# justinkay/aldi

Measured on AMD Instinct MI355X. Metric: images/sec (student+teacher ALDI step), R50-FPN 1333x800, higher is better.
Workload: dtype bf16

## Files before the change

### aldi_amd/_lib.py

```python
from __future__ import annotations

import ctypes as C
import os
import re

_HERE = os.path.dirname(os.path.abspath(__file__))
LIB_PATH = os.path.join(_HERE, "lib", "libaldi_hip.so")
HEADER_PATH = os.path.join(os.path.dirname(_HERE), "include", "aldi_hip.h")


class AldiHipError(RuntimeError):
    pass


if not os.path.exists(LIB_PATH):
    raise ImportError(
        f"{LIB_PATH} not found: build it with `python -c 'import __graft_entry__ as g; g.build()'` "
        "(or `make -C aldi_amd/csrc`). There is no CPU fallback for the ALDI HIP path.")

lib = C.CDLL(LIB_PATH)

F32, BF16 = 0, 1
MAX_IMAGES, MAX_LEVELS = 16, 5
c_void_p, c_int, c_float, c_long = C.c_void_p, C.c_int, C.c_float, C.c_long


def _ctype(decl: str):
    decl = decl.strip()
    if "*" in decl or decl.startswith("aldi_stream_t"):
        return C.c_void_p
    base = decl.rsplit(" ", 1)[0].replace("const", "").strip() if " " in decl else decl
    return {"int": C.c_int, "long": C.c_long, "float": C.c_float, "size_t": C.c_size_t, "unsigned": C.c_uint, "unsigned long long": C.c_ulonglong,
            "double": C.c_double}[base]


def parse_header(path: str = HEADER_PATH):
    src = open(path).read()
    src = re.sub(r"/\*.*?\*/", "", src, flags=re.S)
    protos = {}
    for m in re.finditer(r"\b(int|long|size_t|const char\*)\s+(aldi_\w+)\s*\(([^;{}]*?)\)\s*;", src, flags=re.S):
        ret, name, args = m.group(1), m.group(2), m.group(3)
        args = " ".join(args.split())
        argtypes = [] if args in ("void", "") else [_ctype(a) for a in args.split(",")]
        restype = {"int": C.c_int, "long": C.c_long, "size_t": C.c_size_t, "const char*": C.c_char_p}[ret]
        protos[name] = (restype, argtypes)
    return protos


PROTOS = parse_header()
for _name, (_res, _args) in PROTOS.items():
    _fn = getattr(lib, _name)
    _fn.restype = _res
    _fn.argtypes = _args


def check(status: int, what: str = ""):
    if status != 0:
        raise AldiHipError(f"{what}: status {status}: {lib.aldi_last_error().decode()}")


def call(name: str, *args):
    check(getattr(lib, name)(*args), name)


def set_tuning(name: str, value: int):
    call("aldi_set_tuning", name.encode(), int(value))


def get_tuning(name: str) -> int:
    v = C.c_int(0)
    call("aldi_get_tuning", name.encode(), C.byref(v))
    return v.value


def reset_tuning():
    call("aldi_reset_tuning")


def last_dispatch() -> str:
    return lib.aldi_last_dispatch().decode()


def plan_dispatch(args, n: int = 1) -> str:
    buf = C.create_string_buffer(224)
    call("aldi_conv_igemm_plan", C.byref(args) if isinstance(args, C.Structure) else args, n, buf, len(buf))
    return buf.value.decode()


def plan_wgrad_dispatch(args, n: int = 1, group: bool = False):
    buf = C.create_string_buffer(224)
    ws = C.c_long(0)
    call("aldi_conv_wgrad_plan", C.byref(args) if isinstance(args, C.Structure) else args, n, int(group), buf, len(buf), C.byref(ws))
    return buf.value.decode(), ws.value


class BoxLossChunk(C.Structure):
    _fields_ = [("r0", c_int), ("r1", c_int), ("grad_scale_cls", c_float), ("grad_scale_box", c_float), ("loss_box", c_void_p),
                ("teacher_pred", c_void_p), ("cls_temperature", c_float), ("kl", c_int), ("do_cls", c_int), ("do_reg", c_int),
                ("grad_scale_distill_cls", c_float), ("grad_scale_distill_reg", c_float), ("loss_distill", c_void_p)]


class ConvArgs(C.Structure):
    _fields_ = [
        ("x", c_void_p), ("w", c_void_p), ("y", c_void_p), ("y_f32", c_void_p),
        ("scale", c_void_p), ("shift", c_void_p), ("res", c_void_p), ("mask", c_void_p),
        ("N", c_int), ("H", c_int), ("W", c_int), ("Cin", c_int),
        ("Cout", c_int), ("KH", c_int), ("KW", c_int), ("stride", c_int), ("pad", c_int),
        ("Ho", c_int), ("Wo", c_int),
        ("relu", c_int), ("res_mode", c_int), ("out_scale", c_int), ("OH", c_int), ("OW", c_int),
        ("dtype", c_int), ("ws", c_void_p), ("ksplit", c_int), ("mask_bits", c_void_p), ("bits_out", c_void_p),
    ]


class WgradArgs(C.Structure):
    _fields_ = [
        ("x", c_void_p), ("g", c_void_p), ("dw", c_void_p), ("scale", c_void_p),
        ("N", c_int), ("H", c_int), ("W", c_int), ("Cin", c_int), ("Cout", c_int), ("KH", c_int), ("KW", c_int),
        ("stride", c_int), ("pad", c_int), ("Ho", c_int), ("Wo", c_int), ("dtype", c_int), ("db", c_void_p),
        ("ws", c_void_p), ("ws_bytes", C.c_long),
    ]


class StemArgs(C.Structure):
    _fields_ = [
        ("img", c_void_p), ("w", c_void_p), ("scale", c_void_p), ("shift", c_void_p), ("y", c_void_p),
        ("N", c_int), ("Hs", c_int), ("Ws", c_int), ("Hc", c_int), ("Wc", c_int),
        ("h", c_int * MAX_IMAGES), ("w_img", c_int * MAX_IMAGES),
        ("mean", c_float * 3), ("std", c_float * 3), ("dtype", c_int),
    ]


class RpnGeom(C.Structure):
    _fields_ = [
        ("num_levels", c_int), ("A", c_int), ("C", c_int),
        ("H", c_int * MAX_LEVELS), ("W", c_int * MAX_LEVELS), ("off", c_int * (MAX_LEVELS + 1)),
    ]


class RoiFeats(C.Structure):
    _fields_ = [
        ("feat", c_void_p * 4), ("grad", c_void_p * 4), ("H", c_int * 4), ("W", c_int * 4),
        ("scale", c_float * 4), ("C", c_int),
    ]


class DgwItem(C.Structure):
    _fields_ = [("w_master", c_void_p), ("scale", c_void_p), ("wt", c_void_p),
                ("Cout", c_int), ("KH", c_int), ("KW", c_int), ("Cin", c_int), ("tile_begin", c_int), ("reserved", c_int)]


class FoldItem(C.Structure):
    _fields_ = [("w", c_void_p), ("scale", c_void_p), ("out", c_void_p), ("rows", c_int), ("cols", c_int), ("chunk_begin", c_int), ("reserved", c_int)]


class BottleneckArgs(C.Structure):
    _fields_ = [("x", c_void_p), ("res", c_void_p), ("y", c_void_p), ("w1", c_void_p), ("w2", c_void_p), ("w3", c_void_p),
                ("b1", c_void_p), ("b2", c_void_p), ("b3", c_void_p),
                ("N", c_int), ("H", c_int), ("W", c_int), ("Cin", c_int), ("mid", c_int), ("Cout", c_int)]


class AttnArgs(C.Structure):
    _fields_ = [
        ("qkv", c_void_p), ("rel_h", c_void_p), ("rel_w", c_void_p),
        ("Qp", c_void_p), ("Kp", c_void_p), ("KpT", c_void_p), ("VT", c_void_p), ("QsT", c_void_p),
        ("O", c_void_p), ("lse", c_void_p), ("dO", c_void_p), ("dOT", c_void_p), ("dQp", c_void_p), ("delta", c_void_p),
        ("dqkv", c_void_p), ("drel_h", c_void_p), ("drel_w", c_void_p),
        ("nB", c_int), ("gh", c_int), ("gw", c_int), ("heads", c_int), ("Dq", c_int), ("scale", c_float),
    ]


PtrArray5 = c_void_p * MAX_LEVELS
```

### aldi_amd/csrc/igemm.hip

```cpp
#include "common.h"
#include "igemm_select.h"
#include "tile_prims.h"
#include <stdlib.h>

namespace {

template <typename T, int BM, int BN, int WM, int WN, int LDS_BYTES>
__device__ __forceinline__ void igemm_epilogue(const ConvDev& p, f32x4_t (&acc)[BM / WM / 16][BN / WN / 16], const int m0, const int n0, unsigned char* stg) {
    constexpr int NT = WM * WN * 64;
    constexpr int TM = BM / WM / 16, TN = BN / WN / 16;
    const int tid = threadIdx.x, lane = tid & 63, wave = tid >> 6;
    const int wm = wave / WN, wn = wave % WN;
    const int fr = lane & 15, fq = lane >> 4;
    if (p.dbg & 4) return;
    T* __restrict__ Y = static_cast<T*>(p.y);
    const T* __restrict__ R = static_cast<const T*>(p.res);
    const T* __restrict__ Mk = static_cast<const T*>(p.mask);
    if constexpr (sizeof(T) == 2) {
        constexpr int ROWB = BN * 2 + 16;
        constexpr bool kStageFits = BM * ROWB <= LDS_BYTES;
        if (kStageFits && Y && !p.y_f32 && (p.Cout & 7) == 0) {
            __syncthreads();
            {
                unsigned char* wr = stg + (wm * (BM / WM) + fr) * ROWB + (wn * (BN / WN) + fq * 4) * 2;
#pragma unroll
                for (int j = 0; j < TN; ++j) {
                    const int c = n0 + wn * (BN / WN) + j * 16 + fq * 4;
                    float4 sc = make_float4(1.f, 1.f, 1.f, 1.f), sh = make_float4(0.f, 0.f, 0.f, 0.f);
                    if (c < p.Cout) {
                        if (p.scale) sc = *reinterpret_cast<const float4*>(p.scale + c);
                        if (p.shift) sh = *reinterpret_cast<const float4*>(p.shift + c);
                    }
#pragma unroll
                    for (int i = 0; i < TM; ++i) {
                        uint2 t;
                        if (p.scale || p.shift) {
                            t.x = pack2_bf16(acc[i][j][0] * sc.x + sh.x, acc[i][j][1] * sc.y + sh.y);
                            t.y = pack2_bf16(acc[i][j][2] * sc.z + sh.z, acc[i][j][3] * sc.w + sh.w);
                        } else {
                            t.x = pack2_bf16(acc[i][j][0], acc[i][j][1]);
                            t.y = pack2_bf16(acc[i][j][2], acc[i][j][3]);
                        }
                        *reinterpret_cast<uint2*>(wr + i * 16 * ROWB + j * 32) = t;
                    }
                }
            }
            __syncthreads();
            constexpr int CPR = BN / 8;
            constexpr int RPI = NT / CPR;
            const int rowl0 = tid / CPR, ch8 = tid % CPR;
            const int c = n0 + ch8 * 8;
            if (c >= p.Cout) return;
            const bool plain = p.out_scale == 1 && p.res_mode != 2;
            const unsigned char* rd = stg + rowl0 * ROWB + ch8 * 16;
            typedef short s16x2_t __attribute__((ext_vector_type(2)));
            constexpr int NI = BM / RPI;
            constexpr unsigned OOBX = 0x80000000u;
            const __amdgpu_buffer_rsrc_t ry = make_rsrc_uniform(Y, 0x7fffffffu);
            unsigned ooff[NI], roff[NI], boff[NI];
#pragma unroll
            for (int it = 0; it < NI; ++it) {
                const int m = m0 + rowl0 + it * RPI;
                const bool ok = m < p.M;
                unsigned oidx, ridx;
                if (plain) {
                    oidx = (unsigned)m * (unsigned)p.Cout;
                    ridx = oidx;
                } else {
                    const int mm = ok ? m : 0;
                    const int n = mm / (p.Ho * p.Wo);
                    const int r = mm - n * (p.Ho * p.Wo);
                    const int ho = r / p.Wo, wo = r - ho * p.Wo;
                    if (p.out_scale == 1) oidx = (unsigned)mm * (unsigned)p.Cout;
                    else oidx = (unsigned)((((long)n * p.OH + ho * p.out_scale) * p.OW + wo * p.out_scale) * p.Cout);
                    if (p.res_mode == 2) ridx = (unsigned)((((long)n * (p.Ho >> 1) + (ho >> 1)) * (p.Wo >> 1) + (wo >> 1)) * p.Cout);
                    else ridx = oidx;
                }
                ooff[it] = ok ? (oidx + (unsigned)c) * 2u : OOBX;
                roff[it] = ok ? (ridx + (unsigned)c) * 2u : OOBX;
                boff[it] = ok ? (oidx + (unsigned)c) >> 3 : OOBX;
            }
            u32x4_t rres[NI], rmsk[NI];
            if (p.res_mode) {
                const __amdgpu_buffer_rsrc_t rr_ = make_rsrc_uniform(R, 0x7fffffffu);
#pragma unroll
                for (int it = 0; it < NI; ++it) rres[it] = __builtin_amdgcn_raw_buffer_load_b128(rr_, roff[it], 0, 0);
            }
            if (Mk) {
                const __amdgpu_buffer_rsrc_t rm_ = make_rsrc_uniform(Mk, 0x7fffffffu);
#pragma unroll
                for (int it = 0; it < NI; ++it) rmsk[it] = __builtin_amdgcn_raw_buffer_load_b128(rm_, ooff[it], 0, 0);
            }
            unsigned rbits[NI];
            if (p.mask_bits) {
                const __amdgpu_buffer_rsrc_t rb_ = make_rsrc_uniform(p.mask_bits, 0x7fffffffu);
#pragma unroll
                for (int it = 0; it < NI; ++it) rbits[it] = __builtin_amdgcn_raw_buffer_load_b8(rb_, boff[it], 0, 0);
            }
            const __amdgpu_buffer_rsrc_t rbo = make_rsrc_uniform(p.bits_out, 0x7fffffffu);
#pragma unroll
            for (int it = 0; it < NI; ++it) {
                const uint4 raw4 = *reinterpret_cast<const uint4*>(rd + it * RPI * ROWB);
                uint32_t raw[4] = {raw4.x, raw4.y, raw4.z, raw4.w};
                if (p.res_mode) {
                    const uint32_t rs[4] = {rres[it].x, rres[it].y, rres[it].z, rres[it].w};
#pragma unroll
                    for (int q = 0; q < 4; ++q) {
                        float lo = __uint_as_float(raw[q] << 16) + __uint_as_float(rs[q] << 16);
                        float hi = __uint_as_float(raw[q] & 0xffff0000u) + __uint_as_float(rs[q] & 0xffff0000u);
                        if (p.relu) { lo = fmaxf(lo, 0.f); hi = fmaxf(hi, 0.f); }
                        raw[q] = pack2_bf16(lo, hi);
                    }
                } else if (p.relu) {
#pragma unroll
                    for (int q = 0; q < 4; ++q) {
                        s16x2_t v = *reinterpret_cast<s16x2_t*>(&raw[q]);
                        v = __builtin_elementwise_max(v, s16x2_t{0, 0});
                        raw[q] = *reinterpret_cast<uint32_t*>(&v);
                    }
                }
                if (Mk) {
                    const uint32_t ms[4] = {rmsk[it].x, rmsk[it].y, rmsk[it].z, rmsk[it].w};
#pragma unroll
                    for (int q = 0; q < 4; ++q) {
                        s16x2_t k = *reinterpret_cast<const s16x2_t*>(&ms[q]);
                        k = __builtin_elementwise_min(__builtin_elementwise_max(k, s16x2_t{0, 0}), s16x2_t{1, 1});
                        s16x2_t v = *reinterpret_cast<s16x2_t*>(&raw[q]);
                        v = v * k;
                        raw[q] = *reinterpret_cast<uint32_t*>(&v);
                    }
                }
                if (p.mask_bits) {
                    const unsigned b = rbits[it];
#pragma unroll
                    for (int q = 0; q < 4; ++q) {
                        const unsigned k32 = ((b >> (2 * q)) & 1u) | (((b >> (2 * q + 1)) & 1u) << 16);
                        s16x2_t k = *reinterpret_cast<const s16x2_t*>(&k32);
                        s16x2_t v = *reinterpret_cast<s16x2_t*>(&raw[q]);
                        v = v * k;
                        raw[q] = *reinterpret_cast<uint32_t*>(&v);
                    }
                }
                const u32x4_t ov = {raw[0], raw[1], raw[2], raw[3]};
                __builtin_amdgcn_raw_buffer_store_b128(ov, ry, ooff[it], 0, 0);
                if (p.bits_out) {
                    unsigned b = 0;
#pragma unroll
                    for (int q = 0; q < 4; ++q) {
                        b |= ((short)(raw[q] & 0xffffu) > 0 ? 1u : 0u) << (2 * q);
                        b |= ((short)(raw[q] >> 16) > 0 ? 1u : 0u) << (2 * q + 1);
                    }
                    __builtin_amdgcn_raw_buffer_store_b8((unsigned char)b, rbo, boff[it], 0, 0);
                }
            }
            return;
        }
    }
#pragma unroll
    for (int i = 0; i < TM; ++i) {
        int m = m0 + wm * (BM / WM) + i * 16 + fr;
        if (m >= p.M) continue;
        long oidx, ridx = 0;
        if (p.out_scale == 1 && p.res_mode != 2) {
            oidx = (long)m * p.Cout;
            ridx = oidx;
        } else {
            int n = m / (p.Ho * p.Wo);
            int r = m - n * (p.Ho * p.Wo);
            int ho = r / p.Wo, wo = r - ho * p.Wo;
            if (p.out_scale == 1) oidx = (long)m * p.Cout;
            else oidx = (((long)n * p.OH + ho * p.out_scale) * p.OW + wo * p.out_scale) * p.Cout;
            if (p.res_mode == 2) ridx = (((long)n * (p.Ho >> 1) + (ho >> 1)) * (p.Wo >> 1) + (wo >> 1)) * p.Cout;
            else ridx = oidx;
        }
#pragma unroll
        for (int j = 0; j < TN; ++j) {
            int c = n0 + wn * (BN / WN) + j * 16 + fq * 4;
            if (c >= p.Cout) continue;
            float v[4] = {acc[i][j][0], acc[i][j][1], acc[i][j][2], acc[i][j][3]};
            if (p.scale) {
                float4 sc = *reinterpret_cast<const float4*>(p.scale + c);
                v[0] *= sc.x; v[1] *= sc.y; v[2] *= sc.z; v[3] *= sc.w;
            }
            if (p.shift) {
                float4 sh = *reinterpret_cast<const float4*>(p.shift + c);
                v[0] += sh.x; v[1] += sh.y; v[2] += sh.z; v[3] += sh.w;
            }
            if (p.res_mode) {
                float r4[4];
                load4(R + ridx + c, r4);
                v[0] += r4[0]; v[1] += r4[1]; v[2] += r4[2]; v[3] += r4[3];
            }
            if (p.relu) {
#pragma unroll
                for (int r = 0; r < 4; ++r) v[r] = v[r] > 0.f ? v[r] : 0.f;
            }
            if (Mk) {
                float k4[4];
                load4(Mk + oidx + c, k4);
#pragma unroll
                for (int r = 0; r < 4; ++r) v[r] = k4[r] > 0.f ? v[r] : 0.f;
            }
            if (Y) store4(Y + oidx + c, v);
            if (p.y_f32) store4(p.y_f32 + oidx + c, v);
        }
    }
}


template <int N, int ROWB, int I = 0>
__device__ __forceinline__ void frag_read_each(u32x4_t* f, const unsigned* addr) {
    if constexpr (I < N) {
        f[I] = frag_read<I * 16 * ROWB>(addr[I]);
        frag_read_each<N, ROWB, I + 1>(f, addr);
    }
}

template <int WNE>
__device__ __forceinline__ int direct_perm(int row) {
    const int wv = row / WNE, rr = row % WNE, j = rr >> 4, r = rr & 15;
    return wv * WNE + (j >> 1) * 32 + (r >> 2) * 8 + (j & 1) * 4 + (r & 3);
}
__device__ __forceinline__ unsigned lds_read_u8(unsigned addr) {
    unsigned v;
    asm volatile("ds_read_u8 %0, %1" : "=v"(v) : "v"(addr));
    return v;
}
template <int BM, int BN, int WM, int WN, bool RESL>
__device__ __forceinline__ void igemm_epilogue_direct(const ConvDev& p, f32x4_t (&acc)[BM / WM / 16][BN / WN / 16], const int m0, const int n0,
                                                      u32x4_t (&rres)[BM / WM / 16][BN / WN / 32], const unsigned aux_addr) {
    constexpr int TM = BM / WM / 16, TN = BN / WN / 16, WNE = BN / WN, H = WNE / 32;
    static_assert(TN == 2 * H, "whole 32-channel blocks per wave");
    const int tid = threadIdx.x, lane = tid & 63, wave = tid >> 6;
    const int wm = wave / WN, wn = wave % WN;
    const int fr = lane & 15, fq = lane >> 4;
    if (p.dbg & 4) return;
    u32x4_t sc[TN], sh[TN];
    const bool has_sc = p.scale != nullptr, has_sh = p.shift != nullptr;
#pragma unroll
    for (int j = 0; j < TN; ++j) {
        const unsigned a = aux_addr + (unsigned)(wn * WNE + (j >> 1) * 32 + fq * 8 + (j & 1) * 4) * 4u;
        sc[j] = frag_read<0>(a);
        sh[j] = frag_read<256>(a);
    }
    unsigned mb[TM][H];
#pragma unroll
    for (int i = 0; i < TM; ++i)
#pragma unroll
        for (int h = 0; h < H; ++h) mb[i][h] = lds_read_u8(aux_addr + (unsigned)((wm * (BM / WM) + i * 16 + fr) * (BN / 8) + (wn * H + h) * 4 + fq));
    asm volatile("s_waitcnt lgkmcnt(0)" ::: "memory");
#pragma unroll
    for (int j = 0; j < TN; ++j) { asm volatile("" : "+v"(sc[j])); asm volatile("" : "+v"(sh[j])); }
#pragma unroll
    for (int i = 0; i < TM; ++i)
#pragma unroll
        for (int h = 0; h < H; ++h) asm volatile("" : "+v"(mb[i][h]));
    const bool has_res = RESL && p.res_mode != 0;
    if constexpr (RESL) {
        if (has_res) {
#pragma unroll
            for (int i = 0; i < TM; ++i)
#pragma unroll
                for (int h = 0; h < H; ++h) asm volatile("" : "+v"(rres[i][h]));
        }
    }
    const __amdgpu_buffer_rsrc_t ry = make_rsrc_uniform(p.y, 0x7fffffffu);
    const __amdgpu_buffer_rsrc_t rbo = make_rsrc_uniform(p.bits_out, 0x7fffffffu);
    typedef short s16x2_t __attribute__((ext_vector_type(2)));
    typedef unsigned short u16x2_t __attribute__((ext_vector_type(2)));
#pragma unroll
    for (int i = 0; i < TM; ++i) {
        const int m = m0 + wm * (BM / WM) + i * 16 + fr;
#pragma unroll
        for (int h = 0; h < H; ++h) {
            const int c = n0 + wn * WNE + h * 32 + fq * 8;
            const bool ok = m < p.M && c < p.Cout;
            const unsigned e0 = (unsigned)m * (unsigned)p.Cout + (unsigned)c;
            float v[8];
#pragma unroll
            for (int e = 0; e < 4; ++e) { v[e] = acc[i][2 * h][e]; v[4 + e] = acc[i][2 * h + 1][e]; }
            if (has_sc) {
#pragma unroll
                for (int e = 0; e < 4; ++e) { v[e] *= __uint_as_float(sc[2 * h][e]); v[4 + e] *= __uint_as_float(sc[2 * h + 1][e]); }
            }
            if (has_sh) {
#pragma unroll
                for (int e = 0; e < 4; ++e) { v[e] += __uint_as_float(sh[2 * h][e]); v[4 + e] += __uint_as_float(sh[2 * h + 1][e]); }
            }
            if constexpr (RESL) {
                if (has_res) {
#pragma unroll
                    for (int q = 0; q < 4; ++q) {
                        const unsigned r2 = rres[i][h][q];
                        v[2 * q] += __uint_as_float(r2 << 16);
                        v[2 * q + 1] += __uint_as_float(r2 & 0xffff0000u);
                    }
                }
            }
            if (p.mask_bits) {
#pragma unroll
                for (int t = 0; t < 8; ++t) v[t] = __uint_as_float(__float_as_uint(v[t]) & (unsigned)__builtin_amdgcn_sbfe((int)mb[i][h], t, 1));
            }
            uint32_t d[4];
#pragma unroll
            for (int q = 0; q < 4; ++q) d[q] = pack2_bf16(v[2 * q], v[2 * q + 1]);
            if (p.relu) {
#pragma unroll
                for (int q = 0; q < 4; ++q) {
                    s16x2_t t = *reinterpret_cast<s16x2_t*>(&d[q]);
                    t = __builtin_elementwise_max(t, s16x2_t{0, 0});
                    d[q] = *reinterpret_cast<uint32_t*>(&t);
                }
            }
            const u32x4_t ov = {d[0], d[1], d[2], d[3]};
            __builtin_amdgcn_raw_buffer_store_b128(ov, ry, ok ? e0 * 2u : 0x80000000u, 0, 0);
            if (p.bits_out) {
                unsigned u = 0;
#pragma unroll
                for (int q = 0; q < 4; ++q) {
                    u16x2_t t = *reinterpret_cast<u16x2_t*>(&d[q]);
                    if (!p.relu) { s16x2_t s_ = *reinterpret_cast<s16x2_t*>(&d[q]); s_ = __builtin_elementwise_max(s_, s16x2_t{0, 0}); t = *reinterpret_cast<u16x2_t*>(&s_); }
                    t = __builtin_elementwise_min(t, u16x2_t{1, 1});
                    u |= *reinterpret_cast<unsigned*>(&t) << (2 * q);
                }
                const unsigned b = (u & 0x55u) | ((u >> 15) & 0xaau);
                __builtin_amdgcn_raw_buffer_store_b8((unsigned char)b, rbo, ok ? e0 >> 3 : 0x80000000u, 0, 0);
            }
        }
    }
}

template <typename T, int BM, int BN, int WM, int WN, int KC, bool PIPE, bool HALO = false, int EPI = 0, bool LEAN = false>
__device__ __forceinline__ void igemm_body(const ConvDev& p, int bid, const int nmt, const int nnt) {
    static_assert(!LEAN || (EPI != 0 && !HALO), "lean K loop: the direct-epilogue tap tiles");
    constexpr int NT = WM * WN * 64;
    constexpr bool DIRECT = EPI != 0, RESL = EPI == 2;
    static_assert(!DIRECT || (sizeof(T) == 2 && BN == 64 && (BN / WN) % 32 == 0 && BM * BN / 32 <= NT), "direct epilogue: bf16, 64-channel tiles");
    static_assert(!RESL || (PIPE && !HALO), "residual prefetch: the register-pipelined 1x1 loop");
    constexpr int EP = Elem<T>::kPer16B;
    constexpr int BK = KC * EP;
    constexpr int LOG = KC == 8 ? 3 : 2;
    constexpr int A_IT = (BM * KC) / NT;
    constexpr int B_IT = (BN * KC + NT - 1) / NT;
    constexpr int TM = BM / WM / 16, TN = BN / WN / 16;
    static_assert(HALO || (BM * KC) % NT == 0, "tile/threads mismatch");

    constexpr int NBUF = 3;
    constexpr int SLOTS = HALO ? ((BM + 2) * KC + 63) / 64 * 64 + 3 * BN * KC : (BM + BN) * KC;
    constexpr int NSTAGE = HALO ? 2 : NBUF;
    constexpr int AUX_SLOTS = DIRECT ? 64 : 0;
    constexpr int ZERO_SLOTS = HALO ? 4 : 0;
    __shared__ __attribute__((aligned(128))) uint4 lds_all[NSTAGE * SLOTS + AUX_SLOTS + ZERO_SLOTS];
    uint4 (*const lds)[SLOTS] = reinterpret_cast<uint4 (*)[SLOTS]>(&lds_all[0]);
    uint4* const aux_lds = &lds_all[NSTAGE * SLOTS];
    constexpr int N_RES = RESL ? (BM / WM / 16) * (BN / WN / 32) : 0;
    constexpr int N_PRE = DIRECT ? N_RES + 1 : 0;
    u32x4_t rres[BM / WM / 16][BN / WN / 32 > 0 ? BN / WN / 32 : 1];

    const int tid = threadIdx.x, lane = tid & 63, wave = tid >> 6;
    const int wm = wave / WN, wn = wave % WN;
    if (p.xcd) {
        const int total = nmt * nnt, q = total >> 3, r = total & 7, xcd = bid & 7, idx = bid >> 3;
        bid = (xcd < r ? xcd * (q + 1) : r * (q + 1) + (xcd - r) * q) + idx;
    }
    const int m0 = (bid / nnt) * BM, n0 = (bid % nnt) * BN;
    const T* __restrict__ X = static_cast<const T*>(p.x);
    const T* __restrict__ Wt = static_cast<const T*>(p.w);

    const __amdgpu_buffer_rsrc_t rx = __builtin_amdgcn_make_buffer_rsrc(const_cast<T*>(X), 0, p.x_bytes, 0x00020000);
    const __amdgpu_buffer_rsrc_t rw = __builtin_amdgcn_make_buffer_rsrc(const_cast<T*>(Wt), 0, p.w_bytes, 0x00020000);
    constexpr unsigned OOB = 0x80000000u;
    const int wbase = __builtin_amdgcn_readfirstlane(tid & ~63);
    auto issue_pre = [&]() {
        if constexpr (DIRECT) {
            if constexpr (RESL) {
                const __amdgpu_buffer_rsrc_t rr = make_rsrc_uniform(p.res, 0x7fffffffu);
#pragma unroll
                for (int i = 0; i < BM / WM / 16; ++i) {
                    const int m = m0 + wm * (BM / WM) + i * 16 + (lane & 15);
                    unsigned ridx = (unsigned)m;
                    if (p.res_mode == 2) {
                        const int mm = m < p.M ? m : 0;
                        const int n = mm / (p.Ho * p.Wo), r = mm - n * (p.Ho * p.Wo), ho = r / p.Wo, wo = r - ho * p.Wo;
                        ridx = (unsigned)((n * (p.Ho >> 1) + (ho >> 1)) * (p.Wo >> 1) + (wo >> 1));
                    }
#pragma unroll
                    for (int h = 0; h < BN / WN / 32; ++h) {
                        const int ch = n0 + wn * (BN / WN) + h * 32 + (lane >> 4) * 8;
                        const bool ok = p.res_mode && m < p.M && ch < p.Cout;
                        rres[i][h] = __builtin_amdgcn_raw_buffer_load_b128(rr, ok ? (ridx * (unsigned)p.Cout + (unsigned)ch) * 2u : OOB, 0, 0);
                    }
                }
            }
            if (p.mask_bits) {
                const __amdgpu_buffer_rsrc_t rb = make_rsrc_uniform(p.mask_bits, 0x7fffffffu);
                const int row = tid >> 1, m = m0 + row, ch = n0 + (tid & 1) * 32;
                const bool ok = tid < BM * 2 && m < p.M && ch < p.Cout;
                __builtin_amdgcn_raw_ptr_buffer_load_lds(rb, (__attribute__((address_space(3))) void*)(reinterpret_cast<unsigned*>(aux_lds) + wbase), 4,
                                                         ok ? ((unsigned)m * (unsigned)p.Cout + (unsigned)ch) >> 3 : OOB, 0, 0, 0);
            } else {
                const bool odd = __builtin_amdgcn_readfirstlane(wave) & 1;
                const float* src = odd ? p.shift : p.scale;
                const __amdgpu_buffer_rsrc_t rs = make_rsrc_uniform(src, 0x7fffffffu);
                const int ch = n0 + lane;
                __builtin_amdgcn_raw_ptr_buffer_load_lds(rs, (__attribute__((address_space(3))) void*)(reinterpret_cast<unsigned*>(aux_lds) + (odd ? 64 : 0)), 4,
                                                         src && ch < p.Cout ? (unsigned)ch * 4u : OOB, 0, 0, 0);
            }
        }
    };
    f32x4_t acc[TM][TN];
#pragma unroll
    for (int i = 0; i < TM; ++i)
#pragma unroll
        for (int j = 0; j < TN; ++j) acc[i][j] = f32x4_t{0.f, 0.f, 0.f, 0.f};

    const int fr = lane & 15, fq = lane >> 4;
    bool pre_seen = true;
    if constexpr (HALO) {
    static_assert(KC == 4, "halo form: one MFMA k-step per tap");
    constexpr int AS = ((BM + 2) * KC + 63) / 64 * 64;
    constexpr int WS = 3 * BN * KC;
    constexpr int AH_IT = (AS + NT - 1) / NT, WH_IT = WS / NT;
    static_assert(WS % NT == 0, "weight slots per thread");
    unsigned ha_voff[AH_IT], ha_mask[AH_IT];
#pragma unroll
    for (int it = 0; it < AH_IT; ++it) {
        const int c = tid + it * NT, row = c >> 2, kce = swz_halo(row, c & 3);
        const int q0 = m0 - 1 + row;
        const bool ok = row < BM + 2 && q0 >= 0 && q0 < p.M;
        const int qq = ok ? q0 : 0;
        const int h0 = (qq / p.W) % p.H;
        ha_voff[it] = ((unsigned)qq * (unsigned)p.Cin + (unsigned)(kce * EP)) * (unsigned)sizeof(T);
        ha_mask[it] = ok ? ((h0 >= 1 ? 1u : 0u) | 2u | (h0 <= p.H - 2 ? 4u : 0u)) : 0u;
    }
    unsigned hw_voff[WH_IT];
#pragma unroll
    for (int it = 0; it < WH_IT; ++it) {
        const int c = tid + it * NT, kwi = c / (BN * KC), rem = c - kwi * (BN * KC), row = rem >> 2, kce = swz_halo(row, rem & 3);
        const int co = n0 + (DIRECT ? direct_perm<BN / WN>(row) : row);
        hw_voff[it] = co < p.Cout ? ((unsigned)co * (unsigned)p.K + (unsigned)(kwi * p.Cin + kce * EP)) * (unsigned)sizeof(T) : OOB;
    }
    int gkh = 0, gci = 0;
    unsigned ha_cur[AH_IT], hw_cur[WH_IT];
    auto rebase = [&]() {
        const unsigned a_off = (unsigned)(((gkh - 1) * p.W * p.Cin) * (int)sizeof(T));
#pragma unroll
        for (int it = 0; it < AH_IT; ++it) ha_cur[it] = ((ha_mask[it] >> gkh) & 1u) ? ha_voff[it] + a_off : OOB;
    };
    rebase();
#pragma unroll
    for (int it = 0; it < WH_IT; ++it) hw_cur[it] = hw_voff[it];
    auto issue_group = [&](int buf) {
#pragma unroll
        for (int it = 0; it < AH_IT; ++it)
            if (wbase + it * NT < AS) {
                glds16(rx, &lds[buf][wbase + it * NT], ha_cur[it]);
                ha_cur[it] += (unsigned)(BK * sizeof(T));
            }
#pragma unroll
        for (int it = 0; it < WH_IT; ++it) glds16(rw, &lds[buf][AS + wbase + it * NT], hw_cur[it]);
        gci += BK;
        unsigned w_adv = (unsigned)(BK * sizeof(T));
        if (gci >= p.Cin) {
            gci = 0; ++gkh;
            w_adv = (unsigned)((2 * p.Cin + BK) * (int)sizeof(T));
            rebase();
        }
#pragma unroll
        for (int it = 0; it < WH_IT; ++it) hw_cur[it] += w_adv;
    };
    bool edge_l[TM], edge_r[TM];
#pragma unroll
    for (int i = 0; i < TM; ++i) {
        const int m = m0 + wm * (BM / WM) + i * 16 + fr;
        const int wo = m % p.W;
        edge_l[i] = wo == 0;
        edge_r[i] = wo == p.W - 1;
    }
    const int xrow = wm * (BM / WM) + fr, wrow = wn * (BN / WN) + fr;
    const unsigned lbase = lds_addr(&lds[0][0]);
    unsigned x_rd[3];
#pragma unroll
    for (int kw = 0; kw < 3; ++kw) x_rd[kw] = lbase + (unsigned)((xrow + kw) * KC + swz_halo(xrow + kw, fq)) * 16u;
    const unsigned w_rd = lbase + (unsigned)((AS + wrow * KC) + swz_halo(wrow, fq)) * 16u;
    uint4* const zero_lds = &lds_all[NSTAGE * SLOTS + AUX_SLOTS];
    if (tid < ZERO_SLOTS) zero_lds[tid] = make_uint4(0u, 0u, 0u, 0u);
    unsigned zaddr[TM];
#pragma unroll
    for (int i = 0; i < TM; ++i) zaddr[i] = lds_addr(zero_lds) + (unsigned)fq * 16u - (unsigned)(i * 16 * KC * 16);
    constexpr unsigned GROUP_BYTES = (AS + WS) * 16;
    const int G = 3 * (p.Cin / BK);
    issue_group(0);
    issue_pre();
    int buf = 0;
    for (int g = 0; g < G; ++g) {
        asm volatile("s_waitcnt vmcnt(0)" ::: "memory");
        __builtin_amdgcn_s_barrier();
        __builtin_amdgcn_sched_barrier(0);
        if (g + 1 < G) issue_group(buf ^ 1);
        u32x4_t xf[2][TM], wf[2][TN];
        const unsigned gb = (unsigned)buf * GROUP_BYTES;
        {
            unsigned xa[TM];
#pragma unroll
            for (int i = 0; i < TM; ++i) xa[i] = edge_l[i] ? zaddr[i] : x_rd[0] + gb;
            frag_read_each<TM, KC * 16>(xf[0], xa);
        }
        frag_read_all<TN, KC * 16>(wf[0], w_rd + gb);
        frag_wait<TM, TN>(xf[0], wf[0]);
#pragma unroll
        for (int kw = 0; kw < 3; ++kw) {
            const int cur = kw & 1, nxt = cur ^ 1;
            if (kw < 2) {
                if (kw + 1 == 2) {
                    unsigned xa[TM];
#pragma unroll
                    for (int i = 0; i < TM; ++i) xa[i] = edge_r[i] ? zaddr[i] : x_rd[2] + gb;
                    frag_read_each<TM, KC * 16>(xf[nxt], xa);
                } else {
                    frag_read_all<TM, KC * 16>(xf[nxt], x_rd[kw + 1] + gb);
                }
                frag_read_all<TN, KC * 16>(wf[nxt], w_rd + gb + (unsigned)((kw + 1) * BN * KC * 16));
            }
#pragma unroll
            for (int i = 0; i < TM; ++i)
#pragma unroll
                for (int j = 0; j < TN; ++j) acc[i][j] = Mma<T>::run(wf[cur][j], xf[cur][i], acc[i][j]);
            if (kw < 2) frag_wait<TM, TN>(xf[nxt], wf[nxt]);
        }
        buf ^= 1;
    }
    } else {
    unsigned a_voff[A_IT], a_mask[A_IT];
    int a_kce[A_IT];
    unsigned b_voff[B_IT];
    int b_kce[B_IT];
    const bool ktail = !LEAN && (p.K % BK) != 0;
    if constexpr (LEAN) {
#pragma unroll
        for (int it = 0; it < A_IT; ++it) {
            const int c = tid + it * NT, row = c >> LOG, kce = swz<KC>(row, c & (KC - 1)), m = m0 + row;
            a_voff[it] = m < p.M ? ((unsigned)m * (unsigned)p.Cin + (unsigned)(kce * EP)) * (unsigned)sizeof(T) : OOB;
// ... 203 lines not shown
    if (p.xcd) {
        const int total = nmt * nnt, q = total >> 3, r = total & 7, xcd = bid & 7, idx = bid >> 3;
        bid = (xcd < r ? xcd * (q + 1) : r * (q + 1) + (xcd - r) * q) + idx;
    }
    const int m0 = (bid / nnt) * BM, n0 = (bid % nnt) * BN;
    const T* __restrict__ X = static_cast<const T*>(p.x);
    const T* __restrict__ Wt = static_cast<const T*>(p.w);
    const __amdgpu_buffer_rsrc_t rx = __builtin_amdgcn_make_buffer_rsrc(const_cast<T*>(X), 0, p.x_bytes, 0x00020000);
    const __amdgpu_buffer_rsrc_t rw = __builtin_amdgcn_make_buffer_rsrc(const_cast<T*>(Wt), 0, p.w_bytes, 0x00020000);
    constexpr unsigned OOB = 0x80000000u;
    const int wbase = __builtin_amdgcn_readfirstlane(tid & ~63);
    const bool half_b = __builtin_amdgcn_readfirstlane(wave) >= 4;
    const bool third_pix = wbase + 2 * NT < AS;
    f32x4_t acc[TM][TN];
#pragma unroll
    for (int i = 0; i < TM; ++i)
#pragma unroll
        for (int j = 0; j < TN; ++j) acc[i][j] = f32x4_t{0.f, 0.f, 0.f, 0.f};
    const int fr = lane & 15, fq = lane >> 4;
    if (tid < 4) lds[NS * STAGE + tid] = make_uint4(0u, 0u, 0u, 0u);

    unsigned ha_voff[AH_IT], ha_mask[AH_IT];
#pragma unroll
    for (int it = 0; it < AH_IT; ++it) {
        const int c = tid + it * NT, row = c >> 2, kce = swz_halo(row, c & 3);
        const int q0 = m0 - 1 + row;
        const bool ok = row < BM + 2 && q0 >= 0 && q0 < p.M;
        const int qq = ok ? q0 : 0;
        const int h0 = (qq / p.W) % p.H;
        ha_voff[it] = ((unsigned)qq * (unsigned)p.Cin + (unsigned)(kce * EP)) * (unsigned)sizeof(T);
        ha_mask[it] = ok ? ((h0 >= 1 ? 1u : 0u) | 2u | (h0 <= p.H - 2 ? 4u : 0u)) : 0u;
    }
    unsigned hw_voff[WH_IT];
#pragma unroll
    for (int it = 0; it < WH_IT; ++it) {
        const int c = tid + it * NT, kwi = c / (BN * KC), rem = c - kwi * (BN * KC), row = rem >> 2, kce = swz_halo(row, rem & 3);
        const int co = n0 + row;
        hw_voff[it] = co < p.Cout ? ((unsigned)co * (unsigned)p.K + (unsigned)(kwi * p.Cin + kce * EP)) * (unsigned)sizeof(T) : OOB;
    }
    const int xrow = wm * (BM / WM) + fr, wrow = wn * (BN / WN) + fr;
    const unsigned lbase = lds_addr(&lds[0]);
    const unsigned zrow = lbase + (unsigned)(NS * STAGE) * 16u + (unsigned)fq * 16u;
    bool edge_l[TM], edge_r[TM];
    unsigned zaddr[TM];
#pragma unroll
    for (int i = 0; i < TM; ++i) {
        const int m = m0 + wm * (BM / WM) + i * 16 + fr;
        const int wo = m % p.W;
        edge_l[i] = wo == 0;
        edge_r[i] = wo == p.W - 1;
        zaddr[i] = zrow - (unsigned)(i * 16 * KC * 16);
    }
    unsigned x_rd[3];
#pragma unroll
    for (int kw = 0; kw < 3; ++kw) x_rd[kw] = lbase + (unsigned)((xrow + kw) * KC + swz_halo(xrow + kw, fq)) * 16u;
    const unsigned w_rd = lbase + (unsigned)((AS + wrow * KC) + swz_halo(wrow, fq)) * 16u;
    constexpr unsigned STAGE_BYTES = STAGE * 16;
    const int G = 3 * (p.Cin / BK);

    unsigned a_off = 0, w_off = 0, ikh = 0;
    int gkh = 0, gci = 0;
    auto next_group = [&]() {
        a_off = (unsigned)(((gkh - 1) * p.W * p.Cin + gci) * (int)sizeof(T));
        w_off = (unsigned)((gkh * 3 * p.Cin + gci) * (int)sizeof(T));
        ikh = (unsigned)gkh;
        gci += BK;
        if (gci >= p.Cin) { gci = 0; ++gkh; }
    };
    const unsigned dmask = (p.dbg & 16) ? 0xfffu : 0xffffffffu;
    const bool no_dma = p.dbg & 32, no_mfma = p.dbg & 64;
    auto issue_pair = [&](int pair, int st) {
        uint4* base = &lds[st * STAGE];
        if (no_dma) return;
        if (pair == 0) {
            glds16(rx, base + wbase, ((ha_mask[0] >> ikh) & 1u) ? (ha_voff[0] + a_off) & dmask : OOB);
            glds16(rx, base + wbase + NT, ((ha_mask[1] >> ikh) & 1u) ? (ha_voff[1] + a_off) & dmask : OOB);
        } else if (pair == 1) {
            glds16(rw, base + AS + wbase, hw_voff[0] == OOB ? OOB : (hw_voff[0] + w_off) & dmask);
            glds16(rw, base + AS + wbase + NT, hw_voff[1] == OOB ? OOB : (hw_voff[1] + w_off) & dmask);
        } else {
            glds16(rw, base + AS + wbase + 2 * NT, hw_voff[2] == OOB ? OOB : (hw_voff[2] + w_off) & dmask);
            if (third_pix) glds16(rx, base + wbase + 2 * NT, ((ha_mask[2] >> ikh) & 1u) ? (ha_voff[2] + a_off) & dmask : OOB);
        }
    };
    next_group();
    issue_pair(0, 0); issue_pair(1, 0); issue_pair(2, 0);
    next_group();
    issue_pair(0, 1); issue_pair(1, 1);
    asm volatile("s_waitcnt vmcnt(4)" ::: "memory");
    __builtin_amdgcn_s_barrier();
    __builtin_amdgcn_sched_barrier(0);
    if (half_b) {
        __builtin_amdgcn_s_barrier();
        __builtin_amdgcn_sched_barrier(0);
    }
    int rs = 0, s1 = 1, s2 = 2;
    for (int g = 0; g < G; ++g) {
        const unsigned gb = (unsigned)rs * STAGE_BYTES;
#pragma unroll
        for (int t = 0; t < 3; ++t) {
            u32x4_t xf[TM], wf[TN];
            if (t == 1) {
                frag_read_all<TM, KC * 16>(xf, x_rd[1] + gb);
            } else {
                unsigned xa[TM];
#pragma unroll
                for (int i = 0; i < TM; ++i) xa[i] = (t == 0 ? edge_l[i] : edge_r[i]) ? zaddr[i] : x_rd[t] + gb;
                frag_read_each<TM, KC * 16>(xf, xa);
            }
            frag_read_all<TN, KC * 16>(wf, w_rd + gb + (unsigned)(t * BN * KC * 16));
            if (t == 0) {
                if (g + 1 < G) issue_pair(2, s1);
            } else if (g + 2 < G) {
                if (t == 1) next_group();
                issue_pair(t - 1, s2);
            }
            if (t == 2 && g + 1 < G) {
                if (g + 2 < G && !no_dma) asm volatile("s_waitcnt vmcnt(4)" ::: "memory");
                else asm volatile("s_waitcnt vmcnt(0)" ::: "memory");
            }
            __builtin_amdgcn_sched_barrier(0);
            __builtin_amdgcn_s_barrier();
            __builtin_amdgcn_sched_barrier(0);
            frag_wait<TM, TN>(xf, wf);
            __builtin_amdgcn_sched_barrier(0);
            __builtin_amdgcn_s_setprio(1);
            if (!no_mfma) {
#pragma unroll
                for (int i = 0; i < TM; ++i)
#pragma unroll
                    for (int j = 0; j < TN; ++j) acc[i][j] = Mma<T>::run(wf[j], xf[i], acc[i][j]);
            }
            __builtin_amdgcn_s_setprio(0);
            __builtin_amdgcn_sched_barrier(0);
            __builtin_amdgcn_s_barrier();
            __builtin_amdgcn_sched_barrier(0);
        }
        const int o = rs; rs = s1; s1 = s2; s2 = o;
    }
    if (!half_b) {
        __builtin_amdgcn_s_barrier();
        __builtin_amdgcn_sched_barrier(0);
    }
    igemm_epilogue<T, BM, BN, WM, WN, NS * STAGE * 16>(p, acc, m0, n0, reinterpret_cast<unsigned char*>(&lds[0]));
}

template <typename T, int BN>
__global__ __launch_bounds__(512) void igemm_halo_rs_kernel(ConvDev p) {
    igemm_halo_rs_body<T, BN>(p, (int)(blockIdx.y * gridDim.x + blockIdx.x), (int)gridDim.x, (int)gridDim.y);
}

#include "igemm_halo64.h"
#include "igemm_ws.h"

template <int BM, int NT, bool HALO> constexpr int min_waves_per_simd() { return HALO && BM == 240 ? 2 * NT / 256 : 1; }
template <typename T, int BM, int BN, int WM, int WN, int KC, bool PIPE, bool HALO = false, int EPI = 0, bool LEAN = false>
__global__ __launch_bounds__(WM* WN * 64, (min_waves_per_simd<BM, WM * WN * 64, HALO>())) void igemm_kernel(ConvDev p) {
    igemm_body<T, BM, BN, WM, WN, KC, PIPE, HALO, EPI, LEAN>(p, (int)(blockIdx.y * gridDim.x + blockIdx.x), (int)gridDim.x, (int)gridDim.y);
}

template <typename T, int BM, int BN, int WM, int WN, int KC, bool PIPE, bool HALO = false>
__global__ __launch_bounds__(WM* WN * 64, (min_waves_per_simd<BM, WM * WN * 64, HALO>())) void igemm_group_kernel(ConvGroup G) {
    const int bid = (int)blockIdx.x;
    int i = 0;
    for (int k = 1; k < G.n; ++k)
        if (bid >= G.wg_begin[k]) i = k;
    i = __builtin_amdgcn_readfirstlane(i);
    const int local = bid - G.wg_begin[i];
    if (local >= G.nmt[i] * G.nnt[i]) return;
    igemm_body<T, BM, BN, WM, WN, KC, PIPE, HALO>(G.p[i], local, G.nmt[i], G.nnt[i]);
}

template <int BM, int BN, int WM, int WN, bool DIRECT, bool ILV = false>
__global__ __launch_bounds__(WM* WN * 64) void igemm_halo64_group_kernel(ConvGroup G) {
    const int bid = (int)blockIdx.x;
    int i = 0;
    for (int k = 1; k < G.n; ++k)
        if (bid >= G.wg_begin[k]) i = k;
    i = __builtin_amdgcn_readfirstlane(i);
    const int local = bid - G.wg_begin[i];
    if (local >= G.nmt[i] * G.nnt[i]) return;
    igemm_halo64_body<BM, BN, WM, WN, DIRECT, ILV>(G.p[i], local, G.nmt[i], G.nnt[i]);
}


int group_table(ConvGroup& G, const int BM, const int BN, const ConvDev& d) {
    int wg = 0;
    for (int i = 0; i < G.n; ++i) {
        G.p[i].xcd = d.xcd; G.p[i].dbg = d.dbg;
        G.nmt[i] = cdiv(G.p[i].M, BM); G.nnt[i] = cdiv(G.p[i].Cout, BN);
        G.wg_begin[i] = wg;
        wg += (G.nmt[i] * G.nnt[i] + 7) / 8 * 8;
    }
    for (int i = G.n; i <= kMaxConvGroup; ++i) G.wg_begin[i] = wg;
    return wg;
}

template <typename T, int BM, int BN, int WM, int WN, int KC, bool PIPE, bool HALO, int EPI>
int launch_tile(const Choice& c, const ConvDev& d, const ConvGroup* g, hipStream_t st) {
    constexpr int NT = WM * WN * 64;
    if constexpr (EPI != 0) {
        const dim3 grid(cdiv(d.M, BM), cdiv(d.Cout, BN));
        if constexpr (!HALO) {
            if (c.lean) hipLaunchKernelGGL((igemm_kernel<T, BM, BN, WM, WN, KC, PIPE, HALO, EPI, true>), grid, dim3(NT), 0, st, d);
        }
        if (HALO || !c.lean) hipLaunchKernelGGL((igemm_kernel<T, BM, BN, WM, WN, KC, PIPE, HALO, EPI, false>), grid, dim3(NT), 0, st, d);
    } else if (g) {
        ConvGroup G = *g;
        const int wg = group_table(G, BM, BN, d);
        hipLaunchKernelGGL((igemm_group_kernel<T, BM, BN, WM, WN, KC, PIPE, HALO>), dim3(wg), dim3(NT), 0, st, G);
    } else {
        const dim3 grid(cdiv(d.M, BM), cdiv(d.Cout, BN), d.ksplit > 1 ? d.ksplit : 1);
        hipLaunchKernelGGL((igemm_kernel<T, BM, BN, WM, WN, KC, PIPE, HALO>), grid, dim3(NT), 0, st, d);
    }
    ALDI_CHECK_LAUNCH();
    return ALDI_OK;
}
template <typename T, int BM, int BN, int WM, int WN, int KC, bool PIPE, int EPI>
int launch_TAP(const Choice& c, const ConvDev& d, const ConvGroup* g, hipStream_t st) { return launch_tile<T, BM, BN, WM, WN, KC, PIPE, false, EPI>(c, d, g, st); }
template <typename T, int BM, int BN, int WM, int WN, int KC, bool PIPE, int EPI>
int launch_HALO(const Choice& c, const ConvDev& d, const ConvGroup* g, hipStream_t st) { return launch_tile<T, BM, BN, WM, WN, KC, PIPE, true, EPI>(c, d, g, st); }

template <typename T, int BM, int BN, int WM, int WN, int KC, bool PIPE, int EPI>
int launch_ROLES(const Choice&, const ConvDev& d, const ConvGroup*, hipStream_t st) {
    static_assert(BM == 256 && WM * WN * 64 == 512, "igemm_halo_rs_body: 256 pixels on eight waves");
    const dim3 grid(cdiv(d.M, BM), cdiv(d.Cout, BN));
    hipLaunchKernelGGL((igemm_halo_rs_kernel<T, BN>), grid, dim3(512), 0, st, d);
    ALDI_CHECK_LAUNCH();
    return ALDI_OK;
}

template <typename T, int BM, int BN, int WM, int WN, int KC, bool PIPE, int EPI>
int launch_HALO64(const Choice& c, const ConvDev& d, const ConvGroup* g, hipStream_t st) {
    constexpr int NT = WM * WN * 64;
    constexpr bool HAS_ILV = BM == 256 && BN == 256 && WM == 4 && WN == 2;
    if (g) {
        ConvGroup G = *g;
        const int wg = group_table(G, BM, BN, d);
        if (c.ilv) {
            if (c.direct) hipLaunchKernelGGL((igemm_halo64_group_kernel<BM, BN, WM, WN, true, HAS_ILV>), dim3(wg), dim3(NT), 0, st, G);
            else hipLaunchKernelGGL((igemm_halo64_group_kernel<BM, BN, WM, WN, false, HAS_ILV>), dim3(wg), dim3(NT), 0, st, G);
        } else {
            if (c.direct) hipLaunchKernelGGL((igemm_halo64_group_kernel<BM, BN, WM, WN, true>), dim3(wg), dim3(NT), 0, st, G);
            else hipLaunchKernelGGL((igemm_halo64_group_kernel<BM, BN, WM, WN, false>), dim3(wg), dim3(NT), 0, st, G);
        }
    } else {
        const dim3 grid(cdiv(d.M, BM), cdiv(d.Cout, BN));
        if (c.ilv) {
            if (c.direct) hipLaunchKernelGGL((igemm_halo64_kernel<BM, BN, WM, WN, true, HAS_ILV>), grid, dim3(NT), 0, st, d);
            else hipLaunchKernelGGL((igemm_halo64_kernel<BM, BN, WM, WN, false, HAS_ILV>), grid, dim3(NT), 0, st, d);
        } else {
            if (c.direct) hipLaunchKernelGGL((igemm_halo64_kernel<BM, BN, WM, WN, true>), grid, dim3(NT), 0, st, d);
            else hipLaunchKernelGGL((igemm_halo64_kernel<BM, BN, WM, WN, false>), grid, dim3(NT), 0, st, d);
        }
    }
    ALDI_CHECK_LAUNCH();
    return ALDI_OK;
}

int launch_choice(const Choice& c, const ConvDev& d, const ConvGroup* g, hipStream_t st) {
    switch (c.tile) {
#define IGEMM_TILE_CASE(id, T, form, BM, BN, WM, WN, KC, PIPE, EPI) \
    case id: return launch_##form<T, BM, BN, WM, WN, KC, PIPE != 0, EPI>(c, d, g, st);
        IGEMM_TILES(IGEMM_TILE_CASE)
#undef IGEMM_TILE_CASE
    default: break;
    }
    return aldi_set_error_msg(ALDI_ERR_ARG, "conv_igemm: unknown tile");
}

__global__ __launch_bounds__(256) void splitk_finalize_kernel(const float* __restrict__ ws, int ks, long mc, int C, const float* __restrict__ scale,
                                                              const float* __restrict__ shift, int relu, bf16_t* __restrict__ y) {
    const long e = ((long)blockIdx.x * blockDim.x + threadIdx.x) * 4;
    if (e >= mc) return;
    float4 a = *reinterpret_cast<const float4*>(ws + e);
    for (int z = 1; z < ks; ++z) {
        const float4 b = *reinterpret_cast<const float4*>(ws + z * mc + e);
        a.x += b.x; a.y += b.y; a.z += b.z; a.w += b.w;
    }
    const int c = (int)(e % C);
    if (scale) { const float4 s4 = *reinterpret_cast<const float4*>(scale + c); a.x *= s4.x; a.y *= s4.y; a.z *= s4.z; a.w *= s4.w; }
    if (shift) { const float4 s4 = *reinterpret_cast<const float4*>(shift + c); a.x += s4.x; a.y += s4.y; a.z += s4.z; a.w += s4.w; }
    if (relu) { a.x = fmaxf(a.x, 0.f); a.y = fmaxf(a.y, 0.f); a.z = fmaxf(a.z, 0.f); a.w = fmaxf(a.w, 0.f); }
    uint2 o;
    o.x = pack2_bf16(a.x, a.y); o.y = pack2_bf16(a.z, a.w);
    *reinterpret_cast<uint2*>(y + e) = o;
}

constexpr int kNameCap = 112;

int conv_one(const aldi_conv_args* a, const bool dry, hipStream_t st, char* name) {
    ConvDev d;
    Choice c;
    if (int rc = plan_conv(a, aldi_tuning(), d, c)) return rc;
    dispatch_name(c, name, kNameCap);
    if (dry) return ALDI_OK;
    if (int rc = launch_choice(c, d, nullptr, st)) return rc;
    aldi_note_dispatch(name);
    if (c.ksplit > 1) {
        const long mc = (long)d.M * d.Cout;
        hipLaunchKernelGGL(splitk_finalize_kernel, dim3(cdiv(mc / 4, 256)), dim3(256), 0, st, static_cast<const float*>(a->ws), c.ksplit, mc, d.Cout, a->scale, a->shift,
                           a->relu, static_cast<bf16_t*>(a->y));
        ALDI_CHECK_LAUNCH();
    }
    return ALDI_OK;
}

int conv_many(const aldi_conv_args* args, const int n, const bool dry, hipStream_t st, char* name) {
    if (!args || n < 1) return aldi_set_error_msg(ALDI_ERR_ARG, "conv_igemm_group: no problems");
    if (n == 1 || !conv_group_same(args, n, aldi_tuning())) {
        for (int i = 0; i < n; ++i)
            if (int rc = conv_one(&args[i], dry, st, name)) return rc;
        return ALDI_OK;
    }
    static thread_local ConvGroup G;
    ConvDev d;
    Choice c;
    if (int rc = plan_conv_group(args, n, aldi_tuning(), G, d, c)) return rc;
    dispatch_name(c, name, kNameCap);
    if (dry) return ALDI_OK;
    if (int rc = launch_choice(c, d, &G, st)) return rc;
    aldi_note_dispatch(name);
    return ALDI_OK;
}
}

extern "C" int aldi_conv_igemm(const aldi_conv_args* a, aldi_stream_t stream) {
    char name[kNameCap];
    return conv_one(a, false, static_cast<hipStream_t>(stream), name);
}

extern "C" int aldi_conv_igemm_group(const aldi_conv_args* args, int n, aldi_stream_t stream) {
    char name[kNameCap];
    return conv_many(args, n, false, static_cast<hipStream_t>(stream), name);
}

extern "C" int aldi_conv_igemm_plan(const aldi_conv_args* args, int n, char* name, int cap) {
    char buf[kNameCap] = "";
    const int rc = n == 1 ? conv_one(args, true, nullptr, buf) : conv_many(args, n, true, nullptr, buf);
    if (rc == ALDI_OK && name && cap > 0) snprintf(name, (size_t)cap, "%s", buf);
    return rc;
}
```

### aldi_amd/csrc/igemm_select.h

```cpp
#pragma once
#include "host.h"
#include <stdio.h>

namespace {

struct ConvDev {
    const void* x; const void* w; void* y; float* y_f32;
    const float* scale; const float* shift; const void* res; const void* mask;
    int N, H, W, Cin, Cout, KH, KW, stride, pad, Ho, Wo;
    int relu, res_mode, out_scale, OH, OW;
    int M, K, xcd, dbg;
    unsigned x_bytes, w_bytes;
    int ksplit, slabs_per_split;
    int lean;
    const unsigned char* mask_bits; unsigned char* bits_out;
};

constexpr int kMaxConvGroup = 12;
struct ConvGroup {
    int n;
    int wg_begin[kMaxConvGroup + 1];
    int nmt[kMaxConvGroup], nnt[kMaxConvGroup];
    ConvDev p[kMaxConvGroup];
};
// ... 37 lines not shown
#undef IGEMM_TILE_ROW
};

struct Choice {
    TileId tile;
    bool lean;
    bool direct, ilv;
    int ksplit;
    int ws_wgs;
    int group_n;
};

inline int ws_channels(int K) { return K == 64 || K == 128 ? 256 : K == 256 || K == 512 ? 128 : 0; }
inline bool ws_ok(const ConvDev& d) {
    const int bn = ws_channels(d.K);
    return d.KH * d.KW == 1 && d.stride == 1 && d.pad == 0 && d.K == d.Cin && bn && d.Cout % bn == 0 && d.y && !d.y_f32 && !d.mask && d.out_scale == 1 &&
           d.ksplit <= 1 && (long)d.M * d.Cout * 2 < (1L << 31);
}
inline bool halo64_direct_ok(const ConvDev& d) {
    return d.y && !d.y_f32 && d.out_scale == 1 && (d.Cout & 7) == 0 && !d.mask && !d.mask_bits && !d.bits_out && !d.res_mode;
}
inline bool plain_1x1(const ConvDev& d) { return d.KH * d.KW == 1 && d.stride == 1 && d.pad == 0; }

inline Choice select_tile(const ConvDev& d, const AldiTuning& tn, const bool f32, const int group_n, const ConvDev* group = nullptr) {
    Choice c = {BF16_TAP_128x128, false, false, false, d.ksplit > 1 ? d.ksplit : 0, tn.igemm_ws_wgs, group_n};
    const auto pick = [&](TileId bf16_id, TileId f32_id) {
        c.tile = f32 ? f32_id : bf16_id;
        const TileRow& r = kTiles[c.tile];
        c.lean = r.form == TAP && r.epi != 0 && tn.igemm_lean && plain_1x1(d) && d.K % 64 == 0 && !(tn.igemm_dbg & (8 | 16));
        if (r.form == HALO64) {
            c.direct = (tn.igemm_direct & 8) != 0;
            for (int i = 0; i < (group_n ? group_n : 1); ++i) c.direct = c.direct && halo64_direct_ok(group_n ? group[i] : d);
            c.ilv = c.tile == BF16_HALO64_256x256 && tn.igemm_halo_ilv != 0;
        }
        return c;
    };
#define BOTH(name) pick(BF16_##name, F32_##name)
#define BF16(name) pick(BF16_##name, BF16_##name)
    const bool bf16 = !f32;
    if (d.ksplit > 1) {
        const int tile_knob = tn.igemm_splitk_tile;
        const bool big_ok = (long)cdiv(d.M, 256) * cdiv(d.Cout, 128) * d.ksplit >= 200;
        if (tile_knob == 3 || (tile_knob == 2 && big_ok)) return BF16(TAP_256x128_K64);
        if (tile_knob == 1 || (tile_knob == 4 && big_ok)) return BF16(TAP_256x128);
        return BF16(TAP_128x128_K64);
    }
    const long big = (long)cdiv(d.M, 128) * cdiv(d.Cout, 128);
    const int force = tn.igemm_force;
    const bool direct_ok = bf16 && !group_n && d.y && !d.y_f32 && d.out_scale == 1 && (d.Cout & 7) == 0 && !d.mask && d.ksplit <= 1 &&
                           !(d.mask_bits && (d.scale || d.shift)) && d.Cout >= 64 &&
                           !(d.mask_bits && (d.Cout & 31));
    const int direct = direct_ok ? tn.igemm_direct : 0;
    {
        const bool same3 = d.KH == 3 && d.KW == 3 && d.stride == 1 && d.pad == 1 && d.Ho == d.H && d.Wo == d.W && d.Cin % 32 == 0 && d.out_scale == 1;
        const bool f32_halo = f32 && tn.igemm_halo_f32 > 0 && (long)cdiv(d.M, 128) * cdiv(d.Cout, 64) >= tn.igemm_halo_f32;
        if (tn.igemm_halo && (bf16 || f32_halo) && same3) {
            if (force == 1) return BOTH(HALO_128x128);
            if (bf16 && force == 2 && (direct & 4) && !d.res_mode) return BF16(HALO_128x64_D);
            if (force == 2) return BOTH(HALO_128x64);
            if (force == 4) return BOTH(HALO_256x128);
            if (bf16) {
                if (force == 17 && (direct & 4) && !d.res_mode) return BF16(HALO_96x64_D);
                if (force == 17) return BF16(HALO_96x64);
                if (force == 16 && (direct & 4) && !d.res_mode) return BF16(HALO_64x64_D);
                if (force == 16) return BF16(HALO_64x64);
                if (force == 9) return BF16(HALO_240x128);
                if (force == 10 && !group_n) return BF16(ROLES_256x128);
                if (force == 11 && d.Cin % 64 == 0) return BF16(HALO64_256x256);
                if (force == 13 && d.Cin % 64 == 0) return BF16(HALO64_128x128);
                if (force == 15 && d.Cin % 64 == 0) return BF16(HALO64_256x256_W4);
            }
            if (force == 0 || force == 3) {
                if (d.Cout <= 64) return BOTH(HALO_128x64);
                if (big >= tn.igemm_bigtile_min) {
                    if (bf16 && tn.igemm_bigtile == 64 && d.Cin % 64 == 0 && d.Cout % 256 == 0) return BF16(HALO64_256x256);
                    if (bf16 && tn.igemm_bigtile == 65 && d.Cin % 64 == 0 && d.Cout % 256 == 0) return BF16(HALO64_256x256_W4);
                    if (tn.igemm_bigtile == 1) return BOTH(HALO_128x128);
                    if (bf16 && tn.igemm_bigtile == 10 && !group_n) return BF16(ROLES_256x128);
                    return BOTH(HALO_256x128);
                }
                if (bf16 && tn.igemm_halo64_mid > 0 && big >= tn.igemm_halo64_mid && d.Cin % 64 == 0 && d.Cout % 128 == 0) return BF16(HALO64_128x128);
                const long t64 = (long)cdiv(d.M, 128) * cdiv(d.Cout, 64);
                if (bf16 && tn.igemm_halo96 > 0 && t64 >= 200 && t64 <= 600) {
                    if ((direct & 4) && !d.res_mode) return BF16(HALO_96x64_D);
                    return BF16(HALO_96x64);
                }
                if (bf16 && tn.igemm_halo_small > 0 && t64 <= tn.igemm_halo_small && d.Cin >= 512) {
                    if ((direct & 4) && !d.res_mode) return BF16(HALO_64x64_D);
                    return BF16(HALO_64x64);
                }
                if (bf16 && (direct & 4) && !d.res_mode) return BF16(HALO_128x64_D);
                return BOTH(HALO_128x64);
            }
        }
    }
    if (bf16 && !group_n && ws_ok(d) && (force == 14 || (force == 0 && tn.igemm_ws && (tn.igemm_direct & 1) && d.M >= (d.res_mode == 2 ? 4L : 1L) * tn.igemm_ws_min)))
        return d.K == 64 ? BF16(WS_K64) : d.K == 128 ? BF16(WS_K128) : d.K == 256 ? BF16(WS_K256) : BF16(WS_K512);
    if (force == 5 || (force == 0 && d.Cout <= 16)) return BOTH(TAP_128x16);
    if (force == 1) return BOTH(TAP_128x128);
    if (bf16 && force == 2 && (direct & 1)) return d.res_mode ? BF16(TAP_128x64_DR) : BF16(TAP_128x64_D);
    if (force == 2) return BOTH(TAP_128x64);
    if (force == 3) return BOTH(TAP_64x64);
    if (force == 4) return BOTH(TAP_256x128);
    if (bf16) {
        const bool plain = plain_1x1(d);
        if (plain && force == 6) return BF16(TAP_128x128_K64);
        if (plain && force == 7) return BF16(TAP_128x64_K64);
        if (plain && force == 12 && (direct & 1) && !d.res_mode && d.K % 64 == 0) return BF16(TAP_128x64_K64_D);
        const bool lin256 = tn.igemm_tile != 9 && big >= tn.igemm_lintile_min && d.K >= tn.igemm_bigtile_k;
        if (plain && (force == 8 || (force == 0 && !lin256 && d.Cout > 64 && d.K % 64 == 0 && d.K >= tn.igemm_k64_min))) {
            if ((direct & 2) && !d.res_mode) return BF16(TAP_64x64_K64_D);
            return BF16(TAP_64x64_K64);
        }
    }
    if (f32 && force == 0 && big < tn.igemm_f32_tile64_max) return BOTH(TAP_64x64);
    if (d.Cout <= 64) return BOTH(TAP_128x64);
    if (tn.igemm_tile != 9 && big >= tn.igemm_lintile_min && d.K >= tn.igemm_bigtile_k) {
        if (bf16 && tn.igemm_tile != 7 && plain_1x1(d) && d.K % 64 == 0) return BF16(TAP_256x128_K64);
        return BOTH(TAP_256x128);
    }
    if (big < 200) return BOTH(TAP_64x64);
    if (bf16 && d.K <= tn.igemm_narrow_k && (direct & 1)) return d.res_mode ? BF16(TAP_128x64_DR) : BF16(TAP_128x64_D);
    if (bf16 && d.K <= tn.igemm_narrow_k) return BOTH(TAP_128x64);
    return BOTH(TAP_128x128);
#undef BOTH
#undef BF16
}

inline int dispatch_name(const Choice& c, char* name, int cap) {
    const TileRow& r = kTiles[c.tile];
    const char* elem = r.f32 ? "f32" : "bf16";
    const char* grp = c.group_n ? "_group" : "";
    switch (r.form) {
    case WS: return snprintf(name, cap, "igemm_ws<%s,%d,%d,k%d>", elem, r.BM, r.BN, r.KC * 8);
    case HALO64:
        return snprintf(name, cap, "igemm%s%.0d<%s,%d,%d,%d,%d,halo64%s%s>", grp, c.group_n, elem, r.BM, r.BN, r.WM, r.WN, c.direct ? ",direct" : "",
                        (c.tile == BF16_HALO64_256x256 && !c.ilv) ? ",lockstep" : "");
    case ROLES: return snprintf(name, cap, "igemm<%s,%d,%d,%d,%d,roles,halo>", elem, r.BM, r.BN, r.WM, r.WN);
    default:
        return snprintf(name, cap, "igemm%s%.0d<%s,%d,%d,%d,%d,%s,%s%s%s>%s", grp, c.group_n, elem, r.BM, r.BN, r.WM, r.WN, r.pipe ? "pipe" : "flat", r.form == HALO ? "halo" : "tap",
                        r.KC == 8 ? ",k64" : "", r.epi == 2 ? ",direct+res" : r.epi == 1 ? ",direct" : "", c.ksplit > 1 ? " splitk" : "");
    }
}

inline int fill_convdev(const aldi_conv_args* a, ConvDev& d) {
    if (!a || !a->x || !a->w || (!a->y && !a->y_f32)) return aldi_set_error_msg(ALDI_ERR_ARG, "conv_igemm: null pointer");
    const int bk = a->dtype == ALDI_BF16 ? 32 : 16;
    const int ep = a->dtype == ALDI_BF16 ? 8 : 4;
    if (a->dtype != ALDI_BF16 && a->dtype != ALDI_F32) return aldi_set_error_msg(ALDI_ERR_ARG, "conv_igemm: bad dtype");
    if (a->KH * a->KW == 1 ? (a->Cin % ep != 0) : (a->Cin % bk != 0))
        return aldi_set_error_msg(ALDI_ERR_ARG, "conv_igemm: Cin must be a multiple of 32 (bf16) / 16 (f32) for KxK convs; of a 16-B chunk for 1x1");
    if (a->Cout % 4 != 0) return aldi_set_error_msg(ALDI_ERR_ARG, "conv_igemm: Cout must be a multiple of 4");
    if (a->res_mode == 2 && ((a->Ho & 1) || (a->Wo & 1))) return aldi_set_error_msg(ALDI_ERR_ARG, "conv_igemm: upsample residual needs even Ho,Wo");
    if (a->res_mode && !a->res) return aldi_set_error_msg(ALDI_ERR_ARG, "conv_igemm: res_mode set without res");
    d.x = a->x; d.w = a->w; d.y = a->y; d.y_f32 = a->y_f32; d.scale = a->scale; d.shift = a->shift;
    d.res = a->res; d.mask = a->mask;
    d.N = a->N; d.H = a->H; d.W = a->W; d.Cin = a->Cin; d.Cout = a->Cout; d.KH = a->KH; d.KW = a->KW;
    d.stride = a->stride; d.pad = a->pad; d.Ho = a->Ho; d.Wo = a->Wo;
    d.relu = a->relu; d.res_mode = a->res_mode; d.out_scale = a->out_scale < 1 ? 1 : a->out_scale;
    d.OH = a->OH; d.OW = a->OW;
    long M = (long)a->N * a->Ho * a->Wo;
    if (M <= 0 || M > 0x7fffffffL) return aldi_set_error_msg(ALDI_ERR_ARG, "conv_igemm: bad M");
    d.M = (int)M;
    d.K = a->KH * a->KW * a->Cin;
    const size_t esz = a->dtype == ALDI_BF16 ? 2 : 4;
    const size_t xb = (size_t)a->N * a->H * a->W * a->Cin * esz, wb = (size_t)a->Cout * d.K * esz;
    const size_t yb = (size_t)a->N * (d.out_scale > 1 ? (size_t)a->OH * a->OW : (size_t)a->Ho * a->Wo) * a->Cout * esz;
    if (xb >= 0x80000000ull || wb >= 0x80000000ull || yb >= 0x80000000ull)
        return aldi_set_error_msg(ALDI_ERR_ARG, "conv_igemm: operand larger than 2 GiB (32-bit buffer offsets)");
    if (a->KH * a->KW > 16) return aldi_set_error_msg(ALDI_ERR_ARG, "conv_igemm: at most 16 taps");
    d.x_bytes = (unsigned)xb;
    d.w_bytes = (unsigned)wb;
    d.xcd = 0; d.dbg = 0;
    d.ksplit = 0; d.slabs_per_split = 0; d.lean = 0;
    d.mask_bits = static_cast<const unsigned char*>(a->mask_bits);
    d.bits_out = static_cast<unsigned char*>(a->bits_out);
    if ((a->mask_bits || a->bits_out) && (a->dtype != ALDI_BF16 || (a->Cout & 7) || d.out_scale != 1 || a->res_mode == 2 || !a->y || a->y_f32 || a->ksplit > 1))
        return aldi_set_error_msg(ALDI_ERR_ARG, "conv_igemm: bit masks take bf16 outputs with Cout % 8 == 0 in the plain layout (no fp32 output, scatter, upsampled residual or split-K)");
    if (a->mask_bits && a->mask) return aldi_set_error_msg(ALDI_ERR_ARG, "conv_igemm: mask and mask_bits are alternatives");
    return ALDI_OK;
}

inline int plan_conv(const aldi_conv_args* a, const AldiTuning& tn, ConvDev& d, Choice& c) {
    if (int rc = fill_convdev(a, d)) return rc;
    if (a->ksplit > 1) {
        const int ks = a->ksplit;
        if (a->dtype != ALDI_BF16 || a->KH * a->KW != 1 || a->stride != 1 || a->pad != 0 || a->res_mode || a->mask || a->y_f32 || !a->y || !a->ws ||
            (a->out_scale > 1) || d.K % (64 * ks) != 0 || ks > 64)
            return aldi_set_error_msg(ALDI_ERR_ARG, "conv_igemm: split-K takes bf16 plain 1x1 / linear layers with K % (64 * ksplit) == 0, a workspace, no res / mask / fp32 output");
        d.y = nullptr; d.y_f32 = static_cast<float*>(a->ws); d.scale = nullptr; d.shift = nullptr; d.relu = 0;
        d.ksplit = ks;
    }
    c = select_tile(d, tn, a->dtype != ALDI_BF16, 0);
    d.xcd = tn.igemm_xcd; d.dbg = tn.igemm_dbg;
    if (c.ksplit > 1) d.slabs_per_split = d.K / (kTiles[c.tile].KC * 8) / c.ksplit;
    return ALDI_OK;
}

inline bool conv_group_same(const aldi_conv_args* args, int n, const AldiTuning& tn) {
    bool same = n <= kMaxConvGroup && tn.igemm_group;
    for (int i = 1; i < n && same; ++i) {
        const aldi_conv_args &a = args[0], &b = args[i];
        same = a.dtype == b.dtype && a.Cin == b.Cin && a.Cout == b.Cout && a.KH == b.KH && a.KW == b.KW &&
               a.stride == b.stride && a.pad == b.pad && (a.Ho == a.H) == (b.Ho == b.H) && (a.Wo == a.W) == (b.Wo == b.W) && a.out_scale == b.out_scale &&
               (a.y != nullptr) == (b.y != nullptr) && (a.y_f32 != nullptr) == (b.y_f32 != nullptr);
    }
    return same;
}

inline int plan_conv_group(const aldi_conv_args* args, int n, const AldiTuning& tn, ConvGroup& G, ConvDev& d, Choice& c) {
    G.n = n;
    long Msum = 0;
    for (int i = 0; i < n; ++i) {
        if (int rc = fill_convdev(&args[i], G.p[i])) return rc;
        Msum += G.p[i].M;
    }
    for (int i = 1; i < n; ++i)
        for (int j = i; j > 0 && G.p[j].M > G.p[j - 1].M; --j) { const ConvDev t_ = G.p[j]; G.p[j] = G.p[j - 1]; G.p[j - 1] = t_; }
    d = G.p[0];
    d.M = (int)(Msum > 0x7fffffffL ? 0x7fffffffL : Msum);
    c = select_tile(d, tn, args[0].dtype != ALDI_BF16, n, G.p);
    d.xcd = tn.igemm_xcd; d.dbg = tn.igemm_dbg;
    return ALDI_OK;
}

}
```

### aldi_amd/csrc/igemm_ws.h

```cpp
#pragma once

template <int KS, int TM, int TN>
__global__ __launch_bounds__(256, 2) void igemm_ws_kernel(ConvDev p, const int n_mtiles, const int ncg) {
    typedef bf16_t T;
    constexpr int BM = TM * 16, K = KS * 32, WNE = TN * 16, BN = 4 * WNE, H = TN / 2;
    constexpr int STAGE16 = BM * K * 2 / 16;
    constexpr int P = STAGE16 / 256;
    constexpr int NBUF = 3;
    static_assert(TN % 2 == 0 && STAGE16 % 256 == 0 && P >= 1 && K % 64 == 0, "whole 32-channel blocks per wave; whole DMA pieces per wave; whole 128-byte slabs");
    __shared__ __attribute__((aligned(128))) uint4 lds[NBUF * STAGE16 + BN / 2];
    const int tid = threadIdx.x, lane = tid & 63, wave = tid >> 6;
    const int fr = lane & 15, fq = lane >> 4;

    const int xcd = blockIdx.x & 7, slot = blockIdx.x >> 3;
    const int cg = slot % ncg, g = (slot / ncg) * 8 + xcd, G = (int)(gridDim.x >> 3) / ncg * 8;
    const int nt = g < n_mtiles ? (n_mtiles - g + G - 1) / G : 0;
    const int n0 = cg * BN + wave * WNE;

    u32x4_t wreg[TN][KS];
    {
        const T* __restrict__ Wp = static_cast<const T*>(p.w);
#pragma unroll
        for (int j = 0; j < TN; ++j) {
            const int co = n0 + (j >> 1) * 32 + (fr >> 2) * 8 + (j & 1) * 4 + (fr & 3);
#pragma unroll
            for (int ks = 0; ks < KS; ++ks) wreg[j][ks] = *reinterpret_cast<const u32x4_t*>(Wp + (size_t)co * K + ks * 32 + fq * 8);
        }
    }
    {
        float* aux = reinterpret_cast<float*>(&lds[NBUF * STAGE16]);
        for (int c = tid; c < BN; c += 256) {
            aux[c] = p.scale ? p.scale[cg * BN + c] : 1.f;
            aux[BN + c] = p.shift ? p.shift[cg * BN + c] : 0.f;
        }
    }
    const __amdgpu_buffer_rsrc_t rx = __builtin_amdgcn_make_buffer_rsrc(const_cast<T*>(static_cast<const T*>(p.x)), 0, p.x_bytes, 0x00020000);
    const unsigned out_bytes = (unsigned)p.M * (unsigned)p.Cout * 2u;
    const bool res_up = p.res_mode == 2;
    const __amdgpu_buffer_rsrc_t rr = make_rsrc_uniform(p.res, res_up ? out_bytes >> 2 : out_bytes);
    const __amdgpu_buffer_rsrc_t rmb = make_rsrc_uniform(p.mask_bits, out_bytes >> 4);
    const __amdgpu_buffer_rsrc_t ry = make_rsrc_uniform(p.y, out_bytes);
    const __amdgpu_buffer_rsrc_t rbo = make_rsrc_uniform(p.bits_out, out_bytes >> 4);
    constexpr unsigned OOB = 0x80000000u;

    unsigned vbase[P];
#pragma unroll
    for (int it = 0; it < P; ++it) {
        const int c = (wave + 4 * it) * 64 + lane, rr_ = c >> 3, r = rr_ % BM, s = rr_ / BM, lc = (c & 7) ^ ((r >> 1) & 7);
        vbase[it] = (unsigned)((r * K + s * 64 + lc * 8) * 2);
    }
    const int wbase = __builtin_amdgcn_readfirstlane(wave * 64);
    auto issue_tile = [&](int k, int stage) {
        const unsigned m0b = (unsigned)(g + k * G) * (unsigned)(BM * K * 2);
#pragma unroll
        for (int it = 0; it < P; ++it) glds16(rx, &lds[stage * STAGE16 + it * 256 + wbase], vbase[it] + m0b);
    };
    const unsigned lds0 = lds_addr(&lds[0]);
    const unsigned rd0 = lds0 + (unsigned)(fr * 128 + ((fq ^ ((fr >> 1) & 7)) * 16));
    const unsigned rd1 = lds0 + (unsigned)(fr * 128 + (((4 + fq) ^ ((fr >> 1) & 7)) * 16));
    const unsigned aux_rd = lds0 + (unsigned)(NBUF * STAGE16 * 16) + (unsigned)((wave * WNE + fq * 8) * 4);
    const bool has_sc = p.scale != nullptr, has_sh = p.shift != nullptr, has_res = p.res_mode != 0, has_mb = p.mask_bits != nullptr, has_bo = p.bits_out != nullptr;
    const bool relu = p.relu != 0, no_epi = (p.dbg & 4) != 0;
    const unsigned C2 = (unsigned)p.Cout * 2u, C8 = (unsigned)p.Cout >> 3;
    typedef short s16x2_t __attribute__((ext_vector_type(2)));
    typedef unsigned short u16x2_t __attribute__((ext_vector_type(2)));

    const float inv_wo = 1.f / (float)p.Wo, inv_ho = 1.f / (float)p.Ho;
    auto fdiv = [](unsigned m, unsigned d, float inv) {
        unsigned q = (unsigned)(((float)m + 0.5f) * inv);
        if (q * d > m) --q;
        else if ((q + 1) * d <= m) ++q;
        return q;
    };
    auto fetch_pre = [&](int k, u32x4_t (&rres)[TM][H], unsigned (&mb)[TM][H]) {
        const int m0 = (g + k * G) * BM;
#pragma unroll
        for (int i = 0; i < TM; ++i)
#pragma unroll
            for (int h = 0; h < H; ++h) {
                const unsigned m = (unsigned)(m0 + i * 16 + fr), c = (unsigned)(n0 + h * 32 + fq * 8);
                if (has_res) {
                    unsigned row = m;
                    if (res_up) {
                        const unsigned t_ = fdiv(m, (unsigned)p.Wo, inv_wo), wo = m - t_ * (unsigned)p.Wo, n = fdiv(t_, (unsigned)p.Ho, inv_ho), ho = t_ - n * (unsigned)p.Ho;
                        row = (n * (unsigned)(p.Ho >> 1) + (ho >> 1)) * (unsigned)(p.Wo >> 1) + (wo >> 1);
                    }
                    rres[i][h] = __builtin_amdgcn_raw_buffer_load_b128(rr, m < (unsigned)p.M ? row * C2 + c * 2u : OOB, 0, 0);
                }
                if (has_mb) mb[i][h] = __builtin_amdgcn_raw_buffer_load_b8(rmb, m * C8 + (c >> 3), 0, 0);
            }
    };
    auto step = [&](int k, int stage, u32x4_t (&rres)[TM][H], unsigned (&mb)[TM][H], u32x4_t (&rres_n)[TM][H], unsigned (&mb_n)[TM][H]) {
        __builtin_amdgcn_s_barrier();
        __builtin_amdgcn_sched_barrier(0);
        const int m0 = (g + k * G) * BM;
        const bool more = k + 2 < nt;
        if (more) issue_tile(k + 2, stage == 0 ? 2 : stage - 1);
        __builtin_amdgcn_sched_barrier(0);
        if (k + 1 < nt) fetch_pre(k + 1, rres_n, mb_n);
        __builtin_amdgcn_sched_barrier(0);
        f32x4_t acc[TM][TN];
        const unsigned sb = (unsigned)(stage * STAGE16 * 16);
        u32x4_t xa[TM], xb[TM];
        frag_read_n<TM, 2048, 0>(xa, rd0 + sb);
#pragma unroll
        for (int ks = 0; ks < KS; ++ks) {
            u32x4_t* cur = (ks & 1) ? xb : xa;
            u32x4_t* nxt = (ks & 1) ? xa : xb;
            frag_wait1<TM>(cur);
            if (ks + 1 < KS) {
                const unsigned a = (((ks + 1) & 1) ? rd1 : rd0) + sb + (unsigned)(((ks + 1) >> 1) * BM * 128);
                frag_read_n<TM, 2048, 0>(nxt, a);
            }
#pragma unroll
            for (int i = 0; i < TM; ++i)
#pragma unroll
                for (int j = 0; j < TN; ++j)
                    acc[i][j] = Mma<T>::run(wreg[j][ks], cur[i], ks == 0 ? f32x4_t{0.f, 0.f, 0.f, 0.f} : acc[i][j]);
        }
        if (no_epi) asm volatile("s_waitcnt vmcnt(0)" ::: "memory");
        else if (more) asm volatile("s_waitcnt vmcnt(%0)" ::"n"(P + TM * H) : "memory");
        else asm volatile("s_waitcnt vmcnt(%0)" ::"n"(TM * H) : "memory");
        if (no_epi) return;
#pragma unroll
        for (int h = 0; h < H; ++h) {
            u32x4_t sc0 = frag_read<0>(aux_rd + h * 128), sc1 = frag_read<16>(aux_rd + h * 128);
            u32x4_t sh0 = frag_read<BN * 4>(aux_rd + h * 128), sh1 = frag_read<BN * 4 + 16>(aux_rd + h * 128);
            asm volatile("s_waitcnt lgkmcnt(0)" ::: "memory");
            asm volatile("" : "+v"(sc0)); asm volatile("" : "+v"(sc1)); asm volatile("" : "+v"(sh0)); asm volatile("" : "+v"(sh1));
            const unsigned c = (unsigned)(n0 + h * 32 + fq * 8);
#pragma unroll
            for (int i = 0; i < TM; ++i) {
                const unsigned m = (unsigned)(m0 + i * 16 + fr);
                const unsigned e0 = m * (unsigned)p.Cout + c;
                const bool ok = m < (unsigned)p.M;
                float v[8];
#pragma unroll
                for (int e = 0; e < 4; ++e) { v[e] = acc[i][2 * h][e]; v[4 + e] = acc[i][2 * h + 1][e]; }
                if (has_sc) {
#pragma unroll
                    for (int e = 0; e < 4; ++e) { v[e] *= __uint_as_float(sc0[e]); v[4 + e] *= __uint_as_float(sc1[e]); }
                }
                if (has_sh) {
#pragma unroll
                    for (int e = 0; e < 4; ++e) { v[e] += __uint_as_float(sh0[e]); v[4 + e] += __uint_as_float(sh1[e]); }
                }
                if (has_res) {
#pragma unroll
                    for (int q = 0; q < 4; ++q) {
                        const unsigned r2 = rres[i][h][q];
                        v[2 * q] += __uint_as_float(r2 << 16);
                        v[2 * q + 1] += __uint_as_float(r2 & 0xffff0000u);
                    }
                }
                if (has_mb) {
#pragma unroll
                    for (int t = 0; t < 8; ++t) v[t] = __uint_as_float(__float_as_uint(v[t]) & (unsigned)__builtin_amdgcn_sbfe((int)mb[i][h], t, 1));
                }
                uint32_t d[4];
#pragma unroll
                for (int q = 0; q < 4; ++q) d[q] = pack2_bf16(v[2 * q], v[2 * q + 1]);
                if (relu) {
#pragma unroll
                    for (int q = 0; q < 4; ++q) {
                        s16x2_t t = *reinterpret_cast<s16x2_t*>(&d[q]);
                        t = __builtin_elementwise_max(t, s16x2_t{0, 0});
                        d[q] = *reinterpret_cast<uint32_t*>(&t);
                    }
                }
                const u32x4_t ov = {d[0], d[1], d[2], d[3]};
                __builtin_amdgcn_raw_buffer_store_b128(ov, ry, ok ? e0 * 2u : OOB, 0, 0);
                if (has_bo) {
                    unsigned u = 0;
#pragma unroll
                    for (int q = 0; q < 4; ++q) {
                        u16x2_t t = *reinterpret_cast<u16x2_t*>(&d[q]);
                        if (!relu) { s16x2_t s_ = *reinterpret_cast<s16x2_t*>(&d[q]); s_ = __builtin_elementwise_max(s_, s16x2_t{0, 0}); t = *reinterpret_cast<u16x2_t*>(&s_); }
                        t = __builtin_elementwise_min(t, u16x2_t{1, 1});
                        u |= *reinterpret_cast<unsigned*>(&t) << (2 * q);
                    }
                    const unsigned b = (u & 0x55u) | ((u >> 15) & 0xaau);
                    __builtin_amdgcn_raw_buffer_store_b8((unsigned char)b, rbo, ok ? e0 >> 3 : OOB, 0, 0);
                }
            }
        }
    };

    u32x4_t resA[TM][H], resB[TM][H];
    unsigned mbA[TM][H], mbB[TM][H];
    if (nt > 0) issue_tile(0, 0);
    if (nt > 1) issue_tile(1, 1);
    if (nt > 0) fetch_pre(0, resA, mbA);
    asm volatile("s_waitcnt vmcnt(0)" ::: "memory");
    __syncthreads();
    int stage = 0;
    for (int k = 0; k < nt; k += 2) {
        step(k, stage, resA, mbA, resB, mbB);
        stage = stage == NBUF - 1 ? 0 : stage + 1;
        if (k + 1 < nt) {
            step(k + 1, stage, resB, mbB, resA, mbA);
            stage = stage == NBUF - 1 ? 0 : stage + 1;
        }
    }
}

template <typename T, int BM, int BN, int WM, int WN, int KC, bool PIPE, int EPI>
int launch_WS(const Choice& c, const ConvDev& d, const ConvGroup*, hipStream_t st) {
    const int ncg = d.Cout / BN;
    const int n_mtiles = cdiv(d.M, BM);
    int sets = c.ws_wgs / (8 * ncg);
    if (sets < 1) sets = 1;
    if (sets > cdiv(n_mtiles, 8)) sets = cdiv(n_mtiles, 8);
    const dim3 grid(sets * 8 * ncg), block(256);
    hipLaunchKernelGGL((igemm_ws_kernel<KC / 4, BM / 16, BN / 64>), grid, block, 0, st, d, n_mtiles, ncg);
    ALDI_CHECK_LAUNCH();
    return ALDI_OK;
}
```

### aldi_amd/engine.py

```python
from __future__ import annotations

import contextlib
import dataclasses
import inspect
import math
import os
from collections import OrderedDict
from typing import Dict, List, Optional, Sequence, Tuple

import torch

from . import ops
from .arch import FC_DIM, FPN_C, NUM_ANCHORS, POOL, STAGE_BLOCKS, Packed, ParamLayout, pad_to

PIXEL_MEAN = (103.530, 116.280, 123.675)
PIXEL_STD = (1.0, 1.0, 1.0)
ANCHOR_SIZES = (32, 64, 128, 256, 512)
ANCHOR_RATIOS = (0.5, 1.0, 2.0)
STRIDES = (4, 8, 16, 32, 64)
GMAX = 128
RPN_BATCH, RPN_POS_FRAC = 256, 0.5
ROI_BATCH, ROI_POS_FRAC = 512, 0.25
RPN_PRE = (2000, 1000)
RPN_POST = (1000, 1000)
# ... 193 lines not shown
        ops.sgd_step(self.master, self.grad, self.mom, self.compute if self.dtype != torch.float32 else None, n, lr, momentum,
                     weight_decay, grad_scale * getattr(self, "_gscale", 1.0), self.first_step, self.dtype)
        self._after_sgd()

    def _after_sgd(self):
        self.first_step = False
        if self.lazy_wt:
            self._wt_dirty = True
        else:
            self._refresh_wt()

    def sgd_range_dev(self, lo: int, hi: int, hyper: torch.Tensor):
        hi = min(hi, self.layout.n_train)
        if hi > lo:
            ops.sgd_step_dev(self.master, self.grad, self.mom, self.compute if self.dtype != torch.float32 else None, lo, hi, hyper, self.dtype)

    def ema_from(self, student: "Weights", alpha: float, copy_only: bool):
        n = self.layout.n_total
        if self.dtype == torch.bfloat16:
            ops.ema_update(self.master, student.master, self.compute, n, alpha, copy_only, self.dtype, n_compute=self.layout.n_weights)
            self.refresh(cast=False)
        else:
            ops.ema_update(self.master, student.master, None, n, alpha, copy_only, torch.float32)
            self.refresh()


def make_anchors(shapes: Sequence[Tuple[int, int]], device, sizes: Sequence[float] = ANCHOR_SIZES) -> torch.Tensor:
    out = []
    for (h, w), size, stride in zip(shapes, sizes, STRIDES):
        cell = []
        for r in ANCHOR_RATIOS:
            area = size ** 2.0
            aw = math.sqrt(area / r)
            ah = r * aw
            cell.append([-aw / 2.0, -ah / 2.0, aw / 2.0, ah / 2.0])
        cell = torch.tensor(cell, dtype=torch.float32)
        sx = torch.arange(0, w * stride, step=stride, dtype=torch.float32)
        sy = torch.arange(0, h * stride, step=stride, dtype=torch.float32)
        yy, xx = torch.meshgrid(sy, sx, indexing="ij")
        shifts = torch.stack((xx.reshape(-1), yy.reshape(-1), xx.reshape(-1), yy.reshape(-1)), dim=1)
        out.append((shifts.view(-1, 1, 4) + cell.view(1, -1, 4)).reshape(-1, 4))
    return torch.cat(out).contiguous().to(device)


@dataclasses.dataclass(frozen=True)
class D2Params:
    pixel_mean: Tuple[float, ...] = PIXEL_MEAN
    pixel_std: Tuple[float, ...] = PIXEL_STD
    anchor_sizes: Tuple[float, ...] = ANCHOR_SIZES
    rpn_batch: int = RPN_BATCH
    rpn_pos_frac: float = RPN_POS_FRAC
    rpn_iou: Tuple[float, float] = (0.3, 0.7)
    rpn_pre: Tuple[int, int] = RPN_PRE
    rpn_post: Tuple[int, int] = RPN_POST
    rpn_nms: float = RPN_NMS
    roi_batch: int = ROI_BATCH
    roi_pos_frac: float = ROI_POS_FRAC
    roi_iou: float = 0.5
    roi_weights: Tuple[float, float, float, float] = ROI_WEIGHTS
    score_thresh: float = SCORE_THRESH
    nms_test: float = NMS_TEST
    dets: int = DETS

    @classmethod
    def from_cfg(cls, cfg) -> "D2Params":
        M = cfg.MODEL

        def get(node, key, default):
            return node.get(key, default) if hasattr(node, "get") else getattr(node, key, default)

        def need(cond, what):
            if not cond:
                raise ValueError(f"aldi_amd R50-FPN engine: unsupported config value: {what}")
        rpn, roi, box, ag = M.RPN, M.ROI_HEADS, get(M, "ROI_BOX_HEAD", {}), M.ANCHOR_GENERATOR
        sizes = [list(s_) for s_ in ag.SIZES]
        need(len(sizes) == 5 and all(len(s_) == 1 for s_ in sizes), f"ANCHOR_GENERATOR.SIZES {sizes} (one size per level p2..p6)")
        ratios = [list(r_) for r_ in ag.ASPECT_RATIOS]
        need(all(tuple(float(v) for v in r_) == ANCHOR_RATIOS for r_ in ratios), f"ANCHOR_GENERATOR.ASPECT_RATIOS {ratios} (kernels: {ANCHOR_RATIOS})")
        need(len(M.PIXEL_MEAN) == 3 and len(M.PIXEL_STD) == 3, "PIXEL_MEAN / PIXEL_STD must have 3 entries")
        need(list(get(rpn, "IN_FEATURES", ["p2", "p3", "p4", "p5", "p6"])) == ["p2", "p3", "p4", "p5", "p6"], "RPN.IN_FEATURES")
        need(list(get(roi, "IN_FEATURES", ["p2", "p3", "p4", "p5"])) == ["p2", "p3", "p4", "p5"], "ROI_HEADS.IN_FEATURES")
        need(tuple(get(rpn, "BBOX_REG_WEIGHTS", (1.0, 1.0, 1.0, 1.0))) == (1.0, 1.0, 1.0, 1.0), "RPN.BBOX_REG_WEIGHTS != (1, 1, 1, 1)")
        need(float(get(rpn, "SMOOTH_L1_BETA", 0.0)) == 0.0 and float(get(box, "SMOOTH_L1_BETA", 0.0)) == 0.0, "SMOOTH_L1_BETA != 0 (the losses are pure L1)")
        need(get(rpn, "BBOX_REG_LOSS_TYPE", "smooth_l1") == "smooth_l1" and get(box, "BBOX_REG_LOSS_TYPE", "smooth_l1") == "smooth_l1", "BBOX_REG_LOSS_TYPE")
        need(float(get(rpn, "LOSS_WEIGHT", 1.0)) == 1.0 and float(get(rpn, "BBOX_REG_LOSS_WEIGHT", 1.0)) == 1.0, "RPN loss weights != 1")
        need(int(get(box, "POOLER_RESOLUTION", POOL)) == POOL and int(get(box, "POOLER_SAMPLING_RATIO", 0)) == 0 and
             get(box, "POOLER_TYPE", "ROIAlignV2") == "ROIAlignV2", "ROI_BOX_HEAD pooler (kernels: ROIAlignV2, 7x7, adaptive sampling)")
        need(not get(box, "CLS_AGNOSTIC_BBOX_REG", False), "CLS_AGNOSTIC_BBOX_REG")
        need(get(roi, "PROPOSAL_APPEND_GT", True), "ROI_HEADS.PROPOSAL_APPEND_GT False")
        need(len(rpn.IOU_THRESHOLDS) == 2 and len(roi.IOU_THRESHOLDS) == 1, "IOU_THRESHOLDS (RPN: two, ROI heads: one)")
        pre = (int(rpn.PRE_NMS_TOPK_TRAIN), int(rpn.PRE_NMS_TOPK_TEST))
        post = (int(rpn.POST_NMS_TOPK_TRAIN), int(rpn.POST_NMS_TOPK_TEST))
        need(max(pre) <= 2048 and min(pre + post) >= 1, f"RPN.PRE_NMS_TOPK {pre} (the NMS workspace holds 2048 boxes per level and image)")
        dets = int(get(get(cfg, "TEST", {}), "DETECTIONS_PER_IMAGE", DETS))
        need(1 <= dets <= GMAX, f"TEST.DETECTIONS_PER_IMAGE {dets} (<= {GMAX}: pseudo-label rows)")
        need(int(rpn.BATCH_SIZE_PER_IMAGE) >= 1 and int(roi.BATCH_SIZE_PER_IMAGE) >= 1, "BATCH_SIZE_PER_IMAGE")
        return cls(pixel_mean=tuple(float(v) for v in M.PIXEL_MEAN), pixel_std=tuple(float(v) for v in M.PIXEL_STD),
                   anchor_sizes=tuple(float(s_[0]) for s_ in sizes), rpn_batch=int(rpn.BATCH_SIZE_PER_IMAGE), rpn_pos_frac=float(rpn.POSITIVE_FRACTION),
                   rpn_iou=(float(rpn.IOU_THRESHOLDS[0]), float(rpn.IOU_THRESHOLDS[1])), rpn_pre=pre, rpn_post=post, rpn_nms=float(rpn.NMS_THRESH),
                   roi_batch=int(roi.BATCH_SIZE_PER_IMAGE), roi_pos_frac=float(roi.POSITIVE_FRACTION), roi_iou=float(roi.IOU_THRESHOLDS[0]),
                   roi_weights=tuple(float(v) for v in get(box, "BBOX_REG_WEIGHTS", ROI_WEIGHTS)), score_thresh=float(roi.SCORE_THRESH_TEST),
                   nms_test=float(roi.NMS_THRESH_TEST), dets=dets)


def raise_on_error(code: int, who: str = "engine"):
    if code & 1:
        raise FloatingPointError(f"{who}: predicted boxes or scores contain Inf/NaN. Training has diverged.")
    if code & 2:
        raise RuntimeError(f"{who}: sparse RPN-head backward: more active pixels than (2 * BATCH_SIZE_PER_IMAGE + 4 * positives) per image; "
                           "the excess was dropped, gradients of this step are wrong -- or, from the detection post-processing: a row of class "
                           "scores contains Inf/NaN; the row was dropped")
    if code & 4:
        raise RuntimeError(f"{who}: detection post-processing: more than 8192 candidates above SCORE_THRESH_TEST in one image; the excess was dropped")
    if code & 8:
        raise RuntimeError(f"{who}: RPN top-k: the group barrier of `topk_fused_kernel` timed out (its workgroups were not co-resident); the candidates "
                           "of this step are wrong.  Set ALDI_RPN_TOPK_FUSED=0 for the five-launch path")
    if code:
        raise RuntimeError(f"{who}: device error word {code}")


class Ctx(dict):
    __getattr__ = dict.__getitem__
    __setattr__ = dict.__setitem__


class RCNN:
    p = D2Params()

    def __init__(self, weights: Weights, num_classes: int, params: Optional[D2Params] = None):
        self.wts = weights
        if params is not None:
            self.p = params
        self.K = num_classes
        self.device, self.dtype = weights.device, weights.dtype
        self.Cp = weights.layout.t["box_pred"].rows
        self.Ch = weights.layout.t["rpn_head_out"].rows
        self._anchor_cache: Dict[tuple, tuple] = {}
        self._ws: Dict[str, torch.Tensor] = {}
        self.err = torch.zeros(1, dtype=torch.int32, device=self.device)
        torch.set_num_threads(1)
        idx = lambda n: int(n.rsplit(".", 1)[1])
        names = list(getattr(weights.layout, "t", {}))
        self.img_da_layers = sorted((n for n in names if n.startswith("img_align.model.")), key=idx)
        self.ins_da_layers = sorted((n for n in names if n.startswith("ins_align.model.")), key=idx)
        self.has_img_da, self.has_ins_da = bool(self.img_da_layers), bool(self.ins_da_layers)
        self.fused_stem = os.environ.get("ALDI_FUSED_STEM", "1") == "1"
        self.wgrad_tail_split = int(os.environ.get("ALDI_WGRAD_TAIL_SPLIT", "2"))
        self.group_wgrad = os.environ.get("ALDI_WGRAD_GROUP", "1") == "1"
        self.mask_bits = os.environ.get("ALDI_MASK_BITS", "1") == "1"
        self.mask_bits_inner = os.environ.get("ALDI_MASK_BITS_INNER", "1") == "1"
        self.level_groups = os.environ.get("ALDI_LEVEL_GROUPS", "1") == "1"
        self.fused_res2 = os.environ.get("ALDI_FUSED_RES2", "1") == "1"
        self.fused_res2_shortcut = os.environ.get("ALDI_FUSED_RES2_SHORTCUT", "1") == "1"
        self._wg_queue: list = []
        self.sparse_rpn_backward = os.environ.get("ALDI_RPN_SPARSE_BWD", "1") == "1"
        spec = getattr(weights.layout, "img_da", None)
        self.img_da_level = ("p2", "p3", "p4", "p5", "p6").index(spec["layer"]) if spec else 0

    def stage_images(self, images: Sequence[torch.Tensor]):
        sizes = [(int(im.shape[1]), int(im.shape[2])) for im in images]
        Hs = pad_to(max(s[0] for s in sizes), 32)
        Ws = pad_to(max(s[1] for s in sizes), 32)
        N = len(images)
        if all(im.is_cuda for im in images):
            st = torch.zeros((N, 3, Hs, Ws), dtype=torch.uint8, device=self.device)
            for i, im in enumerate(images):
                st[i, :, : sizes[i][0], : sizes[i][1]] = im
        else:
            host = torch.zeros((N, 3, Hs, Ws), dtype=torch.uint8).pin_memory()
            for i, im in enumerate(images):
                host[i, :, : sizes[i][0], : sizes[i][1]] = im
            st = host.to(self.device, non_blocking=True)
        hw = torch.tensor(sizes, dtype=torch.int32).to(self.device)
        return st, sizes, hw

    def stage_gt(self, instances: Sequence[dict]):
        N = len(instances)
        gb = torch.zeros((N, GMAX, 4), dtype=torch.float32)
        gc = torch.zeros((N, GMAX), dtype=torch.int32)
        cnt = torch.zeros((N,), dtype=torch.int32)
        on_dev = []
        for i, inst in enumerate(instances):
            b = inst["gt_boxes"]
            b = b.tensor if hasattr(b, "tensor") else b
            g = int(b.shape[0])
            if g > GMAX:
                raise ValueError(f"more than {GMAX} GT boxes in one image")
            if g:
                if b.is_cuda:
                    on_dev.append((i, g, b, inst["gt_classes"]))
                else:
                    gb[i, :g] = b.reshape(-1, 4).to(torch.float32)
                    gc[i, :g] = inst["gt_classes"].to(torch.int32)
            cnt[i] = g
        gbd, gcd, cntd = ops.upload_packed([gb, gc, cnt], self.device)
        for i, g, b, cl in on_dev:
            gbd[i, :g] = b.reshape(-1, 4).to(torch.float32)
            gcd[i, :g] = cl.to(torch.int32)
        return {"boxes": gbd, "classes": gcd, "count": cntd, "host_count": cnt.tolist()}

    def geometry(self, Hs: int, Ws: int):
        key = (Hs, Ws)
        if key not in self._anchor_cache:
            shapes = []
            h, w = Hs // 4, Ws // 4
            for l in range(4):
                shapes.append((h, w))
                if l < 3:
                    h, w = h // 2, w // 2
            shapes.append(((shapes[3][0] - 1) // 2 + 1, (shapes[3][1] - 1) // 2 + 1))
            geom = ops.make_geom(shapes, NUM_ANCHORS, self.Ch)
            anchors = make_anchors(shapes, self.device, getattr(self, "anchor_sizes", self.p.anchor_sizes))
            self._anchor_cache[key] = (shapes, geom, anchors)
            while len(self._anchor_cache) > 16:
                self._anchor_cache.pop(next(iter(self._anchor_cache)))
        else:
            self._anchor_cache[key] = self._anchor_cache.pop(key)
        return self._anchor_cache[key]

    def workspace(self, name: str, nbytes: int) -> torch.Tensor:
        t = self._ws.get(name)
        if t is None or t.numel() < nbytes:
            t = torch.empty(nbytes, dtype=torch.uint8, device=self.device)
            self._ws[name] = t
        return t

    def _conv_call(self, x, name, *, relu=False, res=None, res_mode=0, want_f32=False, out=None, bits_out=None):
        W = self.wts
        p = W.layout.t[name]
        return x, W.w(name), dict(stride=p.stride, pad=p.pad, scale=W.scale(name), shift=W.shift(name), res=res, res_mode=res_mode, relu=relu,
                                  want_f32=want_f32, out=out, bits_out=bits_out)

    def conv(self, x, name, **kw):
        x, w, kw = self._conv_call(x, name, **kw)
        return ops.conv2d(x, w, **kw)

    def _serve(self, req):
        if isinstance(req, list):
            return ops.conv2d_group([self._conv_call(r[0], r[1], **r[2]) for r in req])
        return self.conv(req[0], req[1], **req[2])

    def _drive(self, gen):
        try:
            req = next(gen)
            while True:
                req = gen.send(self._serve(req))
        except StopIteration as e:
            return e.value

    @staticmethod
    def drive_pair(eng_a, gen_a, eng_b, gen_b, streams=None):
        res = [None, None]
        ctx_a = torch.cuda.stream(streams[0]) if streams else contextlib.nullcontext()
        ctx_b = torch.cuda.stream(streams[1]) if streams else contextlib.nullcontext()
        try:
            with ctx_a:
                ra = next(gen_a)
        except StopIteration as e:
            ra, res[0] = None, e.value
        try:
            with ctx_b:
                rb = next(gen_b)
        except StopIteration as e:
            rb, res[1] = None, e.value
        while ra is not None or rb is not None:
            if streams:
                if ra is not None:
                    with ctx_a:
                        ya = eng_a._serve(ra)
                        try:
                            ra = gen_a.send(ya)
                        except StopIteration as e:
                            ra, res[0] = None, e.value
                if rb is not None:
                    with ctx_b:
                        yb = eng_b._serve(rb)
                        try:
                            rb = gen_b.send(yb)
                        except StopIteration as e:
                            rb, res[1] = None, e.value
                continue
            if ra is not None and rb is not None:
                la, lb = (ra if isinstance(ra, list) else [ra]), (rb if isinstance(rb, list) else [rb])
                ys = ops.conv2d_group([eng_a._conv_call(r[0], r[1], **r[2]) for r in la] + [eng_b._conv_call(r[0], r[1], **r[2]) for r in lb])
                ya = ys[:len(la)] if isinstance(ra, list) else ys[0]
                yb = ys[len(la):] if isinstance(rb, list) else ys[len(la)]
            elif ra is not None:
                ya = eng_a._serve(ra)
            else:
                yb = eng_b._serve(rb)
            if ra is not None:
                try:
                    ra = gen_a.send(ya)
                except StopIteration as e:
                    ra, res[0] = None, e.value
            if rb is not None:
                try:
                    rb = gen_b.send(yb)
                except StopIteration as e:
                    rb, res[1] = None, e.value
        return res[0], res[1]

    def trunk(self, st_u8: torch.Tensor, sizes, save: bool) -> Ctx:
        return self._drive(self.trunk_steps(st_u8, sizes, save))

    def prefix_pipelinable(self) -> bool:
        return type(self) is RCNN and self.dtype == torch.bfloat16 and self.fused_stem and self.fused_res2

    def trunk_steps(self, st_u8: torch.Tensor, sizes, save: bool, fpn: bool = True, pre: Optional[torch.Tensor] = None,
                    prefix_out: Optional[torch.Tensor] = None):
        W = self.wts
        c = Ctx()
        bu = "backbone.bottom_up."
        if pre is not None:
            x = pre
        elif self.dtype == torch.bfloat16 and self.fused_stem:
            x = ops.stem_pool_forward(st_u8, sizes, W.stem_packed(bu + "stem.conv1"), W.scale(bu + "stem.conv1"), W.shift(bu + "stem.conv1"),
                                      self.p.pixel_mean, self.p.pixel_std)
        else:
            stem = ops.stem_forward(st_u8, sizes, W.w_master(bu + "stem.conv1"), W.scale(bu + "stem.conv1"), W.shift(bu + "stem.conv1"),
                                    self.p.pixel_mean, self.p.pixel_std, self.dtype)
            x = ops.maxpool3s2(stem)
            del stem
        blocks = []
        cs = []
        out_bits = {}
        fuse2 = self.dtype == torch.bfloat16 and self.fused_res2
        if fuse2:
            res2 = [f"{bu}res2.{b}.conv{k}" for b in range(STAGE_BLOCKS[0]) for k in (1, 2, 3)]
            fw = dict(zip(res2, W.folded(res2)))
        assert prefix_out is None or (fuse2 and pre is None)
        for si, nb in enumerate(STAGE_BLOCKS):
            if si == 0 and pre is not None:
                cs.append(x)
                continue
            for b in range(nb):
                p = f"{bu}res{si + 2}.{b}."
                if si == 0 and fuse2:
                    fold_sc = b == 0 and self.fused_res2_shortcut
                    sc = (yield x, p + "shortcut", {}) if b == 0 and not fold_sc else x
                    x = ops.bottleneck_fused(x, sc, fw[p + "conv1"], fw[p + "conv2"], fw[p + "conv3"], W.shift(p + "conv1"), W.shift(p + "conv2"),
                                             W.shift(p + "conv3"), out=prefix_out if (prefix_out is not None and b == nb - 1) else None,
                                             shortcut=(W.w(p + "shortcut"), W.scale(p + "shortcut"), W.shift(p + "shortcut")) if fold_sc else None)
                    continue
                sc = (yield x, p + "shortcut", {}) if b == 0 else x
                want_bits = save and si > 0 and self.mask_bits and self.dtype == torch.bfloat16

                def bits_for(inp, name):
                    if not want_bits:
                        return None
                    lt = W.layout.t[name]
                    ho = (inp.shape[1] + 2 * lt.pad - lt.kk) // lt.stride + 1
                    wo = (inp.shape[2] + 2 * lt.pad - lt.kk) // lt.stride + 1
                    return torch.empty(inp.shape[0] * ho * wo * (lt.wshape[0] // 8), dtype=torch.uint8, device=self.device)
                b1 = bits_for(x, p + "conv1") if self.mask_bits_inner else None
                h1 = yield x, p + "conv1", dict(relu=True, bits_out=b1)
                b2 = bits_for(h1, p + "conv2") if self.mask_bits_inner else None
                h2 = yield h1, p + "conv2", dict(relu=True, bits_out=b2)
                bits = bits_for(h2, p + "conv3")
                out = yield h2, p + "conv3", dict(relu=True, res=sc, res_mode=1, bits_out=bits)
                if save and si > 0:
                    blocks.append((p, x, h1, h2, out, b == 0))
                    if bits is not None:
                        out_bits[out.data_ptr()] = bits
                        if b1 is not None:
                            out_bits[h1.data_ptr()], out_bits[h2.data_ptr()] = b1, b2
                x = out
            cs.append(x)
            if prefix_out is not None:
                return x
        if not fpn:
            if save:
                c.blocks, c.cs, c.out_bits = blocks, cs, out_bits
            else:
                c.cs = cs
            return c
        prev = {}
        P = {}
        prev[5] = yield cs[3], "backbone.fpn_lateral5", {}
        if self.level_groups:
            for lvl in (4, 3, 2):
                prev[lvl] = yield cs[lvl - 2], f"backbone.fpn_lateral{lvl}", dict(res=prev[lvl + 1], res_mode=2)
            outs = yield [(prev[lvl], f"backbone.fpn_output{lvl}", {}) for lvl in (2, 3, 4, 5)]
            P.update(zip((2, 3, 4, 5), outs))
        else:
            P[5] = yield prev[5], "backbone.fpn_output5", {}
            for lvl in (4, 3, 2):
                prev[lvl] = yield cs[lvl - 2], f"backbone.fpn_lateral{lvl}", dict(res=prev[lvl + 1], res_mode=2)
                P[lvl] = yield prev[lvl], f"backbone.fpn_output{lvl}", {}
        P[6] = ops.subsample2(P[5])
        c.P = [P[2], P[3], P[4], P[5], P[6]]
        if save:
            c.blocks, c.cs, c.prev, c.out_bits = blocks, cs, prev, out_bits
        return c

    def rpn_head(self, c: Ctx, save: bool):
        self._drive(self.rpn_head_steps(c, save))

    def rpn_head_steps(self, c: Ctx, save: bool):
        px = [f.shape[0] * f.shape[1] * f.shape[2] for f in c.P]
        flat = torch.empty((1, sum(px), 1, FPN_C), dtype=self.dtype, device=self.device)
        ts, o, reqs = [], 0, []
        for f, n in zip(c.P, px):
            view = flat[0, o:o + n, 0].view(f.shape[0], f.shape[1], f.shape[2], FPN_C)
            reqs.append((f, "proposal_generator.rpn_head.conv", dict(relu=True, out=view)))
            o += n
        if self.level_groups:
            ts = yield reqs
        else:
            for r in reqs:
                ts.append((yield r))
        hf = yield flat, "rpn_head_out", dict(want_f32=True)
        heads, o = [], 0
        for f, n in zip(c.P, px):
            heads.append(hf[0, o:o + n, 0].view(f.shape[0], f.shape[1], f.shape[2], hf.shape[3]))
            o += n
        c.head, c.head_flat = heads, hf
        if save:
            c.rpn_t = ts

    def box_head(self, pooled: torch.Tensor, c: Optional[Ctx] = None):
        R = pooled.shape[0]
        x = pooled.view(R, 1, 1, POOL * POOL * FPN_C)
        fc1 = self.conv(x, "roi_heads.box_head.fc1", relu=True)
        bits2 = None
        if c is not None and self.mask_bits and self.dtype == torch.bfloat16 and R > 0 and os.environ.get("ALDI_MASK_BITS_FC", "1") == "1":
            bits2 = torch.empty(R * (FC_DIM // 8), dtype=torch.uint8, device=self.device)
        fc2 = self.conv(fc1, "roi_heads.box_head.fc2", relu=True, bits_out=bits2)
        pred = self.conv(fc2, "box_pred", want_f32=True).view(R, self.Cp)
        if c is not None:
            c.pooled, c.fc1, c.fc2 = pooled, fc1, fc2
            if bits2 is not None:
                if c.get("out_bits") is None:
                    c.out_bits = {}
                c.out_bits[fc2.data_ptr()] = bits2
        return pred, fc2

    def roi_feats(self, c: Ctx, grads=None):
        return ops.make_roi_feats(c.P[:4], grads, [1.0 / s for s in STRIDES[:4]])

    def _sample_host(self, counts: List[List[int]], batch: int, frac: float):
        N = len(counts)
        S = batch
        sel = torch.zeros((N, 2, S), dtype=torch.int32)
        nsel = torch.zeros((N, 2), dtype=torch.int32)
        for n, (npos, nneg) in enumerate(counts):
            num_pos = min(npos, int(batch * frac))
            num_neg = min(nneg, batch - num_pos)
            perm1 = randperm_prefix(npos, num_pos)
            perm2 = randperm_prefix(nneg, num_neg)
            sel[n, 0, :num_pos] = perm1.to(torch.int32)
            sel[n, 1, :num_neg] = perm2.to(torch.int32)
            nsel[n, 0], nsel[n, 1] = num_pos, num_neg
        return sel, nsel, nsel.tolist()

    def _sample(self, counts: List[List[int]], batch: int, frac: float):
        sel, nsel, h = self._sample_host(counts, batch, frac)
        sel_d, nsel_d = ops.upload_packed([sel, nsel], self.device)
        return sel_d, nsel_d, h

    def rpn_match(self, geom, anchors, gt, N):
        sumA = anchors.shape[0]
        dev = self.device
        best_iou = torch.empty((N, sumA), dtype=torch.float32, device=dev)
        best_idx = torch.empty((N, sumA), dtype=torch.int32, device=dev)
        labels = torch.empty((N, sumA), dtype=torch.int32, device=dev)
        scratch = ops.box_match_scratch(N, GMAX, dev)
        ops.box_match(anchors, 0, None, sumA, gt["boxes"], gt["count"], GMAX, N, self.p.rpn_iou[0], self.p.rpn_iou[1], True, best_iou, best_idx, scratch, labels)
        lists = torch.empty((N, 2, sumA), dtype=torch.int32, device=dev)
        counts = torch.empty((N, 2), dtype=torch.int32, device=dev)
        ops.compact_labels(labels, sumA, N, 0, lists, counts)
        return labels, best_idx, lists, counts

    def rpn_sample(self, lists, counts, N, host_counts=None):
        if host_counts is None:
            both = torch.cat([counts.view(-1), self.err.view(-1)]).cpu().tolist()
            raise_on_error(both[-1])
            host_counts = [both[2 * i: 2 * i + 2] for i in range(N)]
        lists = lists.contiguous()
        sel, nsel, nsel_h = self._sample(host_counts, self.p.rpn_batch, self.p.rpn_pos_frac)
        L_ = lists.shape[2]
        labels = torch.empty((N, L_), dtype=torch.int32, device=self.device)
        ops.rpn_apply_sample(labels, L_, N, lists, sel, nsel, self.p.rpn_batch)
        n_fg = sum(a for a, _ in nsel_h)
        n_valid = sum(a + b for a, b in nsel_h)
        return labels, n_valid, n_fg, host_counts

    def proposals(self, c: Ctx, geom, anchors, hw, N, training: bool):
        nl = 5
        ws = self.workspace("rpn", ops.rpn_proposals_workspace(N, nl))
        post = self.p.rpn_post[0 if training else 1]
        boxes = torch.empty((N, post, 4), dtype=torch.float32, device=self.device)
        scores = torch.empty((N, post), dtype=torch.float32, device=self.device)
        count = torch.empty((N,), dtype=torch.int32, device=self.device)
        ops.rpn_proposals(geom, c.head, anchors, hw, N, self.p.rpn_pre[0 if training else 1], post, self.p.rpn_nms, ws, boxes, scores, count, self.err)
        return boxes, scores, count

    def forward_train(self, images, instances, *, roi_seed: Optional[int] = None, pre_roi_hook=None,
                      gt_dev: Optional[dict] = None, do_align: bool = False, labeled: bool = True,
                      da_weights: Tuple[float, float] = (0.0, 0.0)) -> Ctx:
        N = len(images)
        st, sizes, hw = self.stage_images(images)
        shapes, geom, anchors = self.geometry(st.shape[2], st.shape[3])
        gt = gt_dev if gt_dev is not None else self.stage_gt(instances)
        c = self.trunk(st, sizes, save=True)
        c.N, c.sizes, c.hw, c.geom, c.anchors, c.gt, c.shapes = N, sizes, hw, geom, anchors, gt, shapes
        self.rpn_head(c, save=True)
        dev = self.device
        _, matched, lists, counts = self.rpn_match(geom, anchors, gt, N)
        labels, _, _, c.rpn_host_counts = self.rpn_sample(lists, counts, N)
        c.rpn_labels, c.rpn_matched, c.rpn_lists, c.rpn_counts = labels, matched, lists, counts
        c.loss_rpn = torch.zeros(2, dtype=torch.float32, device=dev)
        ops.rpn_loss(geom, c.head, None, anchors, labels, matched, gt["boxes"], gt["count"], GMAX, N, 1.0 / (self.p.rpn_batch * N), 0.0, 0.0, c.loss_rpn)
# ... 339 lines not shown
        else:
            scratch = torch.empty((N, GMAX), dtype=torch.int32, device=dev)
            ops.roi_prepare(props, prop_count, P, gt["boxes"], gt["classes"], gt["count"], GMAX, N, self.K, self.p.roi_iou, cand, ccount, best_iou, best_idx,
                            scratch, labels, cls)
            ops.compact_labels(cls, Lc, N, self.K, lists, counts)
        return dict(cand=cand, cls=cls, best_idx=best_idx, lists=lists, counts=counts, Lc=Lc, counts_tail=cbuf)

    def _roi_gather(self, c: Ctx, prep: dict, sel, nsel, nsel_h, gt, N, row_off_dev=None):
        dev = self.device
        rows = [a + b for a, b in nsel_h]
        row_off = [0]
        for r in rows[:-1]:
            row_off.append(row_off[-1] + r)
        R = sum(rows)
        c.R, c.rows = R, rows
        c.rois = torch.empty((max(R, 1), 5), dtype=torch.float32, device=dev)
        c.r_cls = torch.empty((max(R, 1),), dtype=torch.int32, device=dev)
        c.r_gt = torch.empty((max(R, 1), 4), dtype=torch.float32, device=dev)
        c.r_idx = torch.empty((max(R, 1),), dtype=torch.int32, device=dev)
        if row_off_dev is None:
            row_off_dev = torch.tensor(row_off, dtype=torch.int32).to(dev)
        ops.roi_gather(prep["cand"], prep["cls"], prep["best_idx"], prep["Lc"], prep["lists"], sel, nsel, self.p.roi_batch,
                       row_off_dev, gt["boxes"], gt["count"], GMAX, N, c.rois, c.r_cls, c.r_gt, c.r_idx)

    def roi_sample(self, c: Ctx, props, prop_count, gt, N):
        prep = self._roi_prepare(props, prop_count, gt, N)
        host_counts = prep["counts"].cpu().tolist()
        c.roi_host_counts = host_counts
        sel, nsel, nsel_h = self._sample(host_counts, self.p.roi_batch, self.p.roi_pos_frac)
        self._roi_gather(c, prep, sel, nsel, nsel_h, gt, N)

    def roi_forward(self, c: Ctx):
        R = c.R
        pooled = torch.empty((R, POOL, POOL, FPN_C), dtype=self.dtype, device=self.device)
        ops.roialign(self.roi_feats(c), c.rois, R, POOL, pooled, backward=False)
        c.pred, _ = self.box_head(pooled, c)

    def box_head_on(self, c_feats: Ctx, rois: torch.Tensor, R: int):
        pooled = torch.empty((R, POOL, POOL, FPN_C), dtype=self.dtype, device=self.device)
        ops.roialign(self.roi_feats(c_feats), rois, R, POOL, pooled, backward=False)
        pred, fc2 = self.box_head(pooled)
        return pred

    def inference(self, images, pl_thresh: float, keep_ctx: bool = True, staged=None, pl_out=None) -> Ctx:
        st, sizes, hw = staged if staged is not None else self.stage_images(images)
        c = self.trunk(st, sizes, save=False)
        self.rpn_head(c, save=False)
        return self.inference_heads(c, st, sizes, hw, pl_thresh, pl_out=pl_out)

    def inference_heads(self, c: Ctx, st, sizes, hw, pl_thresh: float, pl_out=None) -> Ctx:
        N = st.shape[0]
        shapes, geom, anchors = self.geometry(st.shape[2], st.shape[3])
        c.N, c.sizes, c.hw, c.geom, c.anchors, c.shapes = N, sizes, hw, geom, anchors, shapes
        props, pscores, pcount = self.proposals(c, geom, anchors, hw, N, training=False)
        P = props.shape[1]
        rois = torch.empty((N * P, 5), dtype=torch.float32, device=self.device)
        ops.rois_from_proposals(props, pcount, P, N, rois)
        pooled = torch.empty((N * P, POOL, POOL, FPN_C), dtype=self.dtype, device=self.device)
        ops.roialign(self.roi_feats(c), rois, N * P, POOL, pooled, backward=False)
        pred, _ = self.box_head(pooled)
        dev = self.device
        ws = self.workspace("det", ops.detections_workspace(N))
        d = Ctx()
        d.boxes = torch.empty((N, self.p.dets, 4), dtype=torch.float32, device=dev)
        d.scores = torch.empty((N, self.p.dets), dtype=torch.float32, device=dev)
        d.classes = torch.empty((N, self.p.dets), dtype=torch.int32, device=dev)
        d.count = torch.empty((N,), dtype=torch.int32, device=dev)
        if pl_out is not None:
            pl_boxes, pl_cls, pl_count = pl_out
        else:
            pl_boxes = torch.empty((N, GMAX, 4), dtype=torch.float32, device=dev)
            pl_cls = torch.empty((N, GMAX), dtype=torch.int32, device=dev)
            pl_count = torch.empty((N,), dtype=torch.int32, device=dev)
        pl_scores = torch.empty((N, GMAX), dtype=torch.float32, device=dev)
        ops.detections(pred, self.Cp, self.K, props, pcount, P, N, hw, self.p.roi_weights, self.p.score_thresh, self.p.nms_test, self.p.dets, pl_thresh, ws,
                       d.boxes, d.scores, d.classes, d.count, pl_boxes, pl_cls, pl_scores, pl_count, self.err)
        c.det = d
        c.pseudo = {"boxes": pl_boxes, "classes": pl_cls, "count": pl_count, "scores": pl_scores}
        c.props, c.prop_count, c.pred_all = props, pcount, pred
        return c

    def feature_pass(self, images, pooling: str = "avg"):
        if type(self) is not RCNN:
            raise ValueError(f"feature_pass: only the R50-FPN engine is supported, not {type(self).__name__}")
        st, sizes, hw = self.stage_images(images)
        c = self.trunk(st, sizes, save=False)
        self.rpn_head(c, save=False)
        N = st.shape[0]
        shapes, geom, anchors = self.geometry(st.shape[2], st.shape[3])
        props, _, pcount = self.proposals(c, geom, anchors, hw, N, training=False)
        P = props.shape[1]
        rois = torch.empty((N * P, 5), dtype=torch.float32, device=self.device)
        ops.rois_from_proposals(props, pcount, P, N, rois)
        pooled = torch.empty((N * P, POOL, POOL, FPN_C), dtype=self.dtype, device=self.device)
        ops.roialign(self.roi_feats(c), rois, N * P, POOL, pooled, backward=False)
        p6 = c.P[4]
        img = torch.empty((N, FPN_C), dtype=torch.float32, device=self.device)
        ops.pool_rows(p6.view(N, p6.shape[1] * p6.shape[2], FPN_C), img, pooling)
        prop = torch.empty((N * P, FPN_C), dtype=torch.float32, device=self.device)
        total = torch.empty((1,), dtype=torch.int32, device=self.device)
        ops.pool_rows_counted(pooled.view(N, P, POOL * POOL, FPN_C), pcount, prop, total, pooling)
        return img, prop, total

    def backward(self, c: Ctx, scales: Dict[str, float]):
        W = self.wts
        T = self.dtype
        dev = self.device
        sc = lambda k: float(scales.get(k, 0.0))
        scratch = torch.zeros(2, dtype=torch.float32, device=dev)
        c.ghead = [torch.zeros_like(h) for h in c.head]
        c.gpred = torch.zeros((max(c.R, 1), self.Cp), dtype=torch.float32, device=dev)
        gt = c.gt
        ops.rpn_loss(c.geom, c.head, c.ghead, c.anchors, c.rpn_labels, c.rpn_matched, gt["boxes"], gt["count"], GMAX, c.N,
                     1.0 / (self.p.rpn_batch * c.N), sc("loss_rpn_cls"), sc("loss_rpn_loc"), scratch)
        ops.box_loss(c.pred, self.Cp, self.K, c.R, c.rois, c.r_cls, c.r_gt, self.p.roi_weights, sc("loss_cls"), sc("loss_box_reg"), c.gpred, scratch)
        if c.distill is not None:
            d = c.distill
            def rpn_d(do_obj, do_reg, s_):
                ops.rpn_distill_loss(c.geom, c.head, d["t_head"], c.ghead, d["labels"], c.N, d["obj_T"], d["n_valid"], d["n_fg"],
                                     do_obj, do_reg, s_, scratch)

            def roi_d(do_cls, do_reg, s_):
                ops.roih_distill_loss(c.pred, d["t_pred"], self.Cp, self.K, c.R, d["cls_T"], d["kl"], do_cls, do_reg, s_, c.gpred, scratch)
            if sc("loss_obj_bce") == sc("loss_rpn_l1"):
                rpn_d(d["do_obj"], d["do_rpn_reg"], sc("loss_obj_bce"))
            else:
                rpn_d(d["do_obj"], False, sc("loss_obj_bce"))
                rpn_d(False, d["do_rpn_reg"], sc("loss_rpn_l1"))
            if sc("loss_cls_ce") == sc("loss_roih_l1"):
                roi_d(d["do_cls"], d["do_roih_reg"], sc("loss_cls_ce"))
            else:
                roi_d(d["do_cls"], False, sc("loss_cls_ce"))
                roi_d(False, d["do_roih_reg"], sc("loss_roih_l1"))
        label = 1.0 if c.labeled else 0.0
        if "img" in c.align:
            acts, pooled, logit = c.align["img"]
            glog = torch.empty(logit.shape, dtype=T, device=dev)
            ops.domain_bce(logit, logit.shape[-1], c.N, label, c.da_weights[0], sc("loss_da_img"), glog, scratch)
            c.align["img"] = (acts, pooled, glog)
        if "ins" in c.align:
            acts, logit = c.align["ins"]
            glog = torch.empty(logit.shape, dtype=T, device=dev)
            ops.domain_bce(logit, logit.shape[-1], c.R, label, c.da_weights[1], sc("loss_da_ins"), glog, scratch)
            c.align["ins"] = (acts, glog)
        al = dict(n0=0, n1=c.N, r0=0, r1=c.R, **c.align)
        self._backward_trunk(c, [al] if c.align else [])

    def _backward_trunk(self, c: Ctx, align_list: List[dict]):
        W = self.wts
        T = self.dtype
        dev = self.device
        gx_pre, gx_ev = {}, None
        side0 = self._wgrad_stream()
        if side0 is not None and "cs" in c:
            side0.wait_stream(torch.cuda.current_stream())
            with torch.cuda.stream(side0):
                for si_, ci_ in ((3, 2), (2, 1)):
                    gx_pre[si_] = torch.zeros_like(c.cs[ci_])
                gx_ev = torch.cuda.Event()
                gx_ev.record(side0)
        sp_pre, aux = None, None
        if self.sparse_rpn_backward:
            aux = self._aux_stream()
            if aux is not None:
                aux.wait_stream(torch.cuda.current_stream())
                with torch.cuda.stream(aux):
                    sp_pre = self._rpn_sparse_prepare(c)
        g_dt = T if (self.sparse_rpn_backward and T == torch.bfloat16) else torch.float32
        gP_roi = [(torch.empty if c.R > 0 else torch.zeros)(f.shape, dtype=g_dt, device=dev) for f in c.P[:4]]
        if c.R > 0:
            g_extra = None
            for al in align_list:
                if "ins" not in al:
                    continue
                acts, g_ = al["ins"]
                r0, r1 = al["r0"], al["r1"]
                if g_extra is None:
                    g_extra = torch.zeros((c.R, 1, 1, FC_DIM), dtype=T, device=dev)
                L_ = self.ins_da_layers
                for i in range(len(L_) - 1, -1, -1):
                    self._wgrad(L_[i], acts[i], g_)
                    if i == 0:
                        ops.conv2d(g_, W.wt(L_[0], negate=True), out=g_extra[r0:r1])
                    else:
                        g_ = ops.conv2d(g_, W.wt(L_[i]), mask=acts[i])
            lo = c.get("gpred_lo")
            gpred = (lo if lo is not None else ops.cast_from_f32(c.gpred[:c.R], T)).view(c.R, 1, 1, self.Cp)
            self._wgrad("box_pred", c.fc2, gpred)
            g_fc2 = ops.conv2d(gpred, W.wt("box_pred"), res=g_extra, res_mode=1 if g_extra is not None else 0, **self._relu_mask(c, c.fc2))
            self._wgrad("roi_heads.box_head.fc2", c.fc1, g_fc2)
            g_fc1 = ops.conv2d(g_fc2, W.wt("roi_heads.box_head.fc2"), mask=c.fc1)
            x = c.pooled.view(c.R, 1, 1, POOL * POOL * FPN_C)
            self._wgrad("roi_heads.box_head.fc1", x, g_fc1)
            g_pooled = ops.conv2d(g_fc1, W.wt("roi_heads.box_head.fc1")).view(c.R, POOL, POOL, FPN_C)
            ops.roialign_backward(self.roi_feats(c, gP_roi), c.rois, c.R, POOL, g_pooled, c.N, rois_sorted=True, grad_dtype=g_dt)
        self._grads_final(["box_pred", "roi_heads.box_head.fc2", "roi_heads.box_head.fc1"])
        if self.sparse_rpn_backward:
            if sp_pre is not None:
                main_ = torch.cuda.current_stream()
                main_.wait_stream(aux)
                for t_ in sp_pre.values():
                    if isinstance(t_, torch.Tensor):
                        t_.record_stream(main_)
                gP = self._rpn_sparse_finish(c, gP_roi, sp_pre)
            else:
                gP = self._rpn_head_backward_sparse(c, gP_roi)
        else:
            gP = []
            for l in range(5):
                gh = ops.cast_from_f32(c.ghead[l], T)
                self._wgrad("rpn_head_out", c.rpn_t[l], gh)
                g_t = ops.conv2d(gh, W.wt("rpn_head_out"), mask=c.rpn_t[l])
                self._wgrad("proposal_generator.rpn_head.conv", c.P[l], g_t)
                gP.append(ops.conv2d(g_t, W.wt("proposal_generator.rpn_head.conv"), pad=1))
            for l in range(4):
                ops.add_f32(gP[l], gP_roi[l], gP[l])
        for al in align_list:
            if "img" not in al:
                continue
            acts, pooled, glog = al["img"]
            n0, n1 = al["n0"], al["n1"]
            L_ = self.img_da_layers
            lvl = self.img_da_level
            self._wgrad(L_[-1], pooled, glog)
            g_pooled = ops.conv2d(glog, W.wt(L_[-1], negate=len(L_) == 1))
            if len(L_) == 1:
                hw = acts[0].shape[1] * acts[0].shape[2]
                gP[lvl][n0:n1] += (g_pooled.float() / hw).to(T)
                continue
            g_ = ops.avgpool_bwd(g_pooled, acts[-1])
            for i in range(len(L_) - 2, -1, -1):
                self._wgrad(L_[i], acts[i], g_)
                if i == 0:
                    ops.conv2d(g_, W.wt(L_[0], negate=True), pad=2, res=gP[lvl][n0:n1], res_mode=1, out=gP[lvl][n0:n1])
                else:
                    g_ = ops.conv2d(g_, W.wt(L_[i]), pad=2, mask=acts[i])
        ops.subsample2_bwd(gP[4], gP[3])
        gprev = {}
        for i, lvl in enumerate((2, 3, 4, 5)):
            self._wgrad(f"backbone.fpn_output{lvl}", c.prev[lvl], gP[i])
        if self.level_groups:
            gs = ops.conv2d_group([(gP[i], W.wt(f"backbone.fpn_output{lvl}"), dict(pad=1)) for i, lvl in enumerate((2, 3, 4, 5))])
            gprev.update(zip((2, 3, 4, 5), gs))
        else:
            for i, lvl in enumerate((2, 3, 4, 5)):
                gprev[lvl] = ops.conv2d(gP[i], W.wt(f"backbone.fpn_output{lvl}"), pad=1)
        sh = [tuple(gprev[lvl].shape) for lvl in (2, 3, 4, 5)]
        if (all(sh[i][1] == 2 * sh[i + 1][1] and sh[i][2] == 2 * sh[i + 1][2] for i in range(3)) and all(gprev[lvl].is_contiguous() for lvl in (2, 3, 4, 5))
                and os.environ.get("ALDI_UPSAMPLE_CHAIN", "1") == "1"):
            ops.upsample2_bwd_chain(gprev[2], gprev[3], gprev[4], gprev[5])
        else:
            for lvl in (3, 4, 5):
                ops.upsample2_bwd(gprev[lvl - 1], gprev[lvl], accumulate=True)
        for lvl in (2, 3, 4, 5):
            self._wgrad(f"backbone.fpn_lateral{lvl}", c.cs[lvl - 2], gprev[lvl])
        self._grads_final(["rpn_head_out", "proposal_generator.rpn_head.conv"] + [f"backbone.fpn_output{l}" for l in (2, 3, 4, 5)] +
                          [f"backbone.fpn_lateral{l}" for l in (2, 3, 4, 5)])
        g = ops.conv2d(gprev[5], W.wt("backbone.fpn_lateral5"), **self._relu_mask(c, c.cs[3]))
        blocks = c.blocks
        bi = len(blocks) - 1
        for si in (3, 2, 1):
            stage_names: List[str] = []
            for b in range(STAGE_BLOCKS[si] - 1, -1, -1):
                p, xin, h1, h2, out, first = blocks[bi]
                bi -= 1
                stage_names += [p + "conv3", p + "conv2", p + "conv1"] + ([p + "shortcut"] if first else [])
                self._wgrad(p + "conv3", h2, g)
                g2 = ops.conv2d(g, W.wt(p + "conv3"), **self._relu_mask(c, h2))
                self._wgrad(p + "conv2", h1, g2)
                g1 = ops.conv2d(g2, W.wt(p + "conv2"), pad=1, **self._relu_mask(c, h1))
                self._wgrad(p + "conv1", xin, g1)
                if si == 1 and not first and self.wgrad_tail_split > 0 and (STAGE_BLOCKS[si] - b) % self.wgrad_tail_split == 0:
                    self._flush_wgrads()
                if first:
                    self._wgrad(p + "shortcut", xin, g)
                    self._grads_final(stage_names)
                    if si == 1:
                        break
                    stride = W.layout.t[p + "conv1"].stride
                    Hin, Win = xin.shape[1], xin.shape[2]
                    gx = gx_pre.pop(si, None)
                    if gx is None or gx.shape != xin.shape:
                        gx = torch.zeros_like(xin)
                    else:
                        torch.cuda.current_stream().wait_event(gx_ev)
                        gx.record_stream(torch.cuda.current_stream())
                    ops.conv2d(g, W.wt(p + "shortcut"), out=gx, out_scale=stride, out_hw=(Hin, Win))
                    ops.conv2d(g1, W.wt(p + "conv1"), out=gx, out_scale=stride, out_hw=(Hin, Win), res=gx, res_mode=1)
                    lvl = si + 1
                    g = ops.conv2d(gprev[lvl], W.wt(f"backbone.fpn_lateral{lvl}"), res=gx, res_mode=1, **self._relu_mask(c, xin))
                else:
                    g = ops.conv2d(g1, W.wt(p + "conv1"), res=g, res_mode=1, **self._relu_mask(c, xin))
        self._join_wgrads()

    def trunk_backward(self, c: Ctx, gC: Dict[int, Optional[torch.Tensor]]):
        W = self.wts
        assert self.dtype == torch.float32, "the bare-trunk backward runs in the fp32 mode (the DETR path's AMP is off)"
        def masked(a, b, act):
            if a is None and b is None:
                return None
            x, y = (a, b) if b is not None else (None, a)
            return ops.add_f32(x, y, torch.empty_like(act), relu_src=act)
        blocks = c.blocks
        bi = len(blocks) - 1
        g = masked(gC.get(5), None, c.cs[3])
        for si in (3, 2, 1):
            stage_names: List[str] = []
            for b in range(STAGE_BLOCKS[si] - 1, -1, -1):
                p, xin, h1, h2, out, first = blocks[bi]
                bi -= 1
                stage_names += [p + "conv3", p + "conv2", p + "conv1"] + ([p + "shortcut"] if first else [])
                self._wgrad(p + "conv3", h2, g)
                g2 = ops.conv2d(g, W.wt(p + "conv3"), mask=h2)
                self._wgrad(p + "conv2", h1, g2)
                g1 = ops.conv2d(g2, W.wt(p + "conv2"), pad=1, mask=h1)
                self._wgrad(p + "conv1", xin, g1)
                if first:
                    self._wgrad(p + "shortcut", xin, g)
                    self._grads_final(stage_names)
                    if si == 1:
                        break
                    stride = W.layout.t[p + "conv1"].stride
                    Hin, Win = xin.shape[1], xin.shape[2]
                    gx = torch.zeros_like(xin)
                    ops.conv2d(g, W.wt(p + "shortcut"), out=gx, out_scale=stride, out_hw=(Hin, Win))
                    ops.conv2d(g1, W.wt(p + "conv1"), out=gx, out_scale=stride, out_hw=(Hin, Win), res=gx, res_mode=1)
                    g = masked(gC.get(si + 1), gx, xin)
                else:
                    g = ops.conv2d(g1, W.wt(p + "conv1"), res=g, res_mode=1, mask=xin)
        self._join_wgrads()

    @staticmethod
    def _relu_mask(c: Ctx, act: torch.Tensor) -> dict:
        bits = (c.get("out_bits") or {}).get(act.data_ptr())
        return dict(mask_bits=bits) if bits is not None else dict(mask=act)

    def _rpn_sparse_prepare(self, c: Ctx):
        W, T, dev = self.wts, self.dtype, self.device
        N, Cf, Ch = c.N, FPN_C, self.Ch
        cap = (2 * self.p.rpn_batch + 4 * int(self.p.rpn_batch * self.p.rpn_pos_frac)) * N
        idx = torch.empty(cap, dtype=torch.int32, device=dev)
        count = torch.empty(1, dtype=torch.int32, device=dev)
        ws = torch.empty(ops.rpn_active_pixels_workspace(c.geom, N), dtype=torch.uint8, device=dev)
        ops.rpn_active_pixels(c.geom, c.ghead, N, cap, idx, count, ws, self.err)
        G = torch.empty((cap, 1, 1, Ch), dtype=T, device=dev)
        Tm = torch.empty((cap, 1, 1, Cf), dtype=T, device=dev)
        X9 = torch.empty((cap, 1, 1, 9 * Cf), dtype=T, device=dev)
        ops.rpn_sparse_gather(c.geom, c.ghead, c.rpn_t, c.P, N, Cf, cap, idx, count, G, Tm, X9)
        g_t = ops.conv2d(G, W.wt("rpn_head_out"), mask=Tm)
        Y = ops.conv2d(g_t, W.wt_flat("proposal_generator.rpn_head.conv"))
        return dict(cap=cap, idx=idx, count=count, G=G, Tm=Tm, X9=X9, g_t=g_t, Y=Y)

    def _rpn_sparse_finish(self, c: Ctx, gP_roi: List[torch.Tensor], sp: dict) -> List[torch.Tensor]:
        T, dev = self.dtype, self.device
        self._wgrad("rpn_head_out", sp["Tm"], sp["G"], temp_x=True)
        self._wgrad("proposal_generator.rpn_head.conv", sp["X9"], sp["g_t"], flat=True, temp_x=True)
        g32 = list(gP_roi) + [torch.zeros(c.P[4].shape, dtype=gP_roi[0].dtype, device=dev)]
        ops.rpn_sparse_scatter(c.geom, g32, sp["Y"], c.N, FPN_C, sp["cap"], sp["idx"], sp["count"])
        return g32 if g32[0].dtype == T else [ops.cast_from_f32(g, T) for g in g32]

    def _rpn_head_backward_sparse(self, c: Ctx, gP_roi: List[torch.Tensor]) -> List[torch.Tensor]:
        return self._rpn_sparse_finish(c, gP_roi, self._rpn_sparse_prepare(c))

    def _aux_stream(self):
        if not hasattr(self, "_aux_side"):
            self._aux_side = torch.cuda.Stream(device=self.device) if os.environ.get("ALDI_AUX_STREAM", "1") == "1" and torch.device(self.device).type == "cuda" else None
        return self._aux_side

    def _grads_final(self, names: List[str]):
        self._flush_wgrads()
        cb = getattr(self, "grad_ready", None)
        if cb is None:
            return
        evs = []
        side = getattr(self, "_wg_side", None)
        if side is not None and self._wgrad_pending:
            ev = torch.cuda.Event()
            ev.record(side)
            evs.append(ev)
        ev = torch.cuda.Event()
        ev.record()
        evs.append(ev)
        if len(inspect.signature(cb).parameters) >= 2:
            cb(self.wts.layout.ranges(names), evs)
        else:
            self._join_wgrads()
            cb(self.wts.layout.ranges(names))

    def _wgrad(self, name: str, x: torch.Tensor, g: torch.Tensor, flat: bool = False, temp_x: bool = False):
        W = self.wts
        p = W.layout.t[name]
        geo = dict(KH=1, KW=1, stride=1, pad=0) if flat else dict(KH=p.kk, KW=p.kk, stride=p.stride, pad=p.pad)
        geo["scale"] = W.scale(name)
        if (not flat and p.kk == 1 and p.stride == 2 and p.pad == 0 and self.dtype == torch.bfloat16 and getattr(self, "group_wgrad", False)
                and os.environ.get("ALDI_WGRAD_SUBSAMPLE", "1") == "1"):
            cache = self.__dict__.setdefault("_sub_cache", {})
            hit = cache.get(id(x))
            if hit is None or hit[0] is not x:
                side_ = self._wgrad_stream()
                if side_ is not None and os.environ.get("ALDI_WGRAD_SUBSAMPLE_SIDE", "1") == "1":
                    ev_ = torch.cuda.Event()
                    ev_.record()
                    side_.wait_event(ev_)
                    with torch.cuda.stream(side_):
                        hit = (x, ops.subsample2(x))
                else:
                    hit = (x, ops.subsample2(x))
                cache.clear()
                cache[id(x)] = hit
            x, temp_x = hit[1], True
            geo.update(stride=1)
        if getattr(self, "group_wgrad", False) and self.dtype == torch.bfloat16:
            fused_bias = p.bias and os.environ.get("ALDI_WGRAD_BIAS_FUSED", "1") == "1"
            if fused_bias:
                geo["db"] = W.gb(name)
            self._wg_queue.append((x, g, W.gw(name), geo, W.gb(name) if p.bias and not fused_bias else None, temp_x))
            return
        side = self._wgrad_stream()
        if p.bias:
            geo["db"] = W.gb(name)
        if side is None:
            ops.conv_wgrad(x, g, W.gw(name), **geo)
            return
        ev = torch.cuda.Event()
        ev.record()
        side.wait_event(ev)
        g.record_stream(side)
        if temp_x:
            x.record_stream(side)
        with torch.cuda.stream(side):
            ops.conv_wgrad(x, g, W.gw(name), **geo)
        self._wgrad_pending = True

    def _flush_wgrads(self):
        q = getattr(self, "_wg_queue", None)
        if not q:
            return
        self._wg_queue = []
        side = self._wgrad_stream()

        def launch():
            ops.conv_wgrad_group([(x, g, dw, geo) for x, g, dw, geo, _, _ in q])
            for _, g, _, _, gb, _ in q:
                if gb is not None:
                    ops.bias_grad(g, gb)
        if side is None:
# ... 26 lines not shown
```

### aldi_amd/ops.py

```python
from __future__ import annotations

import ctypes as C
import os
from typing import List, Optional, Sequence

import torch

from . import _lib as L


def dtype_code(t: torch.dtype) -> int:
    if t == torch.float32:
        return L.F32
    if t == torch.bfloat16:
        return L.BF16
    raise TypeError(f"unsupported dtype {t}")


def _p(t: Optional[torch.Tensor]):
    return None if t is None else t.data_ptr()


_RAW_STREAM = getattr(torch._C, "_cuda_getCurrentRawStream", None)


def stream_ptr() -> int:
    if _RAW_STREAM is not None:
        return _RAW_STREAM(torch.cuda.current_device())
    return torch.cuda.current_stream().cuda_stream


def upload_packed(tensors, device):
    metas, off = [], 0
    for t in tensors:
        nb = t.numel() * t.element_size()
        metas.append((off, nb))
        off += (nb + 15) // 16 * 16
    host = torch.empty(max(off, 16), dtype=torch.uint8).pin_memory()
    for t, (o, nb) in zip(tensors, metas):
        if nb:
            host[o:o + nb] = t.contiguous().view(-1).view(torch.uint8)
    dev = host.to(device, non_blocking=True)
    return [dev[o:o + nb].view(t.dtype).view(t.shape) for t, (o, nb) in zip(tensors, metas)]


def conv2d(x: torch.Tensor, w: torch.Tensor, *, stride: int = 1, pad: int = 0,
           scale: Optional[torch.Tensor] = None, shift: Optional[torch.Tensor] = None,
           res: Optional[torch.Tensor] = None, res_mode: int = 0, relu: bool = False,
           mask: Optional[torch.Tensor] = None, out: Optional[torch.Tensor] = None,
           out_f32: Optional[torch.Tensor] = None, want_f32: bool = False,
           out_scale: int = 1, out_hw=None, ksplit: Optional[int] = None, mask_bits: Optional[torch.Tensor] = None,
           bits_out: Optional[torch.Tensor] = None) -> torch.Tensor:
    N, H, W_, Cin = x.shape
    Cout, KH, KW, Cin2 = w.shape
    assert Cin == Cin2 and x.is_contiguous() and w.is_contiguous() and x.dtype == w.dtype, (x.shape, w.shape, x.dtype, w.dtype)
    Ho = (H + 2 * pad - KH) // stride + 1
    Wo = (W_ + 2 * pad - KW) // stride + 1
    if out_scale > 1:
        OH, OW = out_hw
        shape = (N, OH, OW, Cout)
    else:
        OH = OW = 0
        shape = (N, Ho, Wo, Cout)
    if out is None and not want_f32:
        out = torch.empty(shape, dtype=x.dtype, device=x.device)
    if want_f32 and out_f32 is None:
        out_f32 = torch.empty(shape, dtype=torch.float32, device=x.device)
    ws = None
    if ksplit is None:
        ksplit = _auto_ksplit(x, N * Ho * Wo, Cout, KH * KW * Cin, KH * KW == 1 and stride == 1 and pad == 0 and res is None and mask is None
                              and not want_f32 and out_f32 is None and out_scale == 1 and mask_bits is None and bits_out is None)
    if ksplit and ksplit > 1:
        ws = torch.empty(ksplit * N * Ho * Wo * Cout, dtype=torch.float32, device=x.device)
    a = L.ConvArgs(_p(x), _p(w), _p(out), _p(out_f32), _p(scale), _p(shift), _p(res), _p(mask),
                   N, H, W_, Cin, Cout, KH, KW, stride, pad, Ho, Wo,
                   int(relu), res_mode, out_scale, OH, OW, dtype_code(x.dtype), _p(ws), int(ksplit or 0), _p(mask_bits), _p(bits_out))
    L.call("aldi_conv_igemm", C.byref(a), stream_ptr())
    return out_f32 if want_f32 and out is None else out


def _auto_ksplit(x, M, Cout, K, plain: bool) -> int:
    if not plain or x.dtype != torch.bfloat16 or K < 4096 or K % 256 or os.environ.get("ALDI_SPLITK", "1") != "1":
        return 0
    tiles = ((M + 127) // 128) * ((Cout + 127) // 128)
    if not (16 <= tiles <= 160) or Cout % 4:
        return 0
    tiles256 = ((M + 255) // 256) * ((Cout + 127) // 128)
    for ks in (2, 4, 7, 8, 14, 16):
        if K % (64 * ks) == 0 and tiles256 * ks >= 216:
            return ks
    return 4 if K % 256 == 0 else 0


def _conv_args(x, w, *, stride=1, pad=0, scale=None, shift=None, res=None, res_mode=0, relu=False, mask=None, out=None, out_f32=None,
               want_f32=False, out_scale=1, out_hw=None, mask_bits=None, bits_out=None):
    N, H, W_, Cin = x.shape
    Cout, KH, KW, Cin2 = w.shape
    assert Cin == Cin2 and x.is_contiguous() and w.is_contiguous() and x.dtype == w.dtype, (x.shape, w.shape, x.dtype, w.dtype)
    Ho = (H + 2 * pad - KH) // stride + 1
    Wo = (W_ + 2 * pad - KW) // stride + 1
    if out_scale > 1:
        OH, OW = out_hw
        shape = (N, OH, OW, Cout)
    else:
        OH = OW = 0
        shape = (N, Ho, Wo, Cout)
    if out is None and not want_f32:
        out = torch.empty(shape, dtype=x.dtype, device=x.device)
    if want_f32 and out_f32 is None:
        out_f32 = torch.empty(shape, dtype=torch.float32, device=x.device)
    a = L.ConvArgs(_p(x), _p(w), _p(out), _p(out_f32), _p(scale), _p(shift), _p(res), _p(mask),
                   N, H, W_, Cin, Cout, KH, KW, stride, pad, Ho, Wo,
                   int(relu), res_mode, out_scale, OH, OW, dtype_code(x.dtype), None, 0, _p(mask_bits), _p(bits_out))
    return a, (out_f32 if want_f32 and out is None else out)


def conv2d_group(calls) -> List[torch.Tensor]:
    arr = (L.ConvArgs * len(calls))()
    outs = []
    for i, (x, w, kw) in enumerate(calls):
        arr[i], y = _conv_args(x, w, **kw)
        outs.append(y)
    L.call("aldi_conv_igemm_group", arr, len(calls), stream_ptr())
    return outs


_WGRAD_WS = {}
WGRAD_WS_EPOCH = 0
WGRAD_ORDERED = os.environ.get("ALDI_WGRAD_ORDERED", "1") != "0"


def _wgrad_workspace(arr, n: int, device) -> None:
    if not WGRAD_ORDERED:
        return
    need = L.lib.aldi_conv_wgrad_group_workspace(arr, n)
    if need < 0:
        raise RuntimeError("aldi_conv_wgrad_group_workspace: " + L.lib.aldi_last_error().decode())
    if need == 0:
        need = 256
    key = (device, stream_ptr())
    buf = _WGRAD_WS.get(key)
    if buf is None or buf.numel() * 4 < need:
        global WGRAD_WS_EPOCH
        if buf is not None:
            WGRAD_WS_EPOCH += 1
            if torch.cuda.is_current_stream_capturing():
                raise RuntimeError("the weight-gradient workspace has to grow during a hipGraph capture: run the new shapes eagerly once first")
        else:
            need = max([need] + [b.numel() * 4 for (d_, _), b in _WGRAD_WS.items() if d_ == device])
        buf = torch.empty((need + (need >> 2) + 3) // 4, dtype=torch.float32, device=device)
        _WGRAD_WS[key] = buf
    arr[0].ws = buf.data_ptr()
    arr[0].ws_bytes = buf.numel() * 4


def conv_wgrad(x: torch.Tensor, g: torch.Tensor, dw: torch.Tensor, *, KH: int, KW: int, stride: int = 1, pad: int = 0,
               scale: Optional[torch.Tensor] = None, db: Optional[torch.Tensor] = None) -> None:
    N, H, W_, Cin = x.shape
    _, Ho, Wo, Cout = g.shape
    assert dw.dtype == torch.float32 and dw.numel() == Cout * KH * KW * Cin and x.dtype == g.dtype, (dw.shape, x.shape, g.shape)
    arr = (L.WgradArgs * 1)()
    arr[0] = L.WgradArgs(_p(x), _p(g), _p(dw), _p(scale), N, H, W_, Cin, Cout, KH, KW, stride, pad, Ho, Wo, dtype_code(x.dtype), _p(db), None, 0)
    if x.dtype == torch.bfloat16:
        _wgrad_workspace(arr, 1, x.device)
    L.call("aldi_conv_wgrad", arr, stream_ptr())


def conv_wgrad_group(problems) -> None:
    arr = (L.WgradArgs * len(problems))()
    for i, (x, g, dw, kw) in enumerate(problems):
        N, H, W_, Cin = x.shape
        _, Ho, Wo, Cout = g.shape
        KH, KW = kw["KH"], kw["KW"]
        assert dw.dtype == torch.float32 and dw.numel() == Cout * KH * KW * Cin and x.dtype == g.dtype, (dw.shape, x.shape, g.shape)
        arr[i] = L.WgradArgs(_p(x), _p(g), _p(dw), _p(kw.get("scale")), N, H, W_, Cin, Cout, KH, KW, kw.get("stride", 1), kw.get("pad", 0), Ho, Wo,
                             dtype_code(x.dtype), _p(kw.get("db")), None, 0)
    _wgrad_workspace(arr, len(problems), problems[0][0].device)
    L.call("aldi_conv_wgrad_group", arr, len(problems), stream_ptr())


def noop() -> None:
    L.call("aldi_noop", stream_ptr())


def bias_grad(g: torch.Tensor, db: torch.Tensor) -> None:
    Cc = g.shape[-1]
    L.call("aldi_bias_grad", _p(g), _p(db), g.numel() // Cc, Cc, dtype_code(g.dtype), stream_ptr())


def dgrad_weights(w_master: torch.Tensor, scale: Optional[torch.Tensor], dtype: torch.dtype,
                  out: Optional[torch.Tensor] = None) -> torch.Tensor:
    Cout, KH, KW, Cin = w_master.shape
    if out is None:
        out = torch.empty((Cin, KH, KW, Cout), dtype=dtype, device=w_master.device)
    L.call("aldi_dgrad_weights", _p(w_master), _p(scale), _p(out), Cout, KH, KW, Cin, dtype_code(dtype), stream_ptr())
    return out


class DgradWeightsPlan:

    def __init__(self, entries, dtype: torch.dtype):
        dev = entries[0][0].device
        self.dtype = dtype
        self.keep = list(entries)
        sizes = [w.numel() for w, _ in entries]
        offs, tot = [], 0
        for n in sizes:
            offs.append(tot)
            tot += (n + 63) // 64 * 64
        self.buf = torch.empty(tot, dtype=dtype, device=dev)
        self.out = []
        items = (L.DgwItem * len(entries))()
        tile = 0
        for i, (w, sc) in enumerate(entries):
            Cout, KH, KW, Cin = w.shape
            o = self.buf[offs[i]:offs[i] + sizes[i]].view(Cin, KH, KW, Cout)
            self.out.append(o)
            it = items[i]
            it.w_master, it.scale, it.wt = w.data_ptr(), (sc.data_ptr() if sc is not None else None), o.data_ptr()
            it.Cout, it.KH, it.KW, it.Cin, it.tile_begin, it.reserved = Cout, KH, KW, Cin, tile, 0
            tile += KH * KW * ((Cout + 31) // 32) * ((Cin + 31) // 32)
        self.total_tiles = tile
        self.n = len(entries)
        raw = torch.frombuffer(bytearray(bytes(items)), dtype=torch.uint8)
        self.items = raw.to(dev)

    def run(self):
        L.call("aldi_dgrad_weights_batch", _p(self.items), self.n, self.total_tiles, dtype_code(self.dtype), stream_ptr())

# ... 384 lines not shown
```

### include/aldi_hip.h

```cpp
#ifndef ALDI_HIP_H
#define ALDI_HIP_H
#include <stddef.h>
#include <stdint.h>

#ifdef __cplusplus
extern "C" {
#endif

typedef void* aldi_stream_t;

enum { ALDI_F32 = 0, ALDI_BF16 = 1 };
enum { ALDI_OK = 0, ALDI_ERR_HIP = -1, ALDI_ERR_ARG = -2 };

const char* aldi_last_error(void);
int aldi_version(void);
int aldi_noop(aldi_stream_t stream);

int aldi_set_tuning(const char* name, int value);
int aldi_get_tuning(const char* name, int* value);
int aldi_reset_tuning(void);
const char* aldi_last_dispatch(void);

typedef struct {
    const void* x;
    const void* w;
    void* y;
    float* y_f32;
    const float* scale;
    const float* shift;
    const void* res;
    const void* mask;
    int N, H, W, Cin;
    int Cout, KH, KW, stride, pad;
    int Ho, Wo;
    int relu;
    int res_mode;
    int out_scale;
    int OH, OW;
    int dtype;
    void* ws;
    int ksplit;
    const void* mask_bits;
    void* bits_out;
} aldi_conv_args;

int aldi_conv_igemm(const aldi_conv_args* a, aldi_stream_t stream);
int aldi_conv_igemm_group(const aldi_conv_args* args, int n, aldi_stream_t stream);
int aldi_conv_igemm_plan(const aldi_conv_args* args, int n, char* name, int cap);

typedef struct {
    const void* x;
    const void* g;
    float* dw;
    const float* scale;
    int N, H, W, Cin, Cout, KH, KW, stride, pad, Ho, Wo;
    int dtype;
    float* db;
    void* ws;
    long ws_bytes;
} aldi_wgrad_args;
int aldi_conv_wgrad(const aldi_wgrad_args* a, aldi_stream_t stream);

int aldi_conv_wgrad_group(const aldi_wgrad_args* args, int n, aldi_stream_t stream);
long aldi_conv_wgrad_group_workspace(const aldi_wgrad_args* args, int n);
int aldi_conv_wgrad_plan(const aldi_wgrad_args* args, int n, int group, char* name, int cap, long* ws_bytes);

int aldi_bias_grad(const void* g, float* db, int M, int C, int dtype, aldi_stream_t stream);

int aldi_dgrad_weights(const float* w_master, const float* scale, void* wt, int Cout, int KH, int KW, int Cin,
                       int dtype, aldi_stream_t stream);

typedef struct aldi_dgw_item {
    const float* w_master;
    const float* scale;
    void* wt;
    int Cout, KH, KW, Cin;
    int tile_begin, reserved;
} aldi_dgw_item;
int aldi_dgrad_weights_batch(const aldi_dgw_item* items, int n_items, int total_tiles, int dtype, aldi_stream_t stream);

typedef struct aldi_bottleneck_args {
    const void* x;
    const void* res;
    void* y;
    const void* w1; const void* w2; const void* w3;
    const float* b1; const float* b2; const float* b3;
    int N, H, W, Cin, mid, Cout;
} aldi_bottleneck_args;
int aldi_bottleneck_fused(const aldi_bottleneck_args* a, aldi_stream_t stream);
int aldi_bottleneck_fused_sc(const aldi_bottleneck_args* a, const void* wsc, const float* sc_scale, const float* sc_shift, aldi_stream_t stream);
typedef struct aldi_fold_item {
    const float* w; const float* scale; void* out;
    int rows, cols, chunk_begin, reserved;
} aldi_fold_item;
int aldi_fold_weights_batch(const aldi_fold_item* items, int n_items, int total_chunks, aldi_stream_t stream);

#define ALDI_MAX_IMAGES 16

typedef struct {
    const uint8_t* img;
    const float* w;
    const float* scale; const float* shift;
    void* y;
    int N, Hs, Ws, Hc, Wc;
    int h[ALDI_MAX_IMAGES], w_img[ALDI_MAX_IMAGES];
    float mean[3], std[3];
    int dtype;
} aldi_stem_args;
int aldi_stem_forward(const aldi_stem_args* a, aldi_stream_t stream);
int aldi_stem_pack_weights(const float* w, void* w_packed, aldi_stream_t stream);
int aldi_stem_pool_forward(const aldi_stem_args* a, const void* w_packed, void* y_pool, aldi_stream_t stream);

int aldi_maxpool3s2(const void* x, void* y, int N, int H, int W, int C, int dtype, aldi_stream_t stream);
int aldi_stage_images(const void* const* images, const int* heights, const int* widths, int n, int C, int Hs, int Ws, void* batch,
                      aldi_stream_t stream);
int aldi_subsample2(const void* x, void* y, int N, int H, int W, int C, int backward, int dtype, aldi_stream_t stream);
int aldi_upsample2_bwd(const void* g, void* out, int N, int Hc, int Wc, int C, int accumulate, int dtype, aldi_stream_t stream);
int aldi_upsample2_bwd_chain(const void* g2, void* o3, void* o4, void* o5, int N, int H5, int W5, int C, int dtype, aldi_stream_t stream);
int aldi_add_f32(const void* a, const float* b, const void* relu_src, void* out, long n, int dtype, aldi_stream_t stream);
int aldi_cast_from_f32(const float* src, void* dst, long n, int dtype, aldi_stream_t stream);

int aldi_sgd_step(float* p, const float* g, float* buf, void* p_compute, long n, float lr, float momentum, float weight_decay,
                  float grad_scale, int first_step, int dtype, aldi_stream_t stream);
int aldi_sgd_step_dev(float* p, const float* g, float* buf, void* p_compute, long n, const float* hyper, int dtype, aldi_stream_t stream);
int aldi_ema_update(float* teacher, const float* student, void* teacher_compute, long n, long n_compute, double alpha, int copy_only, int dtype,
                    aldi_stream_t stream);
int aldi_bn_fold(const float* w, const float* b, const float* mean, const float* var, float* scale, float* shift, int C, aldi_stream_t stream);

#define ALDI_MAX_LEVELS 5
typedef struct {
    int num_levels;
    int A;
    int C;
    int H[ALDI_MAX_LEVELS], W[ALDI_MAX_LEVELS];
    int off[ALDI_MAX_LEVELS + 1];
} aldi_rpn_geom;

int aldi_box_match(const float* boxes, long box_stride_n, const int* box_count, int L,
                   const float* gt_boxes, const int* gt_count, int Gmax, int N,
                   float lo, float hi, int allow_low_quality,
                   float* best_iou, int* best_idx, unsigned* gt_best_scratch, size_t gt_best_bytes, int* labels, aldi_stream_t stream);
size_t aldi_compact_labels_workspace(int L, int N);
int aldi_compact_labels(const int* labels, int L, int N, int bg_label, int* lists, int* counts, void* workspace, aldi_stream_t stream);
int aldi_rpn_apply_sample(int* labels, int L, int N, const int* lists, const int* sel, const int* nsel, int S, aldi_stream_t stream);
int aldi_rpn_loss(const aldi_rpn_geom* gm, float* const* head, float* const* grad, const float* anchors, const int* labels, const int* matched,
                  const float* gt_boxes, const int* gt_count, int Gmax, int N, float inv_norm, float grad_scale_cls, float grad_scale_loc,
                  float* loss2, aldi_stream_t stream);
size_t aldi_rpn_proposals_workspace(int N, int num_levels);
int aldi_rpn_proposals(const aldi_rpn_geom* gm, float* const* head, const float* anchors, const int* img_hw, int N,
                       int pre_nms_topk, int post_nms_topk, float nms_thresh, void* workspace,
                       float* out_boxes, float* out_scores, int* out_count, int* err_flag, aldi_stream_t stream);

size_t aldi_rpn_active_pixels_workspace(const aldi_rpn_geom* gm, int N);
int aldi_rpn_active_pixels(const aldi_rpn_geom* gm, float* const* grad_head, int N, int cap, int* idx, int* count, void* workspace,
                           int* err_flag, aldi_stream_t stream);
int aldi_rpn_sparse_gather(const aldi_rpn_geom* gm, float* const* grad_head, const void* const* hidden, const void* const* feat, int N, int Cf,
                           int cap, const int* idx, const int* count, void* G, void* Tm, void* X9, int dtype, aldi_stream_t stream);
int aldi_rpn_sparse_scatter(const aldi_rpn_geom* gm, void* const* gfeat, const void* Y, int N, int Cf, int cap, const int* idx,
                            const int* count, int dtype, int grad_dtype, aldi_stream_t stream);

typedef struct {
    const void* feat[4];
    float* grad[4];
    int H[4], W[4];
    float scale[4];
    int C;
} aldi_roi_feats;

int aldi_roi_prepare(const float* props, const int* pcount, int P, const float* gt_boxes, const int* gt_classes, const int* gt_count,
                     int Gmax, int N, int K, float iou_thresh, float* cand, int* ccount, float* best_iou, int* best_idx,
                     unsigned* gt_best_scratch, int* labels, int* cls, aldi_stream_t stream);
int aldi_roi_prepare_lists(const float* props, const int* pcount, int P, const float* gt_boxes, const int* gt_classes, const int* gt_count,
                           int Gmax, int N, int K, float iou_thresh, float* cand, int* ccount, float* best_iou, int* best_idx, int* labels,
                           int* cls, int* lists, int* counts, unsigned* tickets, const int* tail_a, const int* tail_b, aldi_stream_t stream);
int aldi_roi_gather(const float* cand, const int* cls, const int* best_idx, int L, const int* lists, const int* sel, const int* nsel, int S,
                    const int* row_off, const float* gt_boxes, const int* gt_count, int Gmax, int N,
                    float* rois, int* r_cls, float* r_gt, int* r_idx, aldi_stream_t stream);
int aldi_rois_from_proposals(const float* props, const int* pcount, int P, int N, float* rois, aldi_stream_t stream);
int aldi_roialign(const aldi_roi_feats* f, const float* rois, int R, int P, void* pooled, int backward, int dtype, aldi_stream_t stream);
int aldi_roialign_backward(const aldi_roi_feats* f, const float* rois, int R, int P, const void* g_pooled, int N, int rois_sorted, int dtype,
                           int grad_dtype, aldi_stream_t stream);

int aldi_box_loss(const float* pred, int Cp, int K, int R, const float* rois, const int* cls, const float* gt_boxes,
                  const float* weights4, float grad_scale_cls, float grad_scale_box, float* grad, float* loss2, aldi_stream_t stream);
typedef struct {
    int r0, r1;
    float grad_scale_cls, grad_scale_box;
    float* loss_box;
    const float* teacher_pred;
    float cls_temperature;
    int kl, do_cls, do_reg;
    float grad_scale_distill_cls, grad_scale_distill_reg;
    float* loss_distill;
} aldi_box_loss_chunk;
int aldi_box_losses_fused(const float* pred, int Cp, int K, const float* rois, const int* cls, const float* gt_boxes, const float* weights4,
                          const aldi_box_loss_chunk* chunks, int nchunks, float* grad, void* grad_lo, aldi_stream_t stream);
size_t aldi_detections_workspace(int N);
int aldi_detections(const float* pred, int Cp, int K, const float* props, const int* pcount, int P, int N, const int* img_hw,
                    const float* weights4, float score_thresh, float nms_thresh, int topk, float pl_thresh, void* workspace,
                    float* det_boxes, float* det_scores, int* det_cls, int* det_count,
                    float* pl_boxes, int* pl_cls, float* pl_scores, int* pl_count, int pl_rows, int* err_flag, aldi_stream_t stream);
// ... 163 lines not shown
```

Baseline: 511.0.

## Fuse stage-entrance shortcut conv into conv3 GEMM and fold backward input grad

Adds a paired implicit-GEMM kernel that computes the 1x1 strided shortcut conv first, applies its BN scale/shift, keeps the result in registers as the residual, then runs conv3 and adds it in the epilogue. The shortcut output tensor no longer has to be written and re-read. In backward, the strided shortcut and conv1 input-grad convolutions are fused into one pair GEMM at reduced resolution. A new res_mode=3 then upsamples the residual by scattering into the lateral-conv epilogue, which replaces the zero-filled full-resolution buffer and the side-stream precompute. Risks include a different bf16 rounding point for the residual and lower parallelism from the 128x64 tile.

```diff
diff --git a/aldi_amd/_lib.py b/aldi_amd/_lib.py
--- a/aldi_amd/_lib.py
+++ b/aldi_amd/_lib.py
@@ -87,6 +87,12 @@
     return buf.value.decode()
 
 
+def plan_pair_dispatch(args, pre) -> str:
+    buf = C.create_string_buffer(224)
+    call("aldi_conv_pair_igemm_plan", C.byref(args), C.byref(pre), buf, len(buf))
+    return buf.value.decode()
+
+
 def plan_wgrad_dispatch(args, n: int = 1, group: bool = False):
     buf = C.create_string_buffer(224)
     ws = C.c_long(0)
@@ -110,6 +116,11 @@
         ("relu", c_int), ("res_mode", c_int), ("out_scale", c_int), ("OH", c_int), ("OW", c_int),
         ("dtype", c_int), ("ws", c_void_p), ("ksplit", c_int), ("mask_bits", c_void_p), ("bits_out", c_void_p),
     ]
+
+
+class ConvPreArgs(C.Structure):
+    _fields_ = [("x2", c_void_p), ("w2", c_void_p), ("scale2", c_void_p), ("shift2", c_void_p),
+                ("H2", c_int), ("W2", c_int), ("Cin2", c_int), ("stride2", c_int), ("rounding", c_int)]
 
 
 class WgradArgs(C.Structure):
diff --git a/aldi_amd/csrc/igemm.hip b/aldi_amd/csrc/igemm.hip
--- a/aldi_amd/csrc/igemm.hip
+++ b/aldi_amd/csrc/igemm.hip
@@ -51,7 +51,8 @@
             const int rowl0 = tid / CPR, ch8 = tid % CPR;
             const int c = n0 + ch8 * 8;
             if (c >= p.Cout) return;
-            const bool plain = p.out_scale == 1 && p.res_mode != 2;
+            const bool plain = p.out_scale == 1 && p.res_mode < 2;
+            const int up = p.res_mode & 1;
             const unsigned char* rd = stg + rowl0 * ROWB + ch8 * 16;
             typedef short s16x2_t __attribute__((ext_vector_type(2)));
             constexpr int NI = BM / RPI;
@@ -63,6 +64,7 @@
                 const int m = m0 + rowl0 + it * RPI;
                 const bool ok = m < p.M;
                 unsigned oidx, ridx;
+                bool rok = ok;
                 if (plain) {
                     oidx = (unsigned)m * (unsigned)p.Cout;
                     ridx = oidx;
@@ -73,11 +75,13 @@
                     const int ho = r / p.Wo, wo = r - ho * p.Wo;
                     if (p.out_scale == 1) oidx = (unsigned)mm * (unsigned)p.Cout;
                     else oidx = (unsigned)((((long)n * p.OH + ho * p.out_scale) * p.OW + wo * p.out_scale) * p.Cout);
-                    if (p.res_mode == 2) ridx = (unsigned)((((long)n * (p.Ho >> 1) + (ho >> 1)) * (p.Wo >> 1) + (wo >> 1)) * p.Cout);
-                    else ridx = oidx;
+                    if (p.res_mode >= 2) {
+                        ridx = (unsigned)((((long)n * ((p.Ho + up) >> 1) + (ho >> 1)) * ((p.Wo + up) >> 1) + (wo >> 1)) * p.Cout);
+                        rok = ok && !(up & (ho | wo));
+                    } else ridx = oidx;
                 }
                 ooff[it] = ok ? (oidx + (unsigned)c) * 2u : OOBX;
-                roff[it] = ok ? (ridx + (unsigned)c) * 2u : OOBX;
+                roff[it] = rok ? (ridx + (unsigned)c) * 2u : OOBX;
                 boff[it] = ok ? (oidx + (unsigned)c) >> 3 : OOBX;
             }
             u32x4_t rres[NI], rmsk[NI];
@@ -161,7 +165,8 @@
         int m = m0 + wm * (BM / WM) + i * 16 + fr;
         if (m >= p.M) continue;
         long oidx, ridx = 0;
-        if (p.out_scale == 1 && p.res_mode != 2) {
+        bool rok = true;
+        if (p.out_scale == 1 && p.res_mode < 2) {
             oidx = (long)m * p.Cout;
             ridx = oidx;
         } else {
@@ -170,8 +175,11 @@
             int ho = r / p.Wo, wo = r - ho * p.Wo;
             if (p.out_scale == 1) oidx = (long)m * p.Cout;
             else oidx = (((long)n * p.OH + ho * p.out_scale) * p.OW + wo * p.out_scale) * p.Cout;
-            if (p.res_mode == 2) ridx = (((long)n * (p.Ho >> 1) + (ho >> 1)) * (p.Wo >> 1) + (wo >> 1)) * p.Cout;
-            else ridx = oidx;
+            const int up = p.res_mode & 1;
+            if (p.res_mode >= 2) {
+                ridx = (((long)n * ((p.Ho + up) >> 1) + (ho >> 1)) * ((p.Wo + up) >> 1) + (wo >> 1)) * p.Cout;
+                rok = !(up & (ho | wo));
+            } else ridx = oidx;
         }
 #pragma unroll
         for (int j = 0; j < TN; ++j) {
@@ -187,8 +195,8 @@
                 v[0] += sh.x; v[1] += sh.y; v[2] += sh.z; v[3] += sh.w;
             }
             if (p.res_mode) {
-                float r4[4];
-                load4(R + ridx + c, r4);
+                float r4[4] = {0.f, 0.f, 0.f, 0.f};
+                if (rok) load4(R + ridx + c, r4);
                 v[0] += r4[0]; v[1] += r4[1]; v[2] += r4[2]; v[3] += r4[3];
             }
             if (p.relu) {
@@ -226,7 +234,7 @@
     asm volatile("ds_read_u8 %0, %1" : "=v"(v) : "v"(addr));
     return v;
 }
-template <int BM, int BN, int WM, int WN, bool RESL>
+template <int BM, int BN, int WM, int WN, bool RESL, bool TWO = false>
 __device__ __forceinline__ void igemm_epilogue_direct(const ConvDev& p, f32x4_t (&acc)[BM / WM / 16][BN / WN / 16], const int m0, const int n0,
                                                       u32x4_t (&rres)[BM / WM / 16][BN / WN / 32], const unsigned aux_addr) {
     constexpr int TM = BM / WM / 16, TN = BN / WN / 16, WNE = BN / WN, H = WNE / 32;
@@ -286,6 +294,16 @@
             if (has_sh) {
 #pragma unroll
                 for (int e = 0; e < 4; ++e) { v[e] += __uint_as_float(sh[2 * h][e]); v[4 + e] += __uint_as_float(sh[2 * h + 1][e]); }
+            }
+            if constexpr (RESL && TWO) {
+                if (has_res) {
+#pragma unroll
+                    for (int q = 0; q < 4; ++q) {
+                        const unsigned r2 = pack2_bf16(v[2 * q], v[2 * q + 1]);
+                        v[2 * q] = __uint_as_float(r2 << 16);
+                        v[2 * q + 1] = __uint_as_float(r2 & 0xffff0000u);
+                    }
+                }
             }
             if constexpr (RESL) {
                 if (has_res) {
@@ -379,15 +397,17 @@
                 for (int i = 0; i < BM / WM / 16; ++i) {
                     const int m = m0 + wm * (BM / WM) + i * 16 + (lane & 15);
                     unsigned ridx = (unsigned)m;
-                    if (p.res_mode == 2) {
-                        const int mm = m < p.M ? m : 0;
+                    bool rok = true;
+                    if (p.res_mode >= 2) {
+                        const int mm = m < p.M ? m : 0, up = p.res_mode & 1;
                         const int n = mm / (p.Ho * p.Wo), r = mm - n * (p.Ho * p.Wo), ho = r / p.Wo, wo = r - ho * p.Wo;
-                        ridx = (unsigned)((n * (p.Ho >> 1) + (ho >> 1)) * (p.Wo >> 1) + (wo >> 1));
+                        ridx = (unsigned)((n * ((p.Ho + up) >> 1) + (ho >> 1)) * ((p.Wo + up) >> 1) + (wo >> 1));
+                        rok = !(up & (ho | wo));
                     }
 #pragma unroll
                     for (int h = 0; h < BN / WN / 32; ++h) {
                         const int ch = n0 + wn * (BN / WN) + h * 32 + (lane >> 4) * 8;
-                        const bool ok = p.res_mode && m < p.M && ch < p.Cout;
+                        const bool ok = p.res_mode && rok && m < p.M && ch < p.Cout;
                         rres[i][h] = __builtin_amdgcn_raw_buffer_load_b128(rr, ok ? (ridx * (unsigned)p.Cout + (unsigned)ch) * 2u : OOB, 0, 0);
                     }
                 }
@@ -897,6 +917,7 @@
 
 #include "igemm_halo64.h"
 #include "igemm_ws.h"
+#include "igemm_pair.h"
 
 template <int BM, int NT, bool HALO> constexpr int min_waves_per_simd() { return HALO && BM == 240 ? 2 * NT / 256 : 1; }
 template <typename T, int BM, int BN, int WM, int WN, int KC, bool PIPE, bool HALO = false, int EPI = 0, bool LEAN = false>
@@ -1051,6 +1072,18 @@
     return ALDI_OK;
 }
 
+int conv_pair(const aldi_conv_args* a, const aldi_conv_pre_args* pre, const bool dry, hipStream_t st, char* name) {
+    ConvDev d;
+    PairPre q;
+    bool two = false;
+    if (int rc = plan_conv_pair(a, pre, aldi_tuning(), d, q, two)) return rc;
+    pair_dispatch_name(two, name, kNameCap);
+    if (dry) return ALDI_OK;
+    if (int rc = launch_pair(two, d, q, st)) return rc;
+    aldi_note_dispatch(name);
+    return ALDI_OK;
+}
+
 int conv_many(const aldi_conv_args* args, const int n, const bool dry, hipStream_t st, char* name) {
     if (!args || n < 1) return aldi_set_error_msg(ALDI_ERR_ARG, "conv_igemm_group: no problems");
     if (n == 1 || !conv_group_same(args, n, aldi_tuning())) {
@@ -1080,6 +1113,18 @@
     return conv_many(args, n, false, static_cast<hipStream_t>(stream), name);
 }
 
+extern "C" int aldi_conv_pair_igemm(const aldi_conv_args* a, const aldi_conv_pre_args* pre, aldi_stream_t stream) {
+    char name[kNameCap];
+    return conv_pair(a, pre, false, static_cast<hipStream_t>(stream), name);
+}
+
+extern "C" int aldi_conv_pair_igemm_plan(const aldi_conv_args* a, const aldi_conv_pre_args* pre, char* name, int cap) {
+    char buf[kNameCap] = "";
+    const int rc = conv_pair(a, pre, true, nullptr, buf);
+    if (rc == ALDI_OK && name && cap > 0) snprintf(name, (size_t)cap, "%s", buf);
+    return rc;
+}
+
 extern "C" int aldi_conv_igemm_plan(const aldi_conv_args* args, int n, char* name, int cap) {
     char buf[kNameCap] = "";
     const int rc = n == 1 ? conv_one(args, true, nullptr, buf) : conv_many(args, n, true, nullptr, buf);
diff --git a/aldi_amd/csrc/igemm_pair.h b/aldi_amd/csrc/igemm_pair.h
--- /dev/null
+++ b/aldi_amd/csrc/igemm_pair.h
@@ -0,0 +1,186 @@
+#pragma once
+
+template <bool TWO>
+__global__ __launch_bounds__(256, 4) void igemm_pair_kernel(ConvDev p, PairPre q) {
+    typedef bf16_t T;
+    constexpr int BM = 128, BN = 64, WM = 4, WN = 1, KC = 4, NT = 256, EP = 8, BK = KC * EP;
+    constexpr int A_IT = BM * KC / NT, TM = BM / WM / 16, TN = BN / WN / 16, H = TN / 2;
+    static_assert(BN * KC == NT && A_IT == 2, "one weight chunk and two pixel chunks per thread and slab");
+    constexpr int NBUF = 3, SLOTS = (BM + BN) * KC;
+    constexpr int AUX_SLOTS = 64, AUX2_SLOTS = 32;
+    __shared__ __attribute__((aligned(128))) uint4 lds_all[NBUF * SLOTS + AUX_SLOTS + AUX2_SLOTS];
+    uint4 (*const lds)[SLOTS] = reinterpret_cast<uint4 (*)[SLOTS]>(&lds_all[0]);
+    uint4* const aux_lds = &lds_all[NBUF * SLOTS];
+    uint4* const aux2_lds = &lds_all[NBUF * SLOTS + AUX_SLOTS];
+
+    const int tid = threadIdx.x, lane = tid & 63, wave = tid >> 6;
+    const int wm = wave;
+    const int nmt = (int)gridDim.x, nnt = (int)gridDim.y;
+    int bid = (int)(blockIdx.y * gridDim.x + blockIdx.x);
+    if (p.xcd) {
+        const int total = nmt * nnt, qq = total >> 3, r = total & 7, xcd = bid & 7, idx = bid >> 3;
+        bid = (xcd < r ? xcd * (qq + 1) : r * (qq + 1) + (xcd - r) * qq) + idx;
+    }
+    const int m0 = (bid / nnt) * BM, n0 = (bid % nnt) * BN;
+    const __amdgpu_buffer_rsrc_t rx = __builtin_amdgcn_make_buffer_rsrc(const_cast<void*>(p.x), 0, p.x_bytes, 0x00020000);
+    const __amdgpu_buffer_rsrc_t rw = __builtin_amdgcn_make_buffer_rsrc(const_cast<void*>(p.w), 0, p.w_bytes, 0x00020000);
+    const __amdgpu_buffer_rsrc_t rx2 = __builtin_amdgcn_make_buffer_rsrc(const_cast<void*>(q.x2), 0, q.x2_bytes, 0x00020000);
+    const __amdgpu_buffer_rsrc_t rw2 = __builtin_amdgcn_make_buffer_rsrc(const_cast<void*>(q.w2), 0, q.w2_bytes, 0x00020000);
+    constexpr unsigned OOB = 0x80000000u;
+    const int wbase = __builtin_amdgcn_readfirstlane(tid & ~63);
+
+    unsigned a1[A_IT], a2[A_IT], b1, b2;
+#pragma unroll
+    for (int it = 0; it < A_IT; ++it) {
+        const int c = tid + it * NT, row = c >> 2, kce = swz<KC>(row, c & (KC - 1)), m = m0 + row;
+        const bool ok = m < p.M;
+        const int mm = ok ? m : 0;
+        const int n = mm / (p.Ho * p.Wo), r = mm - n * (p.Ho * p.Wo), ho = r / p.Wo, wo = r - ho * p.Wo;
+        const unsigned pix = (unsigned)((n * q.H2 + ho * q.stride2) * q.W2 + wo * q.stride2);
+        a1[it] = ok ? (pix * (unsigned)q.Cin2 + (unsigned)(kce * EP)) * 2u : OOB;
+        a2[it] = ok ? ((unsigned)m * (unsigned)p.Cin + (unsigned)(kce * EP)) * 2u : OOB;
+    }
+    {
+        const int row = tid >> 2, kce = swz<KC>(row, tid & (KC - 1));
+        const int co = n0 + direct_perm<BN / WN>(row);
+        b1 = ((unsigned)co * (unsigned)q.Cin2 + (unsigned)(kce * EP)) * 2u;
+        b2 = ((unsigned)co * (unsigned)p.K + (unsigned)(kce * EP)) * 2u;
+    }
+    const int S1 = q.Cin2 / BK, S = S1 + p.K / BK;
+    auto issue_slab = [&](int s, int buf) {
+        if (s < S1) {
+#pragma unroll
+            for (int it = 0; it < A_IT; ++it) {
+                glds16(rx2, &lds[buf][wbase + it * NT], a1[it]);
+                a1[it] += (unsigned)(BK * sizeof(T));
+            }
+            glds16(rw2, &lds[buf][BM * KC + wbase], b1);
+            b1 += (unsigned)(BK * sizeof(T));
+        } else {
+#pragma unroll
+            for (int it = 0; it < A_IT; ++it) {
+                glds16(rx, &lds[buf][wbase + it * NT], a2[it]);
+                a2[it] += (unsigned)(BK * sizeof(T));
+            }
+            glds16(rw, &lds[buf][BM * KC + wbase], b2);
+            b2 += (unsigned)(BK * sizeof(T));
+        }
+    };
+    {
+        const bool odd = __builtin_amdgcn_readfirstlane(wave) & 1;
+        const int ch = n0 + lane;
+        const float* src = odd ? p.shift : p.scale;
+        const __amdgpu_buffer_rsrc_t rs = make_rsrc_uniform(src, 0x7fffffffu);
+        __builtin_amdgcn_raw_ptr_buffer_load_lds(rs, (__attribute__((address_space(3))) void*)(reinterpret_cast<unsigned*>(aux_lds) + (odd ? 64 : 0)), 4,
+                                                 src ? (unsigned)ch * 4u : OOB, 0, 0, 0);
+        const float* src2 = odd ? q.shift2 : q.scale2;
+        const __amdgpu_buffer_rsrc_t rs2 = make_rsrc_uniform(src2, 0x7fffffffu);
+        __builtin_amdgcn_raw_ptr_buffer_load_lds(rs2, (__attribute__((address_space(3))) void*)(reinterpret_cast<unsigned*>(aux2_lds) + (odd ? 64 : 0)), 4,
+                                                 src2 ? (unsigned)ch * 4u : OOB, 0, 0, 0);
+    }
+    __builtin_amdgcn_sched_barrier(0);
+
+    f32x4_t acc[TM][TN];
+#pragma unroll
+    for (int i = 0; i < TM; ++i)
+#pragma unroll
+        for (int j = 0; j < TN; ++j) acc[i][j] = f32x4_t{0.f, 0.f, 0.f, 0.f};
+    u32x4_t rres[TM][H];
+#pragma unroll
+    for (int i = 0; i < TM; ++i)
+#pragma unroll
+        for (int h = 0; h < H; ++h) rres[i][h] = u32x4_t{0u, 0u, 0u, 0u};
+
+    const int fr = lane & 15, fq = lane >> 4;
+    const unsigned aux2_addr = lds_addr(aux2_lds);
+    const bool has_sc2 = q.scale2 != nullptr, has_sh2 = q.shift2 != nullptr;
+    auto seam = [&]() {
+#pragma unroll
+        for (int h = 0; h < H; ++h) {
+            u32x4_t sc[2], sh[2];
+#pragma unroll
+            for (int k = 0; k < 2; ++k) {
+                const unsigned a = aux2_addr + (unsigned)(h * 32 + fq * 8 + k * 4) * 4u;
+                sc[k] = frag_read<0>(a);
+                sh[k] = frag_read<256>(a);
+            }
+            asm volatile("s_waitcnt lgkmcnt(0)" ::: "memory");
+#pragma unroll
+            for (int k = 0; k < 2; ++k) { asm volatile("" : "+v"(sc[k])); asm volatile("" : "+v"(sh[k])); }
+#pragma unroll
+            for (int i = 0; i < TM; ++i) {
+                float v[8];
+#pragma unroll
+                for (int e = 0; e < 4; ++e) { v[e] = acc[i][2 * h][e]; v[4 + e] = acc[i][2 * h + 1][e]; }
+                if (has_sc2) {
+#pragma unroll
+                    for (int e = 0; e < 4; ++e) { v[e] *= __uint_as_float(sc[0][e]); v[4 + e] *= __uint_as_float(sc[1][e]); }
+                }
+                if (has_sh2) {
+#pragma unroll
+                    for (int e = 0; e < 4; ++e) { v[e] += __uint_as_float(sh[0][e]); v[4 + e] += __uint_as_float(sh[1][e]); }
+                }
+#pragma unroll
+                for (int qd = 0; qd < 4; ++qd) rres[i][h][qd] = pack2_bf16(v[2 * qd], v[2 * qd + 1]);
+            }
+        }
+#pragma unroll
+        for (int i = 0; i < TM; ++i)
+#pragma unroll
+            for (int j = 0; j < TN; ++j) acc[i][j] = f32x4_t{0.f, 0.f, 0.f, 0.f};
+    };
+
+    constexpr int N_DMA = A_IT + 1;
+    issue_slab(0, 0);
+    if (S > 1) issue_slab(1, 1);
+    if (S > 2) issue_slab(2, 2);
+    __builtin_amdgcn_sched_barrier(0);
+    constexpr unsigned SLAB_BYTES = SLOTS * 16;
+    const int xrow = wm * (BM / WM) + fr, wrow = fr;
+    const unsigned x_rd0 = lds_addr(&lds[0][0]) + (unsigned)(xrow * KC + swz<KC>(xrow, fq)) * 16u;
+    const unsigned w_rd0 = lds_addr(&lds[0][0]) + (unsigned)((BM + wrow) * KC + swz<KC>(wrow, fq)) * 16u;
+    u32x4_t xf0[TM], wf0[TN], xf1[TM], wf1[TN];
+    if (S > 2) asm volatile("s_waitcnt vmcnt(%0)" ::"n"(2 * N_DMA) : "memory");
+    else if (S > 1) asm volatile("s_waitcnt vmcnt(%0)" ::"n"(N_DMA) : "memory");
+    else asm volatile("s_waitcnt vmcnt(0)" ::: "memory");
+    __builtin_amdgcn_s_barrier();
+    __builtin_amdgcn_sched_barrier(0);
+    frag_read_all<TM, KC * 16>(xf0, x_rd0);
+    frag_read_all<TN, KC * 16>(wf0, w_rd0);
+    frag_wait<TM, TN>(xf0, wf0);
+    int rbuf = 1, ibuf = 0;
+    auto step = [&](int s, u32x4_t* xc, u32x4_t* wc, u32x4_t* xn, u32x4_t* wn_) {
+        const bool more = s + 1 < S;
+        if (more) {
+            if (s + 2 < S) asm volatile("s_waitcnt vmcnt(%0)" ::"n"(N_DMA) : "memory");
+            else asm volatile("s_waitcnt vmcnt(0)" ::: "memory");
+            __builtin_amdgcn_s_barrier();
+            __builtin_amdgcn_sched_barrier(0);
+        }
+        frag_read_all<TM, KC * 16>(xn, x_rd0 + (unsigned)rbuf * SLAB_BYTES);
+        frag_read_all<TN, KC * 16>(wn_, w_rd0 + (unsigned)rbuf * SLAB_BYTES);
+        if (more && s + 3 < S) issue_slab(s + 3, ibuf);
+#pragma unroll
+        for (int i = 0; i < TM; ++i)
+#pragma unroll
+            for (int j = 0; j < TN; ++j) acc[i][j] = Mma<T>::run(wc[j], xc[i], acc[i][j]);
+        frag_wait<TM, TN>(xn, wn_);
+        rbuf = rbuf == NBUF - 1 ? 0 : rbuf + 1;
+        ibuf = ibuf == NBUF - 1 ? 0 : ibuf + 1;
+        if (s + 1 == S1) seam();
+    };
+    for (int s = 0; s < S; s += 2) {
+        step(s, xf0, wf0, xf1, wf1);
+        if (s + 1 < S) step(s + 1, xf1, wf1, xf0, wf0);
+    }
+    __builtin_amdgcn_sched_barrier(0);
+    igemm_epilogue_direct<BM, BN, WM, WN, true, TWO>(p, acc, m0, n0, rres, lds_addr(aux_lds));
+}
+
+int launch_pair(const bool two, const ConvDev& d, const PairPre& q, hipStream_t st) {
+    const dim3 grid(cdiv(d.M, 128), d.Cout / 64);
+    if (two) hipLaunchKernelGGL((igemm_pair_kernel<true>), grid, dim3(256), 0, st, d, q);
+    else hipLaunchKernelGGL((igemm_pair_kernel<false>), grid, dim3(256), 0, st, d, q);
+    ALDI_CHECK_LAUNCH();
+    return ALDI_OK;
+}
diff --git a/aldi_amd/csrc/igemm_select.h b/aldi_amd/csrc/igemm_select.h
--- a/aldi_amd/csrc/igemm_select.h
+++ b/aldi_amd/csrc/igemm_select.h
@@ -213,6 +213,7 @@
         return aldi_set_error_msg(ALDI_ERR_ARG, "conv_igemm: Cin must be a multiple of 32 (bf16) / 16 (f32) for KxK convs; of a 16-B chunk for 1x1");
     if (a->Cout % 4 != 0) return aldi_set_error_msg(ALDI_ERR_ARG, "conv_igemm: Cout must be a multiple of 4");
     if (a->res_mode == 2 && ((a->Ho & 1) || (a->Wo & 1))) return aldi_set_error_msg(ALDI_ERR_ARG, "conv_igemm: upsample residual needs even Ho,Wo");
+    if (a->res_mode < 0 || a->res_mode > 3 || (a->res_mode == 3 && a->out_scale > 1)) return aldi_set_error_msg(ALDI_ERR_ARG, "conv_igemm: res_mode is 0 .. 3 (3: dense output only)");
     if (a->res_mode && !a->res) return aldi_set_error_msg(ALDI_ERR_ARG, "conv_igemm: res_mode set without res");
     d.x = a->x; d.w = a->w; d.y = a->y; d.y_f32 = a->y_f32; d.scale = a->scale; d.shift = a->shift;
     d.res = a->res; d.mask = a->mask;
@@ -285,4 +286,34 @@
     return ALDI_OK;
 }
 
-}
+struct PairPre {
+    const void* x2; const void* w2; const float* scale2; const float* shift2;
+    int H2, W2, Cin2, stride2;
+    unsigned x2_bytes, w2_bytes;
+};
+inline bool pair_ok(const ConvDev& d, const bool f32, const PairPre& q) {
+    return !f32 && plain_1x1(d) && d.y && !d.y_f32 && d.out_scale == 1 && !d.res_mode && !d.mask && !d.mask_bits && d.ksplit <= 1 && d.Cout % 64 == 0 &&
+           d.K % 32 == 0 && q.x2 && q.w2 && q.Cin2 > 0 && q.Cin2 % 32 == 0 && q.stride2 >= 1 && q.H2 >= 1 && q.W2 >= 1 &&
+           (q.H2 - 1) / q.stride2 + 1 == d.Ho && (q.W2 - 1) / q.stride2 + 1 == d.Wo;
+}
+inline int plan_conv_pair(const aldi_conv_args* a, const aldi_conv_pre_args* pre, const AldiTuning& tn, ConvDev& d, PairPre& q, bool& two) {
+    if (!pre) return aldi_set_error_msg(ALDI_ERR_ARG, "conv_pair_igemm: null pointer");
+    if (int rc = fill_convdev(a, d)) return rc;
+    q = PairPre{pre->x2, pre->w2, pre->scale2, pre->shift2, pre->H2, pre->W2, pre->Cin2, pre->stride2, 0u, 0u};
+    const size_t xb = (size_t)(a->N > 0 ? a->N : 0) * (size_t)(q.H2 > 0 ? q.H2 : 0) * (size_t)(q.W2 > 0 ? q.W2 : 0) * (size_t)(q.Cin2 > 0 ? q.Cin2 : 0) * 2;
+    const size_t wb = (size_t)a->Cout * (size_t)(q.Cin2 > 0 ? q.Cin2 : 0) * 2;
+    if (a->dtype != ALDI_BF16 || a->ksplit > 1 || !pair_ok(d, false, q) || xb >= 0x80000000ull || wb >= 0x80000000ull || (unsigned)pre->rounding > 2u)
+        return aldi_set_error_msg(ALDI_ERR_ARG, "conv_pair_igemm: takes bf16, two 1x1 convs without padding on one output grid, the main one plain (stride 1, no res / "
+                                                "mask / fp32 output / scatter / split-K), Cout % 64 == 0, Cin % 32 == 0, Cin2 % 32 == 0");
+    q.x2_bytes = (unsigned)xb; q.w2_bytes = (unsigned)wb;
+    d.res_mode = 1;
+    d.res = pre->x2;
+    two = pre->rounding == 2;
+    if (pre->rounding == 0) two = kTiles[select_tile(d, tn, false, 0).tile].epi == 0;
+    d.res = nullptr;
+    d.xcd = tn.igemm_xcd; d.dbg = tn.igemm_dbg;
+    return ALDI_OK;
+}
+inline int pair_dispatch_name(const bool two, char* name, int cap) { return snprintf(name, cap, "igemm_pair<bf16,128,64,4,1,pipe,tap,round%d>", two ? 2 : 1); }
+
+}
diff --git a/aldi_amd/csrc/igemm_ws.h b/aldi_amd/csrc/igemm_ws.h
--- a/aldi_amd/csrc/igemm_ws.h
+++ b/aldi_amd/csrc/igemm_ws.h
@@ -36,8 +36,10 @@
     }
     const __amdgpu_buffer_rsrc_t rx = __builtin_amdgcn_make_buffer_rsrc(const_cast<T*>(static_cast<const T*>(p.x)), 0, p.x_bytes, 0x00020000);
     const unsigned out_bytes = (unsigned)p.M * (unsigned)p.Cout * 2u;
-    const bool res_up = p.res_mode == 2;
-    const __amdgpu_buffer_rsrc_t rr = make_rsrc_uniform(p.res, res_up ? out_bytes >> 2 : out_bytes);
+    const bool res_up = p.res_mode >= 2;
+    const unsigned res_s2 = (unsigned)p.res_mode & 1u;
+    const unsigned rHo = (unsigned)(p.Ho + (int)res_s2) >> 1, rWo = (unsigned)(p.Wo + (int)res_s2) >> 1;
+    const __amdgpu_buffer_rsrc_t rr = make_rsrc_uniform(p.res, res_up ? (unsigned)p.N * rHo * rWo * (unsigned)p.Cout * 2u : out_bytes);
     const __amdgpu_buffer_rsrc_t rmb = make_rsrc_uniform(p.mask_bits, out_bytes >> 4);
     const __amdgpu_buffer_rsrc_t ry = make_rsrc_uniform(p.y, out_bytes);
     const __amdgpu_buffer_rsrc_t rbo = make_rsrc_uniform(p.bits_out, out_bytes >> 4);
@@ -81,11 +83,13 @@
                 const unsigned m = (unsigned)(m0 + i * 16 + fr), c = (unsigned)(n0 + h * 32 + fq * 8);
                 if (has_res) {
                     unsigned row = m;
+                    bool rok = m < (unsigned)p.M;
                     if (res_up) {
                         const unsigned t_ = fdiv(m, (unsigned)p.Wo, inv_wo), wo = m - t_ * (unsigned)p.Wo, n = fdiv(t_, (unsigned)p.Ho, inv_ho), ho = t_ - n * (unsigned)p.Ho;
-                        row = (n * (unsigned)(p.Ho >> 1) + (ho >> 1)) * (unsigned)(p.Wo >> 1) + (wo >> 1);
-                    }
-                    rres[i][h] = __builtin_amdgcn_raw_buffer_load_b128(rr, m < (unsigned)p.M ? row * C2 + c * 2u : OOB, 0, 0);
+                        row = (n * rHo + (ho >> 1)) * rWo + (wo >> 1);
+                        rok = rok && !(res_s2 & (ho | wo));
+                    }
+                    rres[i][h] = __builtin_amdgcn_raw_buffer_load_b128(rr, rok ? row * C2 + c * 2u : OOB, 0, 0);
                 }
                 if (has_mb) mb[i][h] = __builtin_amdgcn_raw_buffer_load_b8(rmb, m * C8 + (c >> 3), 0, 0);
             }
diff --git a/aldi_amd/engine.py b/aldi_amd/engine.py
--- a/aldi_amd/engine.py
+++ b/aldi_amd/engine.py
@@ -369,6 +369,7 @@
         self.level_groups = os.environ.get("ALDI_LEVEL_GROUPS", "1") == "1"
         self.fused_res2 = os.environ.get("ALDI_FUSED_RES2", "1") == "1"
         self.fused_res2_shortcut = os.environ.get("ALDI_FUSED_RES2_SHORTCUT", "1") == "1"
+        self.fused_stage_entrance = os.environ.get("ALDI_FUSED_STAGE_ENTRANCE", "1") == "1"
         self._wg_queue: list = []
         self.sparse_rpn_backward = os.environ.get("ALDI_RPN_SPARSE_BWD", "1") == "1"
         spec = getattr(weights.layout, "img_da", None)
@@ -442,11 +443,15 @@
             self._ws[name] = t
         return t
 
-    def _conv_call(self, x, name, *, relu=False, res=None, res_mode=0, want_f32=False, out=None, bits_out=None):
+    def _conv_call(self, x, name, *, relu=False, res=None, res_mode=0, want_f32=False, out=None, bits_out=None, pre=None):
         W = self.wts
         p = W.layout.t[name]
-        return x, W.w(name), dict(stride=p.stride, pad=p.pad, scale=W.scale(name), shift=W.shift(name), res=res, res_mode=res_mode, relu=relu,
-                                  want_f32=want_f32, out=out, bits_out=bits_out)
+        kw = dict(stride=p.stride, pad=p.pad, scale=W.scale(name), shift=W.shift(name), res=res, res_mode=res_mode, relu=relu,
+                  want_f32=want_f32, out=out, bits_out=bits_out)
+        if pre is not None:
+            x2, n2 = pre
+            kw["pre"] = (x2, W.w(n2), W.scale(n2), W.shift(n2), W.layout.t[n2].stride)
+        return x, W.w(name), kw
 
     def conv(self, x, name, **kw):
         x, w, kw = self._conv_call(x, name, **kw)
@@ -497,15 +502,17 @@
                         except StopIteration as e:
                             rb, res[1] = None, e.value
                 continue
-            if ra is not None and rb is not None:
+            paired = any(not isinstance(r, list) and r[2].get("pre") is not None for r in (ra, rb) if r is not None)
+            if ra is not None and rb is not None and not paired:
                 la, lb = (ra if isinstance(ra, list) else [ra]), (rb if isinstance(rb, list) else [rb])
                 ys = ops.conv2d_group([eng_a._conv_call(r[0], r[1], **r[2]) for r in la] + [eng_b._conv_call(r[0], r[1], **r[2]) for r in lb])
                 ya = ys[:len(la)] if isinstance(ra, list) else ys[0]
                 yb = ys[len(la):] if isinstance(rb, list) else ys[len(la)]
-            elif ra is not None:
-                ya = eng_a._serve(ra)
             else:
-                yb = eng_b._serve(rb)
+                if ra is not None:
+                    ya = eng_a._serve(ra)
+                if rb is not None:
+                    yb = eng_b._serve(rb)
             if ra is not None:
                 try:
                     ra = gen_a.send(ya)
@@ -560,7 +567,8 @@
                                              W.shift(p + "conv3"), out=prefix_out if (prefix_out is not None and b == nb - 1) else None,
                                              shortcut=(W.w(p + "shortcut"), W.scale(p + "shortcut"), W.shift(p + "shortcut")) if fold_sc else None)
                     continue
-                sc = (yield x, p + "shortcut", {}) if b == 0 else x
+                fold_sc = b == 0 and self.dtype == torch.bfloat16 and self.fused_stage_entrance
+                sc = (yield x, p + "shortcut", {}) if b == 0 and not fold_sc else x
                 want_bits = save and si > 0 and self.mask_bits and self.dtype == torch.bfloat16
 
                 def bits_for(inp, name):
@@ -575,7 +583,10 @@
                 b2 = bits_for(h1, p + "conv2") if self.mask_bits_inner else None
                 h2 = yield h1, p + "conv2", dict(relu=True, bits_out=b2)
                 bits = bits_for(h2, p + "conv3")
-                out = yield h2, p + "conv3", dict(relu=True, res=sc, res_mode=1, bits_out=bits)
+                if fold_sc:
+                    out = yield h2, p + "conv3", dict(relu=True, bits_out=bits, pre=(x, p + "shortcut"))
+                else:
+                    out = yield h2, p + "conv3", dict(relu=True, res=sc, res_mode=1, bits_out=bits)
                 if save and si > 0:
                     blocks.append((p, x, h1, h2, out, b == 0))
                     if bits is not None:
@@ -1221,7 +1232,7 @@
         dev = self.device
         gx_pre, gx_ev = {}, None
         side0 = self._wgrad_stream()
-        if side0 is not None and "cs" in c:
+        if side0 is not None and "cs" in c and not self._fold_stage_grad():
             side0.wait_stream(torch.cuda.current_stream())
             with torch.cuda.stream(side0):
                 for si_, ci_ in ((3, 2), (2, 1)):
@@ -1346,21 +1357,35 @@
                     self._grads_final(stage_names)
                     if si == 1:
                         break
-                    stride = W.layout.t[p + "conv1"].stride
-                    Hin, Win = xin.shape[1], xin.shape[2]
                     gx = gx_pre.pop(si, None)
-                    if gx is None or gx.shape != xin.shape:
-                        gx = torch.zeros_like(xin)
-                    else:
+                    if gx is not None and gx.shape == xin.shape:
                         torch.cuda.current_stream().wait_event(gx_ev)
                         gx.record_stream(torch.cuda.current_stream())
-                    ops.conv2d(g, W.wt(p + "shortcut"), out=gx, out_scale=stride, out_hw=(Hin, Win))
-                    ops.conv2d(g1, W.wt(p + "conv1"), out=gx, out_scale=stride, out_hw=(Hin, Win), res=gx, res_mode=1)
-                    lvl = si + 1
-                    g = ops.conv2d(gprev[lvl], W.wt(f"backbone.fpn_lateral{lvl}"), res=gx, res_mode=1, **self._relu_mask(c, xin))
+                    else:
+                        gx = None
+                    g = self._stage_input_grad(c, si, p, xin, g, g1, gprev[si + 1], gx)
                 else:
                     g = ops.conv2d(g1, W.wt(p + "conv1"), res=g, res_mode=1, **self._relu_mask(c, xin))
         self._join_wgrads()
+
+    def _fold_stage_grad(self) -> bool:
+        return self.dtype == torch.bfloat16 and self.fused_stage_entrance
+
+    def _stage_input_grad(self, c: Ctx, si: int, p: str, xin: torch.Tensor, g: torch.Tensor, g1: torch.Tensor, gprev: torch.Tensor,
+                          gx: Optional[torch.Tensor] = None) -> torch.Tensor:
+        W = self.wts
+        stride = W.layout.t[p + "conv1"].stride
+        lvl = si + 1
+        lat = W.wt(f"backbone.fpn_lateral{lvl}")
+        if self._fold_stage_grad() and stride == 2:
+            gq = ops.conv2d(g1, W.wt(p + "conv1"), pre=(g, W.wt(p + "shortcut"), None, None, 1, 2))
+            return ops.conv2d(gprev, lat, res=gq, res_mode=3, **self._relu_mask(c, xin))
+        Hin, Win = xin.shape[1], xin.shape[2]
+        if gx is None:
+            gx = torch.zeros_like(xin)
+        ops.conv2d(g, W.wt(p + "shortcut"), out=gx, out_scale=stride, out_hw=(Hin, Win))
+        ops.conv2d(g1, W.wt(p + "conv1"), out=gx, out_scale=stride, out_hw=(Hin, Win), res=gx, res_mode=1)
+        return ops.conv2d(gprev, lat, res=gx, res_mode=1, **self._relu_mask(c, xin))
 
     def trunk_backward(self, c: Ctx, gC: Dict[int, Optional[torch.Tensor]]):
         W = self.wts
diff --git a/aldi_amd/ops.py b/aldi_amd/ops.py
--- a/aldi_amd/ops.py
+++ b/aldi_amd/ops.py
@@ -50,7 +50,7 @@
            mask: Optional[torch.Tensor] = None, out: Optional[torch.Tensor] = None,
            out_f32: Optional[torch.Tensor] = None, want_f32: bool = False,
            out_scale: int = 1, out_hw=None, ksplit: Optional[int] = None, mask_bits: Optional[torch.Tensor] = None,
-           bits_out: Optional[torch.Tensor] = None) -> torch.Tensor:
+           bits_out: Optional[torch.Tensor] = None, pre=None) -> torch.Tensor:
     N, H, W_, Cin = x.shape
     Cout, KH, KW, Cin2 = w.shape
     assert Cin == Cin2 and x.is_contiguous() and w.is_contiguous() and x.dtype == w.dtype, (x.shape, w.shape, x.dtype, w.dtype)
@@ -75,6 +75,13 @@
     a = L.ConvArgs(_p(x), _p(w), _p(out), _p(out_f32), _p(scale), _p(shift), _p(res), _p(mask),
                    N, H, W_, Cin, Cout, KH, KW, stride, pad, Ho, Wo,
                    int(relu), res_mode, out_scale, OH, OW, dtype_code(x.dtype), _p(ws), int(ksplit or 0), _p(mask_bits), _p(bits_out))
+    if pre is not None:
+        x2, w2, scale2, shift2, stride2 = pre[:5]
+        assert res is None and x2.is_contiguous() and w2.is_contiguous() and x2.dtype == x.dtype == w2.dtype and x2.shape[0] == N, (x2.shape, w2.shape)
+        assert w2.shape == (Cout, 1, 1, x2.shape[3]), (w2.shape, Cout, x2.shape)
+        q = L.ConvPreArgs(_p(x2), _p(w2), _p(scale2), _p(shift2), x2.shape[1], x2.shape[2], x2.shape[3], stride2, pre[5] if len(pre) > 5 else 0)
+        L.call("aldi_conv_pair_igemm", C.byref(a), C.byref(q), stream_ptr())
+        return out
     L.call("aldi_conv_igemm", C.byref(a), stream_ptr())
     return out_f32 if want_f32 and out is None else out
 
diff --git a/include/aldi_hip.h b/include/aldi_hip.h
--- a/include/aldi_hip.h
+++ b/include/aldi_hip.h
@@ -47,6 +47,17 @@
 int aldi_conv_igemm(const aldi_conv_args* a, aldi_stream_t stream);
 int aldi_conv_igemm_group(const aldi_conv_args* args, int n, aldi_stream_t stream);
 int aldi_conv_igemm_plan(const aldi_conv_args* args, int n, char* name, int cap);
+
+typedef struct {
+    const void* x2;
+    const void* w2;
+    const float* scale2;
+    const float* shift2;
+    int H2, W2, Cin2, stride2;
+    int rounding;
+} aldi_conv_pre_args;
+int aldi_conv_pair_igemm(const aldi_conv_args* a, const aldi_conv_pre_args* pre, aldi_stream_t stream);
+int aldi_conv_pair_igemm_plan(const aldi_conv_args* a, const aldi_conv_pre_args* pre, char* name, int cap);
 
 typedef struct {
     const void* x;
```

New measurement: 517.7 (median of 6 runs). 1.3% higher.
